# shanjiayao/PTT

Measured on AMD Instinct MI355X. Metric: tracklet frames/sec (hot path: PointNet++ SA stack + Point-Track-Transformer blocks), higher is better.
Workload: dtype f32

## Files before the change

### include/ptt_hip.h

```cpp
#ifndef PTT_HIP_H
#define PTT_HIP_H

#include <stddef.h>
#include <stdint.h>

#ifdef __cplusplus
extern "C" {
#endif

#define PTT_ABI_VERSION 28

enum {
    PTT_OK = 0,
    PTT_EINVAL = -1,
    PTT_EUNSUPPORTED = -2,
    PTT_ELAUNCH = -3,
    PTT_EWORKSPACE = -4
};

typedef void* ptt_stream_t;

int ptt_version(void);
const char* ptt_error_name(int code);
const char* ptt_last_error_string(void);

int ptt_fps_f32(const float* xyz, int B, int N, int npoint, int32_t* idx_out,
                ptt_stream_t stream);
int ptt_fps_ws_f32(const float* xyz, int B, int N, int npoint, int32_t* idx_out, float* workspace,
                   size_t workspace_elems, ptt_stream_t stream);

int ptt_gather_f32(const float* feat, const int32_t* idx, int B, int C, int N, int M,
                   float* out, ptt_stream_t stream);
int ptt_gather_grad_f32(const float* grad_out, const int32_t* idx, int B, int C, int N,
                        int M, float* grad_feat, ptt_stream_t stream);

int ptt_select_centres_f32(const float* xyz, const int32_t* idx, int B, int N, int M, float* new_xyz,
                           int64_t* idx64_out, ptt_stream_t stream);

int ptt_ball_query_f32(const float* new_xyz, const float* xyz, int B, int M, int N,
                       float radius, int nsample, int32_t* idx_out, ptt_stream_t stream);

int ptt_centres_ball_query_f32(const float* xyz, const int32_t* sel, int B, int N, int M, float radius, int nsample,
                               float* new_xyz, int64_t* idx64_out, int32_t* idx_out, ptt_stream_t stream);

int ptt_group_f32(const float* feat, const int32_t* idx, int B, int C, int N, int M,
                  int ns, float* out, ptt_stream_t stream);
int ptt_group_grad_f32(const float* grad_out, const int32_t* idx, int B, int C, int N,
                       int M, int ns, float* grad_feat, ptt_stream_t stream);

size_t ptt_scatter_add_det_workspace(int B, int N, int E);
int ptt_scatter_add_det_f32(const float* src, const int32_t* idx, int B, int C, int N, int E, float* out,
                            void* workspace, size_t workspace_bytes, ptt_stream_t stream);

int ptt_knn_f32(const float* xyz, int B, int N, int k, int32_t* idx_out,
                ptt_stream_t stream);
int ptt_knn_rel_f32(const float* xyz, int B, int N, int k, int32_t* idx_out, float* rel_out,
                    ptt_stream_t stream);

size_t ptt_packed_weight_elems(int Cout, int K);
int ptt_pack_weight_f32(const float* W, int Cout, int K, float* packed,
                        ptt_stream_t stream);
int ptt_pack_weight_rot_f32(const float* W, int Cout, int K, int rot, float* packed,
                            ptt_stream_t stream);

int ptt_linear_f32(const float* X, int rows, int K, int ldx, const float* Wpacked, int Cout,
                   const float* scale, const float* shift, int relu, const float* residual,
                   int ldr, float* out, int ldo, ptt_stream_t stream);

#define PTT_SA_MAX_LAYERS 4

typedef struct ptt_sa_layer {
    const float* Wpacked;
    const float* scale;
    const float* shift;
    int Cin;
    int Cout;
    int relu;
} ptt_sa_layer;

int ptt_rows_mlp_f32(const float* X, int rows, int K, int ldx, const ptt_sa_layer* layers, int n_layers,
                     const float* residual, int ldr, float* out, int ldo, ptt_stream_t stream);

size_t ptt_ball_query_grid_workspace(int B, int N);
int ptt_ball_query_grid_f32(const float* new_xyz, const float* xyz, int B, int M, int N, float radius, int nsample,
                            int32_t* idx_out, void* workspace, size_t workspace_bytes, ptt_stream_t stream);
int ptt_centres_ball_query_grid_f32(const float* xyz, const int32_t* sel, int B, int N, int M, float radius, int nsample,
                                    float* new_xyz, int64_t* idx64_out, int32_t* idx_out, void* workspace, size_t workspace_bytes,
                                    ptt_stream_t stream);
int ptt_fps_ball_knn_f32(const float* xyz, int B, int N, int M, float radius, int nsample, int k, int32_t* inds,
                         int64_t* inds64, float* new_xyz, int32_t* idx, int32_t* knn, float* rel, ptt_stream_t stream);
#define PTT_POINT_JOBS_MAX 4
typedef struct ptt_point_job {
    const float* xyz; const int32_t* centre_sel; const int32_t* point_sel;
    float* new_xyz; int64_t* idx64_out; int32_t* idx_out; float* rel_out;
    int32_t kind, sel_ld, B, Nraw, Npts, M, nsample;
    float radius;
} ptt_point_job;
int ptt_point_jobs_f32(const ptt_point_job* jobs, int n_jobs, ptt_stream_t stream);

#define PTT_ROW_JOBS_MAX 4
typedef struct ptt_row_job {
    const float* X; const float* X2;
    const float* Xmax;
    const float* Wpacked; const float* scale; const float* shift;
    const float* res; const float* res2;
    float* out; float* out2; float* raw;
    const float* rel; const float* w1;
    const float* qkv; const int32_t* knn; const float* pos;
    int32_t rows, K, K1, ldx, ldx2, Cout;
    int32_t act, res_split, ldr, ldr2, out_split, out_col0, ldo, ldo2, ldraw;
    int32_t prologue, epilogue, ldq, q_off, k_off, v_off, ldp, N;
    float sm_scale;
    int32_t col_tiles;
    const int32_t* idx; const float* xyz; const float* centres; const float* wx;
    float radius;
    int32_t ns, M, normalize_xyz, pro_relu;
} ptt_row_job;
int ptt_row_jobs_f32(const ptt_row_job* jobs, int n_jobs, ptt_stream_t stream);

typedef struct ptt_sa_desc {
    const float* xyz;
    const float* new_xyz;
    const int32_t* idx;
    const float* feat;
    int64_t feat_sb, feat_sc, feat_sn;
    float* out;
    int64_t out_sb, out_sc, out_sm;
    int B, N, M, nsample, C;
    float radius;
    int use_xyz;
    int normalize_xyz;
    int n_layers;
    ptt_sa_layer layers[PTT_SA_MAX_LAYERS];
    const float* l0_point_term;
    const float* l0_xyz_weight;
    int l0_channels;
    int l0_relu;
    void* compact_ws;
    size_t compact_ws_bytes;
} ptt_sa_desc;

int ptt_sa_fused_fwd_f32(const ptt_sa_desc* d, ptt_stream_t stream);
size_t ptt_sa_compact_workspace(int B, int M);

typedef struct ptt_xcorr_desc {
    const float* cos_t;
    const float* P;
    const float* w_sim;
    const float* scale0;
    const float* shift0;
    float* out;
    int64_t out_sb, out_sc, out_sn;
    float* sim_out;
    int B, Ns, Nt, C0;
    int n_layers;
    ptt_sa_layer layers[PTT_SA_MAX_LAYERS];
    int32_t split; int64_t out_sh;
    const float* search_feat; const float* templ_feat;
    int64_t s_sb, s_sn, t_sb, t_sn;
    int C; float eps;
} ptt_xcorr_desc;

int ptt_xcorr_fused_fwd_f32(const ptt_xcorr_desc* d, ptt_stream_t stream);

int ptt_cosine_map_f32(const float* search_feat, int64_t s_sb, int64_t s_sn, int64_t s_sc, const float* templ_feat,
                       int64_t t_sb, int64_t t_sn, int64_t t_sc, int B, int Ns, int Nt, int C, float eps,
                       float* cos_t, ptt_stream_t stream);

typedef struct ptt_attn_desc {
    const float* xyz;
    const float* rel;
    const int32_t* knn;
    const float* qkv;
    const float* Wd1p;
    const float* Wd2p;
    const float* bd2;
    const float* Wg1p;
    const float* bg1;
    const float* Wg2p;
    const float* bg2;
    float* res;
    float* attn;
    int B, N, k, D;
    const int32_t* order;
    int heads;
} ptt_attn_desc;

int ptt_pt_attn_pair_f32(const ptt_attn_desc* d, ptt_stream_t stream);
int ptt_spatial_order_f32(const float* xyz, int B, int N, int32_t* order, ptt_stream_t stream);

typedef struct ptt_crop_job {
    const float* points;
    int64_t ld;
    double lo1[3], hi1[3];
    double trans[3];
    double rot[9];
    double lo2[3], hi2[3];
    float* out;
    int32_t* count;
    int32_t n_points;
    int32_t capacity;
    uint8_t* label_out;
    double ltrans[3];
    double lrot[9];
    double llo[3], lhi[3];
    int32_t append;
    int32_t reserved;
} ptt_crop_job;

int ptt_crop_compact_f32(const ptt_crop_job* jobs_device, int n_jobs, ptt_stream_t stream);
#define PTT_CROP_JOBS_BY_VALUE_MAX 8
int ptt_crop_compact_host_f32(const ptt_crop_job* jobs_host, int n_jobs, ptt_stream_t stream);

#define PTT_MAX_SEGMENTS 4
typedef struct ptt_regularize_job {
    const float* seg[PTT_MAX_SEGMENTS];
    const int32_t* seg_count[PTT_MAX_SEGMENTS];
    int32_t seg_capacity[PTT_MAX_SEGMENTS];
    float* out;
    int32_t* info;
    int32_t n_seg;
    int32_t input_size;
} ptt_regularize_job;

int ptt_regularize_f32(const ptt_regularize_job* jobs_device, int n_jobs, const uint32_t* draws, int n_draws,
                       ptt_stream_t stream);
int ptt_crop_regularize_f32(const ptt_crop_job* crop_jobs, const ptt_regularize_job* reg_jobs_device, int n_jobs,
                            const uint32_t* draws, int n_draws, ptt_stream_t stream);

int ptt_mt19937_fill(uint32_t seed, uint32_t* out_host, int n);

typedef struct ptt_track_box {
    double center[3];
    double wlh[3];
    double quat[4];
} ptt_track_box;

int ptt_track_crop_bounds(const ptt_track_box* boxes, int n, double offset, double scale, const double* extra2,
                          ptt_crop_job* jobs_host, int job_stride);
int ptt_track_box_by_offset(ptt_track_box* boxes, int n, float* offsets, int offset_stride, int use_z,
                            const int32_t* active, int64_t* rng_pos);
int ptt_track_select_update(const float* proposals_host, int P, const int32_t* info_host, ptt_track_box* boxes, int n, int use_z,
                            const int32_t* active, int64_t* rng_pos, float* est_out);

int ptt_select_box_f32(const float* pred_box_data, int B, int P, float* out, int32_t* idx_out, ptt_stream_t stream);

#define PTT_REF_CAMERA 0
#define PTT_REF_LIDAR 1
int ptt_box_overlap_f64(const double* gt, const double* pred, int n, int ref_coord, int dims, double* overlap, double* accuracy,
                        ptt_stream_t stream);

#define PTT_TRAIN_MAX_CANDS 1024
typedef struct ptt_train_cand {
    const float* search;
    const uint8_t* label;
    const float* first;
    const float* prev;
    const int32_t* counts;
    float reg[4];
    uint32_t index;
    uint32_t epoch;
    int32_t capacity;
    int32_t reserved;
} ptt_train_cand;

typedef struct ptt_train_batch_desc {
    float* search_points;
    float* template_points;
    float* cls_label;
    float* reg_label;
    int32_t* src_out;
    int32_t* idx_search_out;
    int32_t* idx_template_out;
    int32_t* info;
    int64_t* totals;
    int32_t B, n_cand;
    int32_t search_size, template_size;
    int32_t min_points;
    uint32_t seed_lo, seed_hi;
    int32_t reserved;
} ptt_train_batch_desc;

int ptt_train_batch_f32(const ptt_train_cand* cands_device, const ptt_train_batch_desc* desc_host, ptt_stream_t stream);
int ptt_philox4x32_10(const uint32_t* counter4, const uint32_t* key2, uint32_t* out4);

size_t ptt_bn_stats_workspace(int R, int C);
int ptt_bn_stats_f32(const float* X, int R, int C, int ldx, float eps, float* mean, float* var, float* invstd,
                     void* workspace, size_t workspace_bytes, ptt_stream_t stream);
int ptt_bn_apply_f32(const float* Z, int ldz, const float* mean, const float* invstd, const float* gamma,
                     const float* beta, int R, int C, int relu, float* X, int ldx, ptt_stream_t stream);
int ptt_bn_bwd_f32(const float* G, int ldg, const float* Act, int lda, const float* Z, int ldz, const float* mean,
                   const float* invstd, const float* gamma, int R, int C, int relu, float* dZ, int ldd,
// ... 227 lines not shown
```

### ptt_amd/_lib.py

```python
import ctypes
import os
import re
from ctypes import Structure, c_char_p, c_double, c_float, c_int, c_int32, c_int64, c_longlong, c_size_t, c_uint32, c_void_p

from .build import HEADER as HEADER_PATH, LIB as LIB_PATH


def _strip_comments(text):
    return re.sub(r"/\*.*?\*/|//[^\n]*", " ", text, flags=re.S)


def parse_defines(text):
    return {n: int(v) for n, v in re.findall(r"^[ \t]*#[ \t]*define[ \t]+(PTT_\w+)[ \t]+(-?\d+)[ \t]*$", _strip_comments(text), re.M)}


CTYPES = {"int": c_int, "int32_t": c_int32, "uint32_t": c_uint32, "int64_t": c_int64, "long long": c_longlong, "size_t": c_size_t,
          "float": c_float, "double": c_double, "ptt_stream_t": c_void_p}


def _ctype(decl, name, is_return=False):
    words = decl.replace("*", " * ").split()
    if not is_return and len(words) > 1 and words[-1] != "*":
        words.pop()
    if "*" in words:
        if not is_return:
            return c_void_p
        if words == ["const", "char", "*"]:
            return c_char_p
    base = " ".join(w for w in words if w != "const")
    if base not in CTYPES:
        raise RuntimeError("ptt_amd: %s of %s in include/ptt_hip.h has the type '%s', which ptt_amd/_lib.py does not map to ctypes"
                           % ("the return value" if is_return else "parameter '%s'" % decl.strip(), name, base))
    return CTYPES[base]


def parse_prototypes(text):
    text = re.sub(r"^[ \t]*#.*$", " ", _strip_comments(text), flags=re.M).replace('extern "C" {', " ")
    text = re.sub(r"\{[^{}]*\}", " ", text)
    protos = {}
    for stmt in text.split(";"):
        stmt = " ".join(stmt.split()).lstrip("} ")
        if not stmt or stmt.split()[0] in ("typedef", "enum", "struct"):
            continue
        m = re.fullmatch(r"(.+?)\b(\w+) ?\((.*)\)", stmt)
        if m is None:
            raise RuntimeError("ptt_amd: cannot read '%s' in include/ptt_hip.h as a function prototype" % stmt)
        ret, name, params = m.groups()
        params = [] if params.strip() == "void" else params.split(",")
        protos[name] = (_ctype(ret, name, is_return=True), [_ctype(p, name) for p in params])
    return protos


def _read_header():
    if not os.path.exists(HEADER_PATH):
        raise RuntimeError("ptt_amd: %s is missing — the Python binding takes every prototype and constant of the C ABI from it" % HEADER_PATH)
    with open(HEADER_PATH) as fh:
        return fh.read()


_header = _read_header()
PROTOTYPES = parse_prototypes(_header)
EXPORTS = list(PROTOTYPES)
DEFINES = parse_defines(_header)
ABI_VERSION = DEFINES["PTT_ABI_VERSION"]
PTT_SA_MAX_LAYERS = DEFINES["PTT_SA_MAX_LAYERS"]
PTT_MAX_SEGMENTS = DEFINES["PTT_MAX_SEGMENTS"]
PTT_CROP_JOBS_BY_VALUE_MAX = DEFINES["PTT_CROP_JOBS_BY_VALUE_MAX"]
PTT_TRAIN_MAX_CANDS = DEFINES["PTT_TRAIN_MAX_CANDS"]


class CropJob(Structure):
    _fields_ = [("points", c_void_p), ("ld", c_int64),
                ("lo1", c_double * 3), ("hi1", c_double * 3), ("trans", c_double * 3), ("rot", c_double * 9),
                ("lo2", c_double * 3), ("hi2", c_double * 3),
                ("out", c_void_p), ("count", c_void_p), ("n_points", c_int32), ("capacity", c_int32),
                ("label_out", c_void_p), ("ltrans", c_double * 3), ("lrot", c_double * 9), ("llo", c_double * 3), ("lhi", c_double * 3),
                ("append", c_int32), ("reserved", c_int32)]


class RegularizeJob(Structure):
    _fields_ = [("seg", c_void_p * PTT_MAX_SEGMENTS), ("seg_count", c_void_p * PTT_MAX_SEGMENTS),
                ("seg_capacity", c_int32 * PTT_MAX_SEGMENTS), ("out", c_void_p), ("info", c_void_p),
                ("n_seg", c_int32), ("input_size", c_int32)]


class TrackBox(Structure):
    _fields_ = [("center", c_double * 3), ("wlh", c_double * 3), ("quat", c_double * 4)]


class TrainCand(Structure):
    _fields_ = [("search", c_void_p), ("label", c_void_p), ("first", c_void_p), ("prev", c_void_p), ("counts", c_void_p),
                ("reg", c_float * 4), ("index", c_uint32), ("epoch", c_uint32), ("capacity", c_int32), ("reserved", c_int32)]


class TrainBatchDesc(Structure):
    _fields_ = [("search_points", c_void_p), ("template_points", c_void_p), ("cls_label", c_void_p), ("reg_label", c_void_p),
                ("src_out", c_void_p), ("idx_search_out", c_void_p), ("idx_template_out", c_void_p), ("info", c_void_p), ("totals", c_void_p),
                ("B", c_int32), ("n_cand", c_int32), ("search_size", c_int32), ("template_size", c_int32), ("min_points", c_int32),
                ("seed_lo", c_uint32), ("seed_hi", c_uint32), ("reserved", c_int32)]


class BnTrainTail(Structure):
    _fields_ = [("gamma", c_void_p), ("beta", c_void_p), ("act_a", c_void_p), ("act_b", c_void_p),
                ("running_mean", c_void_p), ("running_var", c_void_p), ("num_batches_tracked", c_void_p), ("momentum", c_float)]


class BnBwdInput(Structure):
    _fields_ = [("g", c_void_p), ("ldg", c_int), ("arg", c_void_p), ("ns", c_int), ("z", c_void_p), ("ldz", c_int),
                ("k1", c_void_p), ("c0", c_void_p), ("c1", c_void_p), ("mean", c_void_p), ("act_a", c_void_p), ("act_b", c_void_p),
                ("dz_out", c_void_p), ("ldd", c_int)]


class PackJob(Structure):
    _fields_ = [("W", c_void_p), ("out_offset", c_int64), ("stride_out", c_int64), ("stride_k", c_int64),
                ("Cout", c_int32), ("K", c_int32)]


class RowJob(Structure):
    _fields_ = [("X", c_void_p), ("X2", c_void_p), ("Xmax", c_void_p), ("Wpacked", c_void_p), ("scale", c_void_p), ("shift", c_void_p),
                ("res", c_void_p), ("res2", c_void_p), ("out", c_void_p), ("out2", c_void_p), ("raw", c_void_p),
                ("rel", c_void_p), ("w1", c_void_p), ("qkv", c_void_p), ("knn", c_void_p), ("pos", c_void_p),
                ("rows", c_int32), ("K", c_int32), ("K1", c_int32), ("ldx", c_int32), ("ldx2", c_int32), ("Cout", c_int32),
                ("act", c_int32), ("res_split", c_int32), ("ldr", c_int32), ("ldr2", c_int32), ("out_split", c_int32),
                ("out_col0", c_int32), ("ldo", c_int32), ("ldo2", c_int32), ("ldraw", c_int32),
                ("prologue", c_int32), ("epilogue", c_int32), ("ldq", c_int32), ("q_off", c_int32), ("k_off", c_int32),
                ("v_off", c_int32), ("ldp", c_int32), ("N", c_int32), ("sm_scale", c_float), ("col_tiles", c_int32),
                ("idx", c_void_p), ("xyz", c_void_p), ("centres", c_void_p), ("wx", c_void_p), ("radius", c_float),
                ("ns", c_int32), ("M", c_int32), ("normalize_xyz", c_int32), ("pro_relu", c_int32)]


class PointJob(Structure):
    _fields_ = [("xyz", c_void_p), ("centre_sel", c_void_p), ("point_sel", c_void_p), ("new_xyz", c_void_p), ("idx64_out", c_void_p),
                ("idx_out", c_void_p), ("rel_out", c_void_p), ("kind", c_int32), ("sel_ld", c_int32), ("B", c_int32),
                ("Nraw", c_int32), ("Npts", c_int32), ("M", c_int32), ("nsample", c_int32), ("radius", c_float)]


class TrackLossDesc(Structure):
    _fields_ = [("seed_cls", c_void_p), ("cls_label", c_void_p), ("search_inds", c_void_p), ("votes", c_void_p), ("reg_label", c_void_p),
                ("box_data", c_void_p), ("centres", c_void_p), ("pos_weight_seed", c_void_p), ("pos_weight_box", c_void_p),
                ("B", c_int32), ("N", c_int32), ("Ns", c_int32), ("M", c_int32), ("ld_reg", c_int32),
                ("w_seed_cls", c_float), ("w_seed_reg", c_float), ("w_box_cls", c_float), ("w_box_reg", c_float)]


class AdamTensor(Structure):
    _fields_ = [("param", c_void_p), ("grad", c_void_p), ("exp_avg", c_void_p), ("exp_avg_sq", c_void_p), ("n", c_int64)]


class GradJob(Structure):
    _fields_ = [("partial", c_void_p), ("nchunks", c_int32), ("reserved", c_int32)]


class GradSegment(Structure):
    _fields_ = [("dst", c_int64), ("n", c_int32), ("cols", c_int32), ("ld", c_int32), ("job0", c_int32), ("njobs", c_int32), ("out", c_int32),
                ("vec", c_int32), ("reserved", c_int32)]


class AdamHyper(Structure):
    _fields_ = [("beta1", c_float), ("beta2", c_float), ("one_minus_beta1", c_float), ("one_minus_beta2", c_float), ("eps", c_float), ("step_size", c_float), ("bias2_sqrt", c_float),
                ("weight_decay", c_float), ("max_norm", c_float), ("write_clipped", c_int32)]


class SaLayer(Structure):
    _fields_ = [("Wpacked", c_void_p), ("scale", c_void_p), ("shift", c_void_p),
                ("Cin", c_int), ("Cout", c_int), ("relu", c_int)]


class SaDesc(Structure):
    _fields_ = [("xyz", c_void_p), ("new_xyz", c_void_p), ("idx", c_void_p), ("feat", c_void_p),
                ("feat_sb", c_int64), ("feat_sc", c_int64), ("feat_sn", c_int64),
                ("out", c_void_p), ("out_sb", c_int64), ("out_sc", c_int64), ("out_sm", c_int64),
                ("B", c_int), ("N", c_int), ("M", c_int), ("nsample", c_int), ("C", c_int),
                ("radius", c_float), ("use_xyz", c_int), ("normalize_xyz", c_int), ("n_layers", c_int),
                ("layers", SaLayer * PTT_SA_MAX_LAYERS),
                ("l0_point_term", c_void_p), ("l0_xyz_weight", c_void_p), ("l0_channels", c_int), ("l0_relu", c_int),
                ("compact_ws", c_void_p), ("compact_ws_bytes", c_size_t)]


class XcorrDesc(Structure):
    _fields_ = [("cos_t", c_void_p), ("P", c_void_p), ("w_sim", c_void_p), ("scale0", c_void_p), ("shift0", c_void_p),
                ("out", c_void_p), ("out_sb", c_int64), ("out_sc", c_int64), ("out_sn", c_int64),
                ("sim_out", c_void_p),
                ("B", c_int), ("Ns", c_int), ("Nt", c_int), ("C0", c_int),
                ("n_layers", c_int), ("layers", SaLayer * PTT_SA_MAX_LAYERS),
                ("split", c_int32), ("out_sh", c_int64), ("search_feat", c_void_p), ("templ_feat", c_void_p),
                ("s_sb", c_int64), ("s_sn", c_int64), ("t_sb", c_int64), ("t_sn", c_int64), ("C", c_int), ("eps", c_float)]


class AttnDesc(Structure):
    _fields_ = [("xyz", c_void_p), ("rel", c_void_p), ("knn", c_void_p), ("qkv", c_void_p),
                ("Wd1p", c_void_p), ("Wd2p", c_void_p), ("bd2", c_void_p),
                ("Wg1p", c_void_p), ("bg1", c_void_p), ("Wg2p", c_void_p), ("bg2", c_void_p),
                ("res", c_void_p), ("attn", c_void_p),
                ("B", c_int), ("N", c_int), ("k", c_int), ("D", c_int), ("order", c_void_p), ("heads", c_int)]


_lib = None


def lib():
    global _lib
    if _lib is None:
        if not os.path.exists(LIB_PATH):
            raise RuntimeError(
                "ptt_amd: %s is missing — build it with `python -m ptt_amd.build` "
                "(hipcc --offload-arch=gfx950); there is no CPU fallback" % LIB_PATH)
        import torch
        try:
            loaded = ctypes.CDLL(LIB_PATH)
        except OSError as e:
            raise RuntimeError("ptt_amd: cannot load %s: %s" % (LIB_PATH, e))
        for name, (restype, argtypes) in PROTOTYPES.items():
            fn = getattr(loaded, name)
            fn.restype, fn.argtypes = restype, argtypes
        if loaded.ptt_version() != ABI_VERSION:
            raise RuntimeError("ptt_amd: %s has ABI version %d, this package expects %d — rebuild it with "
                               "`python -m ptt_amd.build`" % (LIB_PATH, loaded.ptt_version(), ABI_VERSION))
        _lib = loaded
    return _lib


def check(rc, what):
    if rc != 0:
        l = lib()
        raise RuntimeError("%s failed: %s (%s)" % (what, l.ptt_error_name(rc).decode(),
                                                   l.ptt_last_error_string().decode()))
```

### ptt_amd/csrc/common.h

```cpp
#pragma once
#include <hip/hip_runtime.h>
#include <stdint.h>
#include <stdio.h>
#include "../../include/ptt_hip.h"

namespace ptt {

char* last_error_buf();
int fail(int code, const char* fmt, ...);
int check_launch(const char* what);

static inline hipStream_t as_stream(ptt_stream_t s) { return reinterpret_cast<hipStream_t>(s); }

struct DevSwitches {
    int linear_rt = 1, linear_ct = 1;
    int linear_small = 1;
    int sa_gather1 = 0;
    int sa_stagger = 0;
    int sa_wave = 1;
    int sa_rt = 2;
    int sa_lds = 1;
    int sa_stream = 1;
    int sa_chunk = 2;
    int pair_stagger = 0;
    int pair_lds_pad = 0;
    int sa_lds_chunk = 2;
    int fps_plain = 0;
    int ball_cpw = 0;
    int fps_t = 0;
    int group_grad_global = 0;
    long long* stamps = nullptr;
};
const DevSwitches& dev_switches();

int set_lds_limit(const void* fn, int bytes);

bool wgrad_stream_ok(int R, int Cout, int Cin, int ldz, int ldx);
int wgrad_stream_rows(int R);
int launch_wgrad_stream(const float* dZ, int ldz, const float* X, int ldx, int R, int Cout, int Cin, int rows, float* partial,
                        const float* x_scale, const float* x_shift, hipStream_t s);

template <int CTRL, int ROW_MASK>
__device__ __forceinline__ int dpp_i32(int v) {
    return __builtin_amdgcn_update_dpp(v, v, CTRL, ROW_MASK, 0xF, false);
}
template <int CTRL, int ROW_MASK>
__device__ __forceinline__ float dpp_f32(float v) {
    return __builtin_bit_cast(float, dpp_i32<CTRL, ROW_MASK>(__builtin_bit_cast(int, v)));
}

__device__ __forceinline__ float wave_max_f32(float v) {
    v = fmaxf(v, dpp_f32<0xB1, 0xF>(v));
    v = fmaxf(v, dpp_f32<0x4E, 0xF>(v));
    v = fmaxf(v, dpp_f32<0x141, 0xF>(v));
    v = fmaxf(v, dpp_f32<0x140, 0xF>(v));
    v = fmaxf(v, dpp_f32<0x142, 0xA>(v));
    v = fmaxf(v, dpp_f32<0x143, 0xC>(v));
    return __builtin_bit_cast(float, __builtin_amdgcn_readlane(__builtin_bit_cast(int, v), 63));
}
__device__ __forceinline__ float wave_max_f32_fused(float v) {
    asm volatile(
        "s_nop 1\n\tv_max_f32_dpp %0, %0, %0 quad_perm:[1,0,3,2] row_mask:0xf bank_mask:0xf\n\t"
        "s_nop 1\n\tv_max_f32_dpp %0, %0, %0 quad_perm:[2,3,0,1] row_mask:0xf bank_mask:0xf\n\t"
        "s_nop 1\n\tv_max_f32_dpp %0, %0, %0 row_half_mirror row_mask:0xf bank_mask:0xf\n\t"
        "s_nop 1\n\tv_max_f32_dpp %0, %0, %0 row_mirror row_mask:0xf bank_mask:0xf\n\t"
        "s_nop 1\n\tv_max_f32_dpp %0, %0, %0 row_bcast:15 row_mask:0xa bank_mask:0xf\n\t"
        "s_nop 1\n\tv_max_f32_dpp %0, %0, %0 row_bcast:31 row_mask:0xc bank_mask:0xf\n\t"
        "s_nop 1"
        : "+v"(v));
    return __builtin_bit_cast(float, __builtin_amdgcn_readlane(__builtin_bit_cast(int, v), 63));
}

__device__ __forceinline__ float wave_min_f32(float v) {
    v = fminf(v, dpp_f32<0xB1, 0xF>(v));
    v = fminf(v, dpp_f32<0x4E, 0xF>(v));
    v = fminf(v, dpp_f32<0x141, 0xF>(v));
    v = fminf(v, dpp_f32<0x140, 0xF>(v));
    v = fminf(v, dpp_f32<0x142, 0xA>(v));
    v = fminf(v, dpp_f32<0x143, 0xC>(v));
    return __builtin_bit_cast(float, __builtin_amdgcn_readlane(__builtin_bit_cast(int, v), 63));
}
__device__ __forceinline__ int wave_min_i32(int v) {
    v = min(v, dpp_i32<0xB1, 0xF>(v));
    v = min(v, dpp_i32<0x4E, 0xF>(v));
    v = min(v, dpp_i32<0x141, 0xF>(v));
    v = min(v, dpp_i32<0x140, 0xF>(v));
    v = min(v, dpp_i32<0x142, 0xA>(v));
    v = min(v, dpp_i32<0x143, 0xC>(v));
    return __builtin_amdgcn_readlane(v, 63);
}

}
```

### ptt_amd/csrc/mfma_ops.hip

```cpp
#include <math.h>
#include <stdlib.h>
#include <string.h>
#include "common.h"
#include "mfma_common.h"

#ifndef PTT_PAIR_PF
#define PTT_PAIR_PF 1
#endif
#ifndef PTT_GATHER_BATCH
#define PTT_GATHER_BATCH 16
#endif
#ifndef PTT_SA_WAVES
#define PTT_SA_WAVES 2
#endif

namespace ptt {

#ifdef PTT_DEV
#define PTT_STAMP(i) do { if (p.dbg && threadIdx.x == 0 && blockIdx.x < 4096) p.dbg[blockIdx.x * 8 + (i)] = __builtin_readcyclecounter(); } while (0)
#else
#define PTT_STAMP(i) do { } while (0)
#endif

__device__ __forceinline__ void stagger_second_slot(int first_wave_blocks, int quanta) {
// ... 1099 lines not shown
            for (int c = sub * 4; c < q.C; c += 32) {
                const f32x4 av = *reinterpret_cast<const f32x4*>(a + c), sv = *reinterpret_cast<const f32x4*>(sv_ + c);
#pragma unroll
                for (int k = 0; k < 4; ++k) { dot += av[k] * sv[k]; na += av[k] * av[k]; ns += sv[k] * sv[k]; }
            }
#pragma unroll
            for (int m = 1; m < 8; m <<= 1) { dot += __shfl_xor(dot, m, 64); na += __shfl_xor(na, m, 64); ns += __shfl_xor(ns, m, 64); }
            if (sub == 0) simv[i] = dot / (fmaxf(sqrtf(na), q.eps) * fmaxf(sqrtf(ns), q.eps));
        } else {
            if (t < ROWS) {
                const float cs = q.cos_t[(unsigned)((b * p.M + jj) * q.Nt + i0 + t)];
                simv[t] = cs;
                if (q.sim_out) q.sim_out[(unsigned)((b * q.Nt + i0 + t) * p.M + jj)] = cs;
            }
        }
        __syncthreads();

        const int nq = q.C0 >> 2;
        if (!q.scale0 && !q.shift0 && (q.C0 & 3) == 0 && (256 % nq) == 0) {
            typedef float f32x2 __attribute__((ext_vector_type(2)));
            const int c4 = t % nq, step = 256 / nq;
            const f32x4 w4 = *reinterpret_cast<const f32x4*>(q.wsim + c4 * 4);
            const float* prow = q.P + ((size_t)(b * q.Nt + i0) * q.C0 + c4 * 4);
            for (int i = t / nq; i < ROWS; i += step) {
                const f32x4 pv = *reinterpret_cast<const f32x4*>(prow + (unsigned)(i * q.C0));
                const float cs = simv[i];
                const f32x2 c2 = {cs, cs};
                f32x2 lo = __builtin_elementwise_fma(f32x2{w4[0], w4[1]}, c2, f32x2{pv[0], pv[1]});
                f32x2 hi = __builtin_elementwise_fma(f32x2{w4[2], w4[3]}, c2, f32x2{pv[2], pv[3]});
                *reinterpret_cast<f32x4*>(Xs + i * p.ldk + c4 * 4) =
                    f32x4{fmaxf(lo[0], 0.f), fmaxf(lo[1], 0.f), fmaxf(hi[0], 0.f), fmaxf(hi[1], 0.f)};
            }
        } else {
            for (int c = t; c < q.C0; c += 256) {
                const float wsim = q.wsim[c], sc = q.scale0 ? q.scale0[c] : 1.f, sh = q.shift0 ? q.shift0[c] : 0.f;
                const float* pr = q.P + ((long long)b * q.Nt + i0) * q.C0 + c;
#pragma unroll 8
                for (int i = 0; i < ROWS; ++i) {
                    const float v = (pr[(long long)i * q.C0] + wsim * simv[i]) * sc + sh;
                    Xs[i * p.ldk + c] = fmaxf(v, 0.f);
                }
            }
        }
        __syncthreads();

        for (int l = 0; l < nlast; ++l) {
            const SaLayerDev& L = p.L[l];
            const int ctw = (L.NT + 3) >> 2;
            if (ctw <= 1) sa_layer<32 * RT, 1, RT>(p, L, false, Xs, lane, w, j, 1, pre, &p.L[l + 1]);
            else sa_layer<32 * RT, 2, RT>(p, L, false, Xs, lane, w, j, 1, pre, &p.L[l + 1]);
        }
        {
            const bool affine = LL.scale != nullptr;
            f32x16 acc[RT][2];
#pragma unroll
            for (int rt = 0; rt < RT; ++rt)
#pragma unroll
                for (int u = 0; u < 2; ++u)
#pragma unroll
                    for (int r = 0; r < 16; ++r) acc[rt][u][r] = pre.sh[u];
            int nvalid = 0;
#pragma unroll
            for (int u = 0; u < 2; ++u)
                if (w + 4 * u < LL.NT) nvalid = u + 1;
            gemm_tiles<RT, 2, 0>(Xs, p.ldk, LL.nkb, reinterpret_cast<const f32x4*>(LL.Wp), LL.NT, w, nvalid, lane, acc, pre.w);
#pragma unroll
            for (int u = 0; u < 2; ++u) {
                if (u >= nvalid) break;
                const int col = (w + 4 * u) * 32 + (lane & 31);
                float sc = 1.f, sh = 0.f;
                if (affine) { sc = LL.scale[col]; sh = LL.shift ? LL.shift[col] : 0.f; }
#pragma unroll
                for (int rt = 0; rt < RT; ++rt) {
                    float m = affine ? acc[rt][u][0] * sc + sh : acc[rt][u][0];
#pragma unroll
                    for (int r = 1; r < 16; ++r) m = fmaxf(m, affine ? acc[rt][u][r] * sc + sh : acc[rt][u][r]);
                    run[u] = fmaxf(run[u], max_halves(m));
                }
            }
        }
    }
    if (half == 0) {
#pragma unroll
        for (int u = 0; u < 2; ++u) {
            if (w + 4 * u >= LL.NT) break;
            const int col = (w + 4 * u) * 32 + (lane & 31);
            p.out[(SPLIT ? hsel * q.out_sh : 0) + b * p.osb + col * p.osc + jj * p.osm] = LL.relu ? fmaxf(run[u], 0.f) : run[u];
        }
    }
}

template <int NS, int CT, bool AFFINE, int RT>
__device__ __forceinline__ void sa_wave_layer(const SaParams& p, const SaLayerDev& L, bool last, float* Xw, int lane,
                                              int centre0, int ncentres) {
    f32x16 acc[RT][CT];
#pragma unroll
    for (int u = 0; u < CT; ++u) {
        const float s0 = (!AFFINE && L.shift) ? L.shift[u * 32 + (lane & 31)] : 0.f;
#pragma unroll
        for (int rt = 0; rt < RT; ++rt)
#pragma unroll
            for (int r = 0; r < 16; ++r) acc[rt][u][r] = s0;
    }
    gemm_core<RT, CT, CT, 1>(Xw, p.ldk, L.nkb, reinterpret_cast<const f32x4*>(L.Wp), L.NT, 0, lane, acc);
    __builtin_amdgcn_wave_barrier();
    const int half = lane >> 5;
#pragma unroll
    for (int u = 0; u < CT; ++u) {
        const int col = u * 32 + (lane & 31);
        float sc = 1.f, sv = 0.f;
        if constexpr (AFFINE) { sc = L.scale[col]; sv = L.shift ? L.shift[col] : 0.f; }
#pragma unroll
        for (int rt = 0; rt < RT; ++rt) {
            float y[16];
#pragma unroll
            for (int r = 0; r < 16; ++r) y[r] = AFFINE ? acc[rt][u][r] * sc + sv : acc[rt][u][r];
            if (!last) {
#pragma unroll
                for (int r = 0; r < 16; ++r)
                    Xw[(rt * 32 + tile_row(r, half)) * p.ldk + col] = L.relu ? fmaxf(y[r], 0.f) : y[r];
            } else if (NS == 32) {
                float m = y[0];
#pragma unroll
                for (int r = 1; r < 16; ++r) m = fmaxf(m, y[r]);
                m = max_halves(m);
                if (L.relu) m = fmaxf(m, 0.f);
                if (half == 0 && rt < ncentres) {
                    const int c = centre0 + rt; const int b = c / p.M, mm = c - b * p.M;
                    p.out[b * p.osb + col * p.osc + mm * p.osm] = m;
                }
            } else {
                float m0 = y[0], m1 = y[8];
#pragma unroll
                for (int r = 1; r < 8; ++r) { m0 = fmaxf(m0, y[r]); m1 = fmaxf(m1, y[8 + r]); }
                m0 = max_halves(m0);
                m1 = max_halves(m1);
                if (L.relu) { m0 = fmaxf(m0, 0.f); m1 = fmaxf(m1, 0.f); }
                if (half == 0) {
                    if (2 * rt < ncentres) {
                        const int c = centre0 + 2 * rt; const int b = c / p.M, mm = c - b * p.M;
                        p.out[b * p.osb + col * p.osc + mm * p.osm] = m0;
                    }
                    if (2 * rt + 1 < ncentres) {
                        const int c = centre0 + 2 * rt + 1; const int b = c / p.M, mm = c - b * p.M;
                        p.out[b * p.osb + col * p.osc + mm * p.osm] = m1;
                    }
                }
            }
        }
    }
    __builtin_amdgcn_wave_barrier();
}

constexpr int SAC_HDR = 16;
struct SacTable {
    int32_t* ws; int T;
    __host__ __device__ int32_t* ndist() const { return ws + SAC_HDR; }
    __host__ __device__ int32_t* list(int k) const { return ws + SAC_HDR + (size_t)(1 + k) * T; }
    __host__ __device__ int32_t* rows(int k) const { return ws + SAC_HDR + 5 * (size_t)T + (size_t)((4 << k) - 4) * T; }
    static size_t words(size_t T) { return SAC_HDR + 65 * T; }
};
constexpr int SAC_PASSES = 4;

__global__ __launch_bounds__(64) void sa_compact_zero_kernel(int32_t* ws) {
    if (threadIdx.x < 4) ws[threadIdx.x] = 0;
}

template <bool XYZ>
__global__ __launch_bounds__(256) void sa_compact_kernel(const float* __restrict__ xyz, const int32_t* __restrict__ idx, int N, int M,
                                                         SacTable tab) {
    __shared__ int s_cnt[4], s_base[4], s_cls[32], s_pos[32], s_nd[32];
    __shared__ int s_row[32][32];
    const int t = threadIdx.x, lane = t & 63, half = lane >> 5, s = lane & 31, w = t >> 6;
    const int g0 = blockIdx.x * 32, T = tab.T;
    if (t < 4) s_cnt[t] = 0;
    __syncthreads();
    int iv[SAC_PASSES];
    uint32_t x[SAC_PASSES], y[SAC_PASSES], z[SAC_PASSES];
#pragma unroll
    for (int q = 0; q < SAC_PASSES; ++q) iv[q] = idx[(size_t)min(g0 + q * 8 + w * 2 + half, T - 1) * 32 + s];
    if constexpr (XYZ) {
#pragma unroll
        for (int q = 0; q < SAC_PASSES; ++q) {
            const int b = min(g0 + q * 8 + w * 2 + half, T - 1) / M;
            const uint32_t* pt = reinterpret_cast<const uint32_t*>(xyz) + ((size_t)b * N + iv[q]) * 3;
            x[q] = pt[0]; y[q] = pt[1]; z[q] = pt[2];
        }
    }
#pragma unroll
    for (int q = 0; q < SAC_PASSES; ++q) {
        const int lc = q * 8 + w * 2 + half;
        const int i0a = __builtin_amdgcn_readlane(iv[q], 0), i0b = __builtin_amdgcn_readlane(iv[q], 32);
        const int i0 = half ? i0b : i0a;
        const bool real = s == 0 || iv[q] != i0;
        int dup = 0;
        if constexpr (XYZ) {
            const unsigned long long rm = __ballot(real);
            const int J = 31 - __builtin_clz((uint32_t)rm | (uint32_t)(rm >> 32));
            for (int j = 0; j < J; ++j) {
                const uint32_t xa = __builtin_amdgcn_readlane(x[q], j), xb = __builtin_amdgcn_readlane(x[q], 32 + j);
                const uint32_t ya = __builtin_amdgcn_readlane(y[q], j), yb = __builtin_amdgcn_readlane(y[q], 32 + j);
                const uint32_t za = __builtin_amdgcn_readlane(z[q], j), zb = __builtin_amdgcn_readlane(z[q], 32 + j);
                dup |= (int)(j < s) & (int)(x[q] == (half ? xb : xa)) & (int)(y[q] == (half ? yb : ya)) & (int)(z[q] == (half ? zb : za));
            }
        }
        const bool keep = real && !dup;
        const unsigned long long km = __ballot(keep);
        const uint32_t m = half ? (uint32_t)(km >> 32) : (uint32_t)km;
        const int nd = __popc(m);
        if (keep) s_row[lc][__popc(m & ((1u << s) - 1u))] = iv[q];
        if (s == 0) {
            const int k = nd <= 4 ? 0 : nd <= 8 ? 1 : nd <= 16 ? 2 : 3;
            const bool valid = g0 + lc < T;
            s_cls[lc] = valid ? k : -1;
            s_nd[lc] = nd;
            s_pos[lc] = valid ? atomicAdd(&s_cnt[k], 1) : 0;
            if (valid) tab.ndist()[g0 + lc] = nd;
        }
    }
    __syncthreads();
    if (t < 4) s_base[t] = s_cnt[t] ? atomicAdd(&tab.ws[t], s_cnt[t]) : 0;
    __syncthreads();
    for (int e = t; e < 32 * 32; e += 256) {
        const int lc = e >> 5, j = e & 31, k = s_cls[lc];
        if (k < 0 || j >= (4 << k)) continue;
        const int q = s_base[k] + s_pos[lc];
        tab.rows(k)[(size_t)q * (4 << k) + j] = s_row[lc][j < s_nd[lc] ? j : 0];
        if (j == 0) tab.list(k)[q] = g0 + lc;
    }
}

#ifndef PTT_SAL_WGS
#define PTT_SAL_WGS 1
#endif
#ifndef PTT_SAL_WAVES
#define PTT_SAL_WAVES 12
#endif

template <int ROWS>
struct SacTileT {
    static constexpr int LG = ROWS == 32 ? 3 : 4;
    static_assert(ROWS == 32 || ROWS == 64, "32- or 64-row tiles");
    int k, first, n;
    __device__ __forceinline__ static void count(const int32_t* ws, int total, int (&cnt)[4], int (&tiles)[4]) {
#pragma unroll
        for (int k = 0; k < 4; ++k) {
            cnt[k] = min(max(ws[k], 0), total);
            tiles[k] = (k ? tiles[k - 1] : 0) + ((cnt[k] + ((1 << LG) >> k) - 1) >> (LG - k));
        }
    }
    __device__ __forceinline__ void at(int j, const int (&tiles)[4], const int (&cnt)[4]) {
        k = j < tiles[0] ? 0 : j < tiles[1] ? 1 : j < tiles[2] ? 2 : 3;
        const int j0 = k == 0 ? 0 : k == 1 ? tiles[0] : k == 2 ? tiles[1] : tiles[2];
        const int nk = k == 0 ? cnt[0] : k == 1 ? cnt[1] : k == 2 ? cnt[2] : cnt[3];
        first = (j - j0) << (LG - k);
        n = min((1 << LG) >> k, nk - first);
    }
    __device__ __forceinline__ void row(const SacTable& tab, int s, int& n_out, int& ball) const {
        const int cl = s >> (2 + k), inb = cl < n;
        n_out = tab.rows(k)[(size_t)first * (4 << k) + (inb ? s : (s & ((4 << k) - 1)))];
        ball = tab.list(k)[first + (inb ? cl : 0)];
    }
};
using SacTile = SacTileT<32>;

template <int NU>
__device__ __forceinline__ void sac_store(int k, int n, int ball, int M, const f32x16 (&acc)[NU], const float (&sh)[NU],
                                          float* const (&o)[NU], int relu, int half, int osb, int osm) {
    int ob[8];
#pragma unroll
    for (int g = 0; g < 8; ++g) {
        if (g >= (8 >> k)) break;
        const int id = __builtin_amdgcn_readlane(ball, g << (2 + k)), b = id / M;
        ob[g] = b * osb + (id - b * M) * osm;
    }
#pragma unroll
    for (int u = 0; u < NU; ++u) {
        const f32x16& a = acc[u];
        if (k == 3) {
            const float mx = sas_pool(a, sh[u], relu);
            if (half == 0) o[u][ob[0]] = mx;
        } else if (k == 2) {
            float m0 = a[0], m1 = a[8];
#pragma unroll
            for (int r = 1; r < 8; ++r) { m0 = fmaxf(m0, a[r]); m1 = fmaxf(m1, a[8 + r]); }
            m0 = max_halves(m0) + sh[u]; m1 = max_halves(m1) + sh[u];
            if (relu) { m0 = fmaxf(m0, 0.f); m1 = fmaxf(m1, 0.f); }
            if (half < n) o[u][half ? ob[1] : ob[0]] = half ? m1 : m0;
        } else {
            float m[4];
#pragma unroll
            for (int q = 0; q < 4; ++q) m[q] = fmaxf(fmaxf(a[4 * q], a[4 * q + 1]), fmaxf(a[4 * q + 2], a[4 * q + 3]));
            if (k == 1) {
#pragma unroll
                for (int q = 0; q < 4; ++q) m[q] = max_halves(m[q]) + sh[u];
#pragma unroll
                for (int i = 0; i < 2; ++i) {
                    const int g = 2 * half + i;
                    float v = half ? m[2 + i] : m[i];
                    if (relu) v = fmaxf(v, 0.f);
                    if (g < n) o[u][half ? ob[2 + i] : ob[i]] = v;
                }
            } else {
#pragma unroll
                for (int q = 0; q < 4; ++q) {
                    const int g = 2 * q + half;
                    float v = m[q] + sh[u];
                    if (relu) v = fmaxf(v, 0.f);
                    if (g < n) o[u][half ? ob[2 * q + 1] : ob[2 * q]] = v;
                }
            }
        }
    }
}
// ... 473 lines not shown
extern "C" int ptt_pack_weight_strided_f32(const float* W, int Cout, int K, int64_t stride_out, int64_t stride_k, int batch,
                                           int64_t stride_batch, float* packed, ptt_stream_t stream) {
    if (Cout <= 0 || K <= 0 || batch < 0) return fail(PTT_EINVAL, "ptt_pack_weight_strided_f32: Cout=%d K=%d batch=%d", Cout, K, batch);
    if (batch == 0) return PTT_OK;
    if (!W || !packed) return fail(PTT_EINVAL, "ptt_pack_weight_strided_f32: null pointer");
    const size_t total = ptt_packed_weight_elems(Cout, K);
    const int NT = (Cout + 31) / 32;
    size_t g = (total + 255) / 256;
    if (g > 1024) g = 1024;
    hipLaunchKernelGGL(pack_weight_kernel, dim3((unsigned)g, (unsigned)batch), dim3(256), 0, as_stream(stream), W, Cout, K, NT, 0,
                       total, packed, (long long)stride_out, (long long)stride_k, (long long)stride_batch);
    return check_launch("pack_weight_kernel");
}

extern "C" int ptt_pack_weights_f32(const ptt_pack_job* jobs_device, int n_jobs, float* arena, ptt_stream_t stream) {
    if (n_jobs < 0) return fail(PTT_EINVAL, "ptt_pack_weights_f32: n_jobs=%d", n_jobs);
    if (n_jobs == 0) return PTT_OK;
    if (!jobs_device || !arena) return fail(PTT_EINVAL, "ptt_pack_weights_f32: null pointer");
    if (n_jobs > 65535) return fail(PTT_EUNSUPPORTED, "ptt_pack_weights_f32: n_jobs=%d exceeds one launch (65535)", n_jobs);
    hipLaunchKernelGGL(pack_weights_kernel, dim3(32, (unsigned)n_jobs), dim3(256), 0, as_stream(stream), jobs_device, arena);
    return check_launch("pack_weights_kernel");
}

extern "C" int ptt_pack_weight_f32(const float* W, int Cout, int K, float* packed, ptt_stream_t stream) {
    return ptt_pack_weight_rot_f32(W, Cout, K, 0, packed, stream);
}

static int linear_launch(const float* X, int rows, int K, int ldx, const float* Wpacked, int Cout, const float* scale,
                         const float* shift, int relu, const float* residual, int ldr, float* out, int ldo, int batch,
                         long long xb, long long wb, long long ob, long long rb, ptt_stream_t stream,
                         const float* in_a = nullptr, const float* in_b = nullptr);

extern "C" int ptt_linear_act_in_f32(const float* X, int rows, int K, int ldx, const float* in_scale, const float* in_shift,
                                     const float* Wpacked, int Cout, float* out, int ldo, ptt_stream_t stream) {
    if (!in_scale || !in_shift || (K & 3) || (ldx & 3) || ((reinterpret_cast<uintptr_t>(X) | reinterpret_cast<uintptr_t>(in_scale) |
                                                             reinterpret_cast<uintptr_t>(in_shift)) & 15))
        return fail(PTT_EINVAL, "ptt_linear_act_in_f32: needs K %% 4 == 0, ldx %% 4 == 0 and 16-byte aligned X / in_scale / in_shift");
    return linear_launch(X, rows, K, ldx, Wpacked, Cout, nullptr, nullptr, 0, nullptr, 0, out, ldo, 1, 0, 0, 0, 0, stream, in_scale,
                         in_shift);
}

extern "C" int ptt_linear_f32(const float* X, int rows, int K, int ldx, const float* Wpacked, int Cout,
                              const float* scale, const float* shift, int relu, const float* residual, int ldr,
                              float* out, int ldo, ptt_stream_t stream) {
    return linear_launch(X, rows, K, ldx, Wpacked, Cout, scale, shift, relu, residual, ldr, out, ldo, 1, 0, 0, 0, 0, stream);
}

extern "C" int ptt_linear_batched_f32(const float* X, int rows, int K, int ldx, int64_t x_batch_stride, const float* Wpacked,
                                      int64_t w_batch_stride, int Cout, const float* scale, const float* shift, int relu,
                                      const float* residual, int ldr, int64_t r_batch_stride, float* out, int ldo,
                                      int64_t o_batch_stride, int batch, ptt_stream_t stream) {
    if (batch < 0 || batch > 65535) return fail(PTT_EINVAL, "ptt_linear_batched_f32: batch=%d", batch);
    if (batch == 0) return PTT_OK;
    return linear_launch(X, rows, K, ldx, Wpacked, Cout, scale, shift, relu, residual, ldr, out, ldo, batch, x_batch_stride,
                         w_batch_stride, o_batch_stride, r_batch_stride, stream);
}

static int linear_launch(const float* X, int rows, int K, int ldx, const float* Wpacked, int Cout, const float* scale,
                         const float* shift, int relu, const float* residual, int ldr, float* out, int ldo, int batch,
                         long long xb, long long wb, long long ob, long long rb, ptt_stream_t stream, const float* in_a,
                         const float* in_b) {
    if (rows < 0 || K <= 0 || Cout <= 0 || ldx < K || ldo < Cout || (residual && ldr < Cout))
        return fail(PTT_EINVAL, "ptt_linear_f32: rows=%d K=%d Cout=%d ldx=%d ldo=%d ldr=%d", rows, K, Cout, ldx, ldo,
                    ldr);
    if (rows == 0) return PTT_OK;
    if (!X || !Wpacked || !out) return fail(PTT_EINVAL, "ptt_linear_f32: null pointer");
    LinearParams p;
    p.X = X; p.Wp = Wpacked; p.scale = scale; p.shift = shift; p.residual = residual; p.out = out;
    p.rows = rows; p.K = K; p.ldx = ldx; p.Cout = Cout; p.relu = relu; p.ldr = ldr; p.ldo = ldo;
    p.nkb = (K + 7) / 8; p.NT = (Cout + 31) / 32;
    p.vec_ok = ((ldx & 3) == 0 && (xb & 3) == 0 && (reinterpret_cast<uintptr_t>(X) & 15) == 0) ? 1 : 0;
    p.xb = xb; p.wb = wb; p.ob = ob; p.rb = rb;
    p.in_a = in_a; p.in_b = in_b;
    const bool vec = p.vec_ok && (K & 3) == 0;
    hipStream_t s = as_stream(stream);
    if (dev_switches().linear_small && vec && batch == 1 && !in_a && rows <= 8192 && K <= 520 && K >= 32) {
        const int hb = ((p.nkb + 1) / 2 + LS_PD - 1) / LS_PD * LS_PD;
        const int lds = (32 * (2 * hb * 8 + 4) + 4 * 16 * 64) * (int)sizeof(float);
        if (int rc = set_lds_limit(reinterpret_cast<const void*>(linear_small_kernel), lds)) return rc;
        hipLaunchKernelGGL(linear_small_kernel, dim3((rows + 31) / 32, (p.NT + 3) / 4), dim3(512), lds, s, p);
        return check_launch("linear_small_kernel");
    }
    const int rt64 = (rows + 63) / 64, rt32 = (rows + 31) / 32, cg256 = (p.NT + 7) / 8, cg128 = (p.NT + 3) / 4;
    int RT = dev_switches().linear_rt, CT = dev_switches().linear_ct;
    if (rows >= 32768 && Cout >= 256 && RT == 1 && CT == 1) CT = 2;
    const int lds = 2 * (RT * 32) * LIN_LDK * (int)sizeof(float);
    const dim3 grid(RT == 2 ? rt64 : rt32, CT == 2 ? cg256 : cg128, batch);
    int rc = PTT_OK;
#define PTT_LIN_CASE(R, V, C)                                                                                  \
    if (RT == R && vec == V && CT == C) {                                                                      \
        if ((rc = set_lds_limit(reinterpret_cast<const void*>(linear_kernel<R, V, C>), lds))) return rc;       \
        hipLaunchKernelGGL((linear_kernel<R, V, C>), grid, dim3(256), lds, s, p);                              \
    }
    PTT_LIN_CASE(1, true, 1) PTT_LIN_CASE(1, true, 2) PTT_LIN_CASE(1, false, 1) PTT_LIN_CASE(1, false, 2)
#ifdef PTT_DEV
    PTT_LIN_CASE(2, true, 1) PTT_LIN_CASE(2, true, 2) PTT_LIN_CASE(2, false, 1) PTT_LIN_CASE(2, false, 2)
#endif
#undef PTT_LIN_CASE
    return check_launch("linear_kernel");
}

extern "C" int ptt_rows_mlp_f32(const float* X, int rows, int K, int ldx, const ptt_sa_layer* layers, int n_layers,
                                const float* residual, int ldr, float* out, int ldo, ptt_stream_t stream) {
    if (rows < 0 || K <= 0 || ldx < K || n_layers < 1 || n_layers > PTT_SA_MAX_LAYERS || !layers)
        return fail(PTT_EINVAL, "ptt_rows_mlp_f32: rows=%d K=%d ldx=%d layers=%d", rows, K, ldx, n_layers);
    if (rows == 0) return PTT_OK;
    if (!X || !out) return fail(PTT_EINVAL, "ptt_rows_mlp_f32: null pointer");
    if (K > 264) return fail(PTT_EUNSUPPORTED, "ptt_rows_mlp_f32: K=%d (at most 264 input channels)", K);
    RowsMlpParams p;
    p.X = X; p.residual = residual; p.out = out; p.rows = rows; p.K0 = K; p.ldx = ldx; p.ldr = ldr; p.ldo = ldo;
    p.n_layers = n_layers;
    int maxk = 0, cin = K;
    for (int l = 0; l < n_layers; ++l) {
        const ptt_sa_layer& s = layers[l];
        const bool last = l == n_layers - 1;
        if (s.Cin != cin) return fail(PTT_EINVAL, "ptt_rows_mlp_f32: layer %d Cin=%d, expected %d", l, s.Cin, cin);
        if (s.Cout <= 0 || s.Cout > (last ? 384 : 256))
            return fail(PTT_EUNSUPPORTED, "ptt_rows_mlp_f32: layer %d Cout=%d (inner layers <= 256, the last <= 384)", l, s.Cout);
        if (!s.Wpacked) return fail(PTT_EINVAL, "ptt_rows_mlp_f32: layer %d has no weights", l);
        SaLayerDev& L = p.L[l];
        L.Wp = s.Wpacked; L.scale = s.scale; L.shift = s.shift; L.Cin = s.Cin; L.Cout = s.Cout; L.relu = s.relu;
        L.nkb = (s.Cin + 7) / 8; L.NT = (s.Cout + 31) / 32;
        if (L.nkb * 8 > maxk) maxk = L.nkb * 8;
        if (!last && L.NT * 32 > maxk) maxk = L.NT * 32;
        cin = s.Cout;
    }
    if (ldo < cin || (residual && ldr < cin)) return fail(PTT_EINVAL, "ptt_rows_mlp_f32: ldo=%d ldr=%d Cout=%d", ldo, ldr, cin);
    p.ldk = maxk + 4;
    p.vec_in = ((K & 3) == 0 && (ldx & 3) == 0 && (reinterpret_cast<uintptr_t>(X) & 15) == 0) ? 1 : 0;
    const int lds = 32 * p.ldk * (int)sizeof(float);
    int rc = set_lds_limit(reinterpret_cast<const void*>(rows_mlp_kernel), lds);
    if (rc) return rc;
    hipLaunchKernelGGL(rows_mlp_kernel, dim3((rows + 31) / 32), dim3(256), lds, as_stream(stream), p);
    return check_launch("rows_mlp_kernel");
}

extern "C" size_t ptt_sa_compact_workspace(int B, int M) {
    const long long T = (long long)(B > 0 ? B : 0) * (M > 0 ? M : 0);
    return SacTable::words((size_t)T) * sizeof(int32_t);
}

extern "C" int ptt_sa_fused_fwd_f32(const ptt_sa_desc* d, ptt_stream_t stream) {
    if (!d) return fail(PTT_EINVAL, "ptt_sa_fused_fwd_f32: null descriptor");
    if (d->B < 0 || d->N <= 0 || d->M < 0 || d->C < 0 || d->n_layers < 1 || d->n_layers > PTT_SA_MAX_LAYERS)
        return fail(PTT_EINVAL, "ptt_sa_fused_fwd_f32: B=%d N=%d M=%d C=%d layers=%d", d->B, d->N, d->M, d->C,
                    d->n_layers);
    if (d->nsample != 16 && d->nsample != 32 && d->nsample != 64)
        return fail(PTT_EUNSUPPORTED, "ptt_sa_fused_fwd_f32: nsample=%d (16, 32 and 64 are instantiated)", d->nsample);
    if (d->B == 0 || d->M == 0) return PTT_OK;
    const bool hoist = d->l0_point_term != nullptr;
    if (!d->xyz || !d->new_xyz || !d->idx || !d->out || (!hoist && d->C > 0 && !d->feat))
        return fail(PTT_EINVAL, "ptt_sa_fused_fwd_f32: null pointer");
    if (!d->use_xyz && d->C == 0) return fail(PTT_EINVAL, "ptt_sa_fused_fwd_f32: no xyz and no features");
    if (hoist) {
        const int c0 = d->l0_channels;
        if (!d->use_xyz || !d->l0_xyz_weight || c0 <= 0 || (c0 % 32) != 0 || c0 > 256 ||
            (reinterpret_cast<uintptr_t>(d->l0_point_term) & 15) != 0 ||
            (reinterpret_cast<uintptr_t>(d->l0_xyz_weight) & 15) != 0)
            return fail(PTT_EINVAL, "ptt_sa_fused_fwd_f32: hoisted layer 0 needs use_xyz, 16-byte aligned (B,N,C0) and "
                        "(3,C0) arrays and C0 a multiple of 32 <= 256 (C0=%d)", c0);
    }

    SaParams p;
    p.xyz = d->xyz; p.new_xyz = d->new_xyz; p.idx = d->idx; p.feat = d->feat; p.out = d->out;
    p.fsb = d->feat_sb; p.fsc = d->feat_sc; p.fsn = d->feat_sn;
    p.osb = d->out_sb; p.osc = d->out_sc; p.osm = d->out_sm;
    p.B = d->B; p.N = d->N; p.M = d->M; p.C = d->C; p.use_xyz = d->use_xyz ? 1 : 0;
    p.normalize = d->normalize_xyz ? 1 : 0; p.n_layers = d->n_layers; p.radius = d->radius;
    p.K0 = (d->use_xyz ? 3 : 0) + d->C;
    p.hoist = hoist ? 1 : 0; p.l0_relu = d->l0_relu ? 1 : 0; p.wx = d->l0_xyz_weight;
    if (hoist && d->l0_channels == 128 && (unsigned long long)d->B * d->N * 128ull * sizeof(float) < 0x7fffffffull &&
        !dev_switches().sa_gather1)
        p.hoist = 2;
    if (hoist) {
        p.feat = d->l0_point_term; p.C = d->l0_channels; p.K0 = p.C;
        p.fsc = 1; p.fsn = p.C; p.fsb = (long long)d->N * p.C;
    }
    int maxk = 0, cin = p.K0;
    for (int l = 0; l < d->n_layers; ++l) {
        const ptt_sa_layer& s = d->layers[l];
        if (s.Cin != cin) return fail(PTT_EINVAL, "ptt_sa_fused_fwd_f32: layer %d Cin=%d, expected %d", l, s.Cin, cin);
        if (s.Cout <= 0 || (s.Cout % 32) != 0 || s.Cout > 256)
            return fail(PTT_EUNSUPPORTED, "ptt_sa_fused_fwd_f32: layer %d Cout=%d must be a multiple of 32 <= 256", l,
                        s.Cout);
        if (!s.Wpacked) return fail(PTT_EINVAL, "ptt_sa_fused_fwd_f32: layer %d has no weights", l);
        SaLayerDev& L = p.L[l];
        L.Wp = s.Wpacked; L.scale = s.scale; L.shift = s.shift; L.Cin = s.Cin; L.Cout = s.Cout; L.relu = s.relu;
        L.nkb = (s.Cin + 7) / 8; L.NT = s.Cout / 32;
        if (L.nkb * 8 > maxk) maxk = L.nkb * 8;
        if (l + 1 < d->n_layers && s.Cout > maxk) maxk = s.Cout;
        cin = s.Cout;
    }
    {
        const unsigned long long lim = 0x7fffffffull, B = (unsigned long long)d->B;
        if (B * d->N * 12ull >= lim || B * d->M * d->nsample * 4ull >= lim || B * d->M * (unsigned long long)cin * 4ull >= lim ||
            B * d->N * (unsigned long long)(p.C > 0 ? p.C : 1) * 4ull >= lim)
            return fail(PTT_EUNSUPPORTED, "ptt_sa_fused_fwd_f32: B=%d N=%d M=%d: an array of this launch exceeds 2 GiB "
                        "(32-bit offsets) — split the batch", d->B, d->N, d->M);
    }
    p.ldk = maxk + 4;
    p.vec_gather = (p.C > 0 && p.fsc == 1 && (p.C & 3) == 0 && p.C <= 256 && (p.fsn & 3) == 0 &&
                    (p.fsb & 3) == 0 && (reinterpret_cast<uintptr_t>(p.feat) & 15) == 0) ? 1 : 0;
    p.first_wave = 1024; p.stagger = dev_switches().sa_stagger;
    p.dbg = dev_switches().stamps;
    p.cws = nullptr;
    const int total_centres = d->B * d->M;
    hipStream_t s = as_stream(stream);
    int rc;
    if (d->C == 0 && d->use_xyz && !hoist && d->nsample == 32 && d->n_layers == 3 && p.L[0].Cout == 64 && p.L[1].Cout == 64 &&
        p.L[2].Cout == 128 && !p.L[0].scale && !p.L[1].scale && !p.L[2].scale && p.L[0].relu && p.L[1].relu &&
        dev_switches().sa_lds) {
        const int waves = 256 * PTT_SAL_WAVES * PTT_SAL_WGS;
        p.chunk = (total_centres + waves - 1) / waves;
        if (dev_switches().sa_lds_chunk > 0 && p.chunk > dev_switches().sa_lds_chunk) p.chunk = dev_switches().sa_lds_chunk;
        const int nw = total_centres * 3 <= 256 * PTT_SAL_WAVES ? 4 : PTT_SAL_WAVES;
        int wgs = (total_centres + p.chunk * nw - 1) / (p.chunk * nw);
        const int lds = (4096 + 8192 + PTT_SAL_WAVES * 640) * (int)sizeof(float);
        if (d->compact_ws) {
            if (d->compact_ws_bytes < ptt_sa_compact_workspace(d->B, d->M) || (reinterpret_cast<uintptr_t>(d->compact_ws) & 15))
                return fail(PTT_EWORKSPACE, "ptt_sa_fused_fwd_f32: compact_ws needs %zu bytes, 16-byte aligned (got %zu)",
                            ptt_sa_compact_workspace(d->B, d->M), d->compact_ws_bytes);
            p.cws = static_cast<int32_t*>(d->compact_ws);
            hipLaunchKernelGGL(sa_compact_zero_kernel, dim3(1), dim3(64), 0, s, p.cws);
            if ((rc = check_launch("sa_compact_zero_kernel"))) return rc;
            hipLaunchKernelGGL(sa_compact_kernel<true>, dim3((total_centres + 31) / 32), dim3(256), 0, s, d->xyz, d->idx, d->N, d->M,
                               SacTable{p.cws, total_centres});
            if ((rc = check_launch("sa_compact_kernel"))) return rc;
            if (wgs > 256 * PTT_SAL_WGS) wgs = 256 * PTT_SAL_WGS;
            if ((rc = set_lds_limit(reinterpret_cast<const void*>(sa_lds_kernel<true>), lds))) return rc;
            hipLaunchKernelGGL(sa_lds_kernel<true>, dim3(wgs), dim3(64 * nw), lds, s, p);
            return check_launch("sa_lds_kernel");
        }
        if ((rc = set_lds_limit(reinterpret_cast<const void*>(sa_lds_kernel<false>), lds))) return rc;
        hipLaunchKernelGGL(sa_lds_kernel<false>, dim3(wgs), dim3(64 * nw), lds, s, p);
        return check_launch("sa_lds_kernel");
    }
    size_t wbytes = 0;
    bool wave_ok = true;
    for (int l = 0; l < d->n_layers; ++l) {
        wbytes += (size_t)d->layers[l].Cin * d->layers[l].Cout * sizeof(float);
        const int nt = d->layers[l].Cout / 32;
        if (!(nt == 1 || nt == 2 || nt == 4)) wave_ok = false;
    }
    wave_ok = wave_ok && dev_switches().sa_wave;
    if (wave_ok && wbytes <= 64 * 1024 && d->nsample <= 32) {
        const int lds = 4 * 32 * p.ldk * (int)sizeof(float);
        const int cpw = 32 / d->nsample, per_wg = 4 * cpw;
        const dim3 grid((total_centres + per_wg - 1) / per_wg);
        if (d->nsample == 32) {
            if ((rc = set_lds_limit(reinterpret_cast<const void*>(sa_wave_kernel<32, 1>), lds))) return rc;
            hipLaunchKernelGGL((sa_wave_kernel<32, 1>), grid, dim3(256), lds, s, p);
        } else {
            if ((rc = set_lds_limit(reinterpret_cast<const void*>(sa_wave_kernel<16, 1>), lds))) return rc;
            hipLaunchKernelGGL((sa_wave_kernel<16, 1>), grid, dim3(256), lds, s, p);
        }
        return check_launch("sa_wave_kernel");
    }
    if (p.hoist == 2 && d->nsample == 32 && d->n_layers == 2 && p.L[0].Cin == 128 && p.L[0].Cout == 128 &&
        p.L[1].Cout == 256 && !p.L[0].scale && !p.L[1].scale && p.L[0].relu && dev_switches().sa_stream) {
        p.tiles = (total_centres + 1) / 2;
        int wgs = p.tiles < 512 ? p.tiles : 512;
        p.chunk = (p.tiles + wgs - 1) / wgs;
        if (dev_switches().sa_chunk > 0 && p.chunk > dev_switches().sa_chunk) p.chunk = dev_switches().sa_chunk;
        wgs = (p.tiles + p.chunk - 1) / p.chunk;
        if (d->compact_ws) {
            if (d->compact_ws_bytes < ptt_sa_compact_workspace(d->B, d->M) || (reinterpret_cast<uintptr_t>(d->compact_ws) & 15))
                return fail(PTT_EWORKSPACE, "ptt_sa_fused_fwd_f32: compact_ws needs %zu bytes, 16-byte aligned (got %zu)",
                            ptt_sa_compact_workspace(d->B, d->M), d->compact_ws_bytes);
            p.cws = static_cast<int32_t*>(d->compact_ws);
            hipLaunchKernelGGL(sa_compact_zero_kernel, dim3(1), dim3(64), 0, s, p.cws);
            if ((rc = check_launch("sa_compact_zero_kernel"))) return rc;
            hipLaunchKernelGGL(sa_compact_kernel<false>, dim3((total_centres + 31) / 32), dim3(256), 0, s, d->xyz, d->idx, d->N, d->M,
                               SacTable{p.cws, total_centres});
            if ((rc = check_launch("sa_compact_kernel"))) return rc;
            const int lds = (2 * SAS_TILE + 64 * 4 + 64) * (int)sizeof(float);
            if ((rc = set_lds_limit(reinterpret_cast<const void*>(sa_stream_compact_kernel), lds))) return rc;
            hipLaunchKernelGGL(sa_stream_compact_kernel, dim3(p.tiles < 512 ? p.tiles : 512), dim3(256), lds, s, p);
            return check_launch("sa_stream_compact_kernel");
        }
        const int lds = (2 * SAS_TILE + 4 * 16 * 4) * (int)sizeof(float);
        if ((rc = set_lds_limit(reinterpret_cast<const void*>(sa_stream_kernel<32>), lds))) return rc;
        hipLaunchKernelGGL((sa_stream_kernel<32>), dim3(wgs), dim3(256), lds, s, p);
        return check_launch("sa_stream_kernel");
    }
    int RT = dev_switches().sa_rt;
    if (d->nsample == 64) RT = 2;
    const int lds = 32 * RT * p.ldk * (int)sizeof(float);
    if (lds > 160 * 1024) return fail(PTT_EUNSUPPORTED, "ptt_sa_fused_fwd_f32: %d B of LDS per workgroup", lds);
    const int cpw = 32 * RT / d->nsample;
    const dim3 grid((total_centres + cpw - 1) / cpw);
#define PTT_SA_CASE(NSV, RTV)                                                                                   \
    if (d->nsample == NSV && RT == RTV) {                                                                       \
        if ((rc = set_lds_limit(reinterpret_cast<const void*>(sa_fused_kernel<NSV, RTV>), lds))) return rc;     \
        hipLaunchKernelGGL((sa_fused_kernel<NSV, RTV>), grid, dim3(256), lds, s, p);                            \
    }
    PTT_SA_CASE(32, 2) PTT_SA_CASE(32, 1) PTT_SA_CASE(16, 2) PTT_SA_CASE(16, 1) PTT_SA_CASE(64, 2)
#undef PTT_SA_CASE
    return check_launch("sa_fused_kernel");
}

extern "C" int ptt_xcorr_fused_fwd_f32(const ptt_xcorr_desc* d, ptt_stream_t stream) {
    if (!d) return fail(PTT_EINVAL, "ptt_xcorr_fused_fwd_f32: null descriptor");
    if (d->B < 0 || d->Ns <= 0 || d->C0 <= 0 || d->n_layers < 1 || d->n_layers > PTT_SA_MAX_LAYERS)
        return fail(PTT_EINVAL, "ptt_xcorr_fused_fwd_f32: B=%d Ns=%d C0=%d layers=%d", d->B, d->Ns, d->C0, d->n_layers);
    if (d->Nt <= 0 || (d->Nt % 64) != 0)
        return fail(PTT_EUNSUPPORTED, "ptt_xcorr_fused_fwd_f32: Nt=%d (the template seeds are walked in chunks of 64)", d->Nt);
    if (d->n_layers < 2) return fail(PTT_EUNSUPPORTED, "ptt_xcorr_fused_fwd_f32: needs at least two MFMA layers after layer 0");
    if ((d->C0 % 8) != 0 || d->C0 > 256) return fail(PTT_EUNSUPPORTED, "ptt_xcorr_fused_fwd_f32: C0=%d", d->C0);
    if (d->B == 0) return PTT_OK;
    if (!d->P || !d->w_sim || !d->out) return fail(PTT_EINVAL, "ptt_xcorr_fused_fwd_f32: null pointer");
    if ((unsigned long long)d->B * d->Ns * d->Nt >= 0x7fffffffull || (unsigned long long)d->B * d->Nt * d->C0 >= 0x7fffffffull)
        return fail(PTT_EUNSUPPORTED, "ptt_xcorr_fused_fwd_f32: B=%d Ns=%d Nt=%d: 32-bit element offsets — split the batch",
                    d->B, d->Ns, d->Nt);
    XcorrParams q;
    q.P = d->P; q.wsim = d->w_sim; q.scale0 = d->scale0;
    q.shift0 = d->shift0; q.sim_out = d->sim_out; q.cos_t = d->cos_t;
    q.C0 = d->C0; q.Nt = d->Nt;
    q.sfeat = q.tfeat = nullptr; q.s_sb = q.s_sn = q.t_sb = q.t_sn = 0; q.C = 0; q.eps = 0.f; q.out_sh = 0;
    SaParams& p = q.sa;
    memset(&p, 0, sizeof(p));
    p.out = d->out; p.osb = d->out_sb; p.osc = d->out_sc; p.osm = d->out_sn;
    p.B = d->B; p.M = d->Ns; p.n_layers = d->n_layers;
    int maxk = d->C0, cin = d->C0;
    for (int l = 0; l < d->n_layers; ++l) {
        const ptt_sa_layer& s = d->layers[l];
        if (s.Cin != cin) return fail(PTT_EINVAL, "ptt_xcorr_fused_fwd_f32: layer %d Cin=%d, expected %d", l, s.Cin, cin);
        if (s.Cout <= 0 || (s.Cout % 32) != 0 || s.Cout > 256)
            return fail(PTT_EUNSUPPORTED, "ptt_xcorr_fused_fwd_f32: layer %d Cout=%d", l, s.Cout);
        if (!s.Wpacked) return fail(PTT_EINVAL, "ptt_xcorr_fused_fwd_f32: layer %d has no weights", l);
        SaLayerDev& L = p.L[l];
        L.Wp = s.Wpacked; L.scale = s.scale; L.shift = s.shift; L.Cin = s.Cin; L.Cout = s.Cout; L.relu = s.relu;
        L.nkb = (s.Cin + 7) / 8; L.NT = s.Cout / 32;
        if (l + 1 < d->n_layers && s.Cout > maxk) maxk = s.Cout;
        cin = s.Cout;
    }
    p.ldk = ((maxk + 7) / 8) * 8 + 4;
    p.first_wave = 1024; p.stagger = 2;
    if (d->split) {
        if (!d->search_feat || !d->templ_feat || d->sim_out || (d->C & 3) || (d->s_sb & 3) || (d->s_sn & 3) ||
            (d->t_sb & 3) || (d->t_sn & 3) || ((reinterpret_cast<uintptr_t>(d->search_feat) | reinterpret_cast<uintptr_t>(d->templ_feat)) & 15) ||
            ((d->B * d->Ns) & 7) || d->C <= 0)
            return fail(PTT_EINVAL, "ptt_xcorr_fused_fwd_f32: the split form needs the features (unit channel stride, C %% 4 == 0, 16-byte "
                                    "aligned rows), B * Ns %% 8 == 0 and no sim_out");
        q.sfeat = d->search_feat; q.tfeat = d->templ_feat; q.s_sb = d->s_sb; q.s_sn = d->s_sn; q.t_sb = d->t_sb; q.t_sn = d->t_sn;
        q.C = d->C; q.eps = d->eps; q.out_sh = d->out_sh;
        const int lds = (32 * p.ldk + 32) * (int)sizeof(float);
        int rc = set_lds_limit(reinterpret_cast<const void*>(xcorr_fused_kernel<1, true>), lds);
        if (rc) return rc;
        hipLaunchKernelGGL((xcorr_fused_kernel<1, true>), dim3(2 * d->B * d->Ns), dim3(256), lds, as_stream(stream), q);
        return check_launch("xcorr_fused_kernel");
    }
    if (!d->cos_t) return fail(PTT_EINVAL, "ptt_xcorr_fused_fwd_f32: null pointer (cos_t comes from ptt_cosine_map_f32)");
    const int lds = (64 * p.ldk + 64) * (int)sizeof(float);
    int rc = set_lds_limit(reinterpret_cast<const void*>(xcorr_fused_kernel<2, false>), lds);
    if (rc) return rc;
    hipLaunchKernelGGL((xcorr_fused_kernel<2, false>), dim3(d->B * d->Ns), dim3(256), lds, as_stream(stream), q);
    return check_launch("xcorr_fused_kernel");
}

extern "C" int ptt_cosine_map_f32(const float* search_feat, int64_t s_sb, int64_t s_sn, int64_t s_sc, const float* templ_feat,
                                  int64_t t_sb, int64_t t_sn, int64_t t_sc, int B, int Ns, int Nt, int C, float eps,
                                  float* cos_t, ptt_stream_t stream) {
    if (B < 0 || Ns <= 0 || Nt <= 0 || C <= 0) return fail(PTT_EINVAL, "ptt_cosine_map_f32: B=%d Ns=%d Nt=%d C=%d", B, Ns, Nt, C);
    if (B == 0) return PTT_OK;
    if (!search_feat || !templ_feat || !cos_t) return fail(PTT_EINVAL, "ptt_cosine_map_f32: null pointer");
    CosParams q;
    q.sfeat = search_feat; q.tfeat = templ_feat; q.cos_t = cos_t;
    q.s_sb = s_sb; q.s_sn = s_sn; q.s_sc = s_sc; q.t_sb = t_sb; q.t_sn = t_sn; q.t_sc = t_sc;
    q.B = B; q.Ns = Ns; q.Nt = Nt; q.C = C; q.eps = eps;
    hipLaunchKernelGGL(cos_map_kernel, dim3((B * Ns + 3) / 4), dim3(256), 0, as_stream(stream), q);
    return check_launch("cos_map_kernel");
}

extern "C" int ptt_pt_attn_pair_f32(const ptt_attn_desc* d, ptt_stream_t stream) {
    if (!d) return fail(PTT_EINVAL, "ptt_pt_attn_pair_f32: null descriptor");
    if (d->B < 0 || d->N <= 0) return fail(PTT_EINVAL, "ptt_pt_attn_pair_f32: B=%d N=%d", d->B, d->N);
    if (d->D != 512 || d->k != 16)
        return fail(PTT_EUNSUPPORTED, "ptt_pt_attn_pair_f32: D=%d k=%d (D=512, k=16 is instantiated)", d->D, d->k);
    if (d->B == 0) return PTT_OK;
    if (!d->xyz || !d->knn || !d->qkv || !d->Wd1p || !d->Wd2p || !d->bd2 || !d->Wg1p || !d->bg1 ||
        !d->Wg2p || !d->res)
        return fail(PTT_EINVAL, "ptt_pt_attn_pair_f32: null pointer");
    AttnParams p;
    p.xyz = d->xyz; p.rel = d->rel; p.knn = d->knn; p.qkv = d->qkv; p.Wd1p = d->Wd1p; p.Wd2p = d->Wd2p; p.bd2 = d->bd2;
    p.Wg1p = d->Wg1p; p.bg1 = d->bg1; p.Wg2p = d->Wg2p; p.bg2 = d->bg2; p.res = d->res; p.attn = d->attn;
    p.order = d->order;
    p.BN = d->B * d->N; p.N = d->N;
    p.first_wave = 512; p.stagger = dev_switches().pair_stagger;
    p.dbg = dev_switches().stamps;
    if ((d->N & 1) != 0)
        return fail(PTT_EUNSUPPORTED, "ptt_pt_attn_pair_f32: N=%d must be even (a tile holds two points of one cloud)",
                    d->N);
    const int heads = d->heads ? d->heads : 1;
    int lds = (32 * (512 + 4) + 32 + 32 * 12) * (int)sizeof(float);
    lds += dev_switches().pair_lds_pad;
    const void* kern;
    switch (heads) {
        case 1: kern = reinterpret_cast<const void*>(pt_attn_pair_kernel<512>); break;
        case 2: kern = reinterpret_cast<const void*>(pt_attn_pair_heads_kernel<2>); break;
        case 4: kern = reinterpret_cast<const void*>(pt_attn_pair_heads_kernel<4>); break;
        case 8: kern = reinterpret_cast<const void*>(pt_attn_pair_heads_kernel<8>); break;
        default: return fail(PTT_EUNSUPPORTED, "ptt_pt_attn_pair_f32: heads=%d (1, 2, 4, 8 are instantiated)", d->heads);
    }
    int rc = set_lds_limit(kern, lds);
    if (rc) return rc;
    const dim3 grid((p.BN + 1) / 2);
    switch (heads) {
        case 1: hipLaunchKernelGGL((pt_attn_pair_kernel<512>), grid, dim3(256), lds, as_stream(stream), p); break;
        case 2: hipLaunchKernelGGL((pt_attn_pair_heads_kernel<2>), grid, dim3(256), lds, as_stream(stream), p); break;
        case 4: hipLaunchKernelGGL((pt_attn_pair_heads_kernel<4>), grid, dim3(256), lds, as_stream(stream), p); break;
        default: hipLaunchKernelGGL((pt_attn_pair_heads_kernel<8>), grid, dim3(256), lds, as_stream(stream), p); break;
    }
    return check_launch(heads == 1 ? "pt_attn_pair_kernel" : "pt_attn_pair_heads_kernel");
}
```

### ptt_amd/csrc/point_ops.hip

```cpp
#pragma clang fp contract(off)

#include <limits.h>
#include <stdlib.h>
#include "common.h"

namespace ptt {

__device__ __forceinline__ float sqdist3(float ax, float ay, float az, float bx, float by, float bz) {
    const float dx = ax - bx, dy = ay - by, dz = az - bz;
    return (dx * dx + dy * dy) + dz * dz;
}

__device__ __forceinline__ float knn_dist(float ax, float ay, float az, float bx, float by, float bz) {
    const float d = sqdist3(ax, ay, az, bx, by, bz);
    return d < __builtin_inff() ? d : 3.402823466e+38f;
}

__device__ __forceinline__ float lane_bcast(float v, int src_lane) {
    return __builtin_bit_cast(float, __builtin_amdgcn_readlane(__builtin_bit_cast(int, v), src_lane));
}

typedef float fps_f2 __attribute__((ext_vector_type(2)));


template <int T, int P, bool LX, int ABL = 0>
__global__ __launch_bounds__(T) void fps_kernel(const float* __restrict__ xyz, int N, int npoint,
                                               int32_t* __restrict__ idx_out) {
    constexpr int W = T / 64;
    const int b = blockIdx.x;
    const float* __restrict__ pts = xyz + (size_t)b * N * 3;
    int32_t* __restrict__ out = idx_out + (size_t)b * npoint;
    const int t = threadIdx.x;
    const int lane = t & 63;
    const int wv = t >> 6;

    extern __shared__ int sel_lds[];
    float* xyz_lds = reinterpret_cast<float*>(sel_lds + ((npoint + 3) & ~3));

    float px[P], py[P], pz[P], md[P];
#pragma unroll
    for (int i = 0; i < P; ++i) {
        const int k = t * P + i;
        float x = 0.f, y = 0.f, z = 0.f, m = -1.0f;
        if (k < N) {
            x = pts[3 * k + 0];
            y = pts[3 * k + 1];
            z = pts[3 * k + 2];
            const float mag = (x * x + y * y) + z * z;
            m = (mag > 1e-3f) ? 1e10f : -1.0f;
            if (LX) { xyz_lds[3 * k + 0] = x; xyz_lds[3 * k + 1] = y; xyz_lds[3 * k + 2] = z; }
        }
        px[i] = x; py[i] = y; pz[i] = z; md[i] = m;
    }

    __shared__ __attribute__((aligned(16))) float slots[2][W > 1 ? W : 1][8];

    float lx = pts[0], ly = pts[1], lz = pts[2];
    if (t == 0 && npoint > 0) sel_lds[0] = 0;
    if (LX) __syncthreads();

    for (int j = 1; j < npoint; ++j) {
        float best = -1.0f, bx = 0.f, by = 0.f, bz = 0.f;
        int besti = 0;
        if constexpr ((P % 2) == 0) {
            const fps_f2 lxv = {lx, lx}, lyv = {ly, ly}, lzv = {lz, lz};
#pragma unroll
            for (int i = 0; i < ((ABL & 32) ? 2 : P); i += 2) {
                const fps_f2 dx = fps_f2{px[i], px[i + 1]} - lxv, dy = fps_f2{py[i], py[i + 1]} - lyv,
                             dz = fps_f2{pz[i], pz[i + 1]} - lzv;
                const fps_f2 d = (dx * dx + dy * dy) + dz * dz;
#pragma unroll
                for (int h = 0; h < 2; ++h) {
                    const float m = fminf(md[i + h], d[h]);
                    md[i + h] = m;
                    const bool take = m > best;
                    best = take ? m : best;
                    besti = take ? t * P + i + h : besti;
                    if (!LX) {
                        bx = take ? px[i + h] : bx;
                        by = take ? py[i + h] : by;
                        bz = take ? pz[i + h] : bz;
                    }
                }
            }
        } else {
#pragma unroll
            for (int i = 0; i < P; ++i) {
                const float d = sqdist3(px[i], py[i], pz[i], lx, ly, lz);
                const float m = fminf(md[i], d);
                md[i] = m;
                const bool take = m > best;
                best = take ? m : best;
                besti = take ? t * P + i : besti;
                if (!LX) {
                    bx = take ? px[i] : bx;
                    by = take ? py[i] : by;
                    bz = take ? pz[i] : bz;
                }
            }
        }
        float wmax;
        if constexpr (ABL & 1) wmax = __builtin_amdgcn_readfirstlane(best); else wmax = wave_max_f32_fused(best);
        int src;
        if constexpr (ABL & 2) {
            src = (int)(__builtin_bit_cast(unsigned, wmax) & 63u);
        } else {
            const unsigned long long winners = __ballot(best == wmax);
            src = __ffsll((long long)winners) - 1;
            if constexpr (ABL & 1) src &= 63;
        }
        if constexpr (W == 1) {
            int widx = __builtin_amdgcn_readlane(besti, src);
            if (wmax < 0.f) widx = 0;
            if constexpr ((ABL & 8) != 0) {
                lx = (float)widx * 1e-3f; ly = lx; lz = lx;
            } else if constexpr (LX) {
                lx = xyz_lds[3 * widx + 0]; ly = xyz_lds[3 * widx + 1]; lz = xyz_lds[3 * widx + 2];
            } else if (wmax < 0.f) {
                lx = pts[0]; ly = pts[1]; lz = pts[2];
            } else {
                lx = lane_bcast(bx, src); ly = lane_bcast(by, src); lz = lane_bcast(bz, src);
            }
            if (lane == 0) sel_lds[j] = widx;
        } else if constexpr ((ABL & 4) != 0) {
            int gi = __builtin_amdgcn_readlane(besti, src);
            if (wmax < 0.f) gi = 0;
            if constexpr ((ABL & 8) != 0) { lx = (float)gi * 1e-3f; ly = lx; lz = lx; }
            else { lx = xyz_lds[3 * gi + 0]; ly = xyz_lds[3 * gi + 1]; lz = xyz_lds[3 * gi + 2]; }
            if (lane == 0 && wv == 0) sel_lds[j] = gi;
        } else {
            const int par = j & 1;
            if (lane == src) {
                if constexpr (LX) {
                    *reinterpret_cast<float2*>(slots[par][wv]) = make_float2(best, __builtin_bit_cast(float, besti));
                } else {
                    float4* s4 = reinterpret_cast<float4*>(slots[par][wv]);
                    s4[0] = make_float4(best, __builtin_bit_cast(float, besti), bx, by);
                    slots[par][wv][4] = bz;
                }
            }
            if constexpr ((ABL & 16) == 0) __syncthreads();
            float gd, gx = 0.f, gy = 0.f, gz = 0.f;
            int gi;
            if constexpr (W <= 4) {
                gd = -1.0f; gi = 0;
#pragma unroll
                for (int w = 0; w < W; ++w) {
                    if constexpr (LX) {
                        const float2 s2 = *reinterpret_cast<const float2*>(slots[par][w]);
                        const bool take = s2.x > gd;
                        gd = take ? s2.x : gd;
                        gi = take ? __builtin_bit_cast(int, s2.y) : gi;
                    } else {
                        const float4 s4 = *reinterpret_cast<const float4*>(slots[par][w]);
                        const float sz = slots[par][w][4];
                        const bool take = s4.x > gd;
                        gd = take ? s4.x : gd;
                        gi = take ? __builtin_bit_cast(int, s4.y) : gi;
                        gx = take ? s4.z : gx;
                        gy = take ? s4.w : gy;
                        gz = take ? sz : gz;
                    }
                }
            } else {
                if constexpr (LX) {
                    float2 s2 = make_float2(-1.0f, 0.f);
                    if (lane < W) s2 = *reinterpret_cast<const float2*>(slots[par][lane]);
                    gd = wave_max_f32_fused(s2.x);
                    const int sl = __ffsll((long long)__ballot(s2.x == gd)) - 1;
                    gi = __builtin_amdgcn_readlane(__builtin_bit_cast(int, s2.y), sl);
                } else {
                    float4 s4 = make_float4(-1.0f, 0.f, 0.f, 0.f);
                    float sz = 0.f;
                    if (lane < W) { s4 = *reinterpret_cast<const float4*>(slots[par][lane]); sz = slots[par][lane][4]; }
                    gd = wave_max_f32_fused(s4.x);
                    const int sl = __ffsll((long long)__ballot(s4.x == gd)) - 1;
                    gi = __builtin_amdgcn_readlane(__builtin_bit_cast(int, s4.y), sl);
                    gx = lane_bcast(s4.z, sl); gy = lane_bcast(s4.w, sl); gz = lane_bcast(sz, sl);
                }
            }
            if (gd < 0.f) gi = 0;
            if constexpr ((ABL & 16) != 0) gi &= 1023;
            if constexpr ((ABL & 8) != 0) {
                lx = (float)gi * 1e-3f; ly = lx; lz = lx;
            } else if constexpr (LX) {
                lx = xyz_lds[3 * gi + 0]; ly = xyz_lds[3 * gi + 1]; lz = xyz_lds[3 * gi + 2];
            } else {
                if (gd < 0.f) { gx = pts[0]; gy = pts[1]; gz = pts[2]; }
                lx = gx; ly = gy; lz = gz;
            }
            if (t == 0) sel_lds[j] = gi;
        }
    }
    __syncthreads();
    for (int j = t; j < npoint; j += T) out[j] = sel_lds[j];
}

template <int T, int P>
static int launch_fps(const float* xyz, int B, int N, int npoint, int32_t* idx, hipStream_t s) {
    const size_t sel_bytes = (size_t)((npoint + 3) & ~3) * sizeof(int);
    if (sel_bytes + (size_t)N * 12 + 1024 <= 65536 && !dev_switches().fps_plain) {
#ifdef PTT_DEV
        if (const char* e = getenv("PTT_FPS_ABL")) {
            const int abl = atoi(e);
#define PTT_FPS_ABL_CASE(A) if (abl == A) { hipLaunchKernelGGL((fps_kernel<T, P, true, A>), dim3(B), dim3(T), sel_bytes + (size_t)N * 12, s, xyz, N, npoint, idx); return check_launch("fps_kernel(abl)"); }
            PTT_FPS_ABL_CASE(1) PTT_FPS_ABL_CASE(2) PTT_FPS_ABL_CASE(3) PTT_FPS_ABL_CASE(4) PTT_FPS_ABL_CASE(8) PTT_FPS_ABL_CASE(12) PTT_FPS_ABL_CASE(15)
            PTT_FPS_ABL_CASE(16) PTT_FPS_ABL_CASE(32) PTT_FPS_ABL_CASE(47) PTT_FPS_ABL_CASE(7) PTT_FPS_ABL_CASE(24) PTT_FPS_ABL_CASE(40)
#undef PTT_FPS_ABL_CASE
        }
#endif
        hipLaunchKernelGGL((fps_kernel<T, P, true>), dim3(B), dim3(T), sel_bytes + (size_t)N * 12, s, xyz, N, npoint, idx);
        return check_launch("fps_kernel");
    }
    hipLaunchKernelGGL((fps_kernel<T, P, false>), dim3(B), dim3(T), sel_bytes, s, xyz, N, npoint, idx);
    return check_launch("fps_kernel");
}

template <int CPW>
__device__ __forceinline__ void ball_sweep(const float* __restrict__ pts, int N, float r2, int ns, const float (&cx)[CPW],
                                           const float (&cy)[CPW], const float (&cz)[CPW], int ncentres,
                                           int32_t* __restrict__ out0, int lane) {
    int cnt[CPW], first[CPW];
#pragma unroll
    for (int c = 0; c < CPW; ++c) { cnt[c] = (c < ncentres) ? 0 : ns; first[c] = 0; }
    for (int base = 0; base < N; base += 64) {
        const int k = base + lane;
        const bool in = k < N;
        float px = 0.f, py = 0.f, pz = 0.f;
        if (in) { px = pts[3 * k + 0]; py = pts[3 * k + 1]; pz = pts[3 * k + 2]; }
        bool active = false;
#pragma unroll
        for (int c = 0; c < CPW; ++c) {
            if (cnt[c] >= ns) continue;
            const float d = sqdist3(cx[c], cy[c], cz[c], px, py, pz);
            const bool hit = in && d < r2;
            const unsigned long long mask = __ballot(hit);
            if (mask != 0ull) {
                if (cnt[c] == 0) first[c] = base + (__ffsll((long long)mask) - 1);
                const int pos = cnt[c] + __popcll(mask & ((1ull << lane) - 1ull));
                if (hit && pos < ns) out0[(size_t)c * ns + pos] = k;
                cnt[c] += __popcll(mask);
            }
            active = active || cnt[c] < ns;
        }
        if (!active) break;
    }
#pragma unroll
    for (int c = 0; c < CPW; ++c) {
        if (c >= ncentres) break;
        const int fill = (cnt[c] > 0) ? first[c] : 0;
        for (int s = cnt[c] + lane; s < ns; s += 64) out0[(size_t)c * ns + s] = fill;
    }
}

template <int CPW>
__global__ __launch_bounds__(256) void ball_query_kernel(const float* __restrict__ new_xyz,
                                                         const float* __restrict__ xyz, int BM, int M, int N,
                                                         float r2, int ns, int32_t* __restrict__ idx_out) {
    const int centre = (blockIdx.x * 4 + (threadIdx.x >> 6)) * CPW;
    if (centre >= BM) return;
    const int lane = threadIdx.x & 63;
    const int b = centre / M;
    float cx[CPW], cy[CPW], cz[CPW];
    const int nc = min(CPW, BM - centre);
#pragma unroll
    for (int c = 0; c < CPW; ++c) {
        const int cc = centre + (c < nc ? c : 0);
        cx[c] = new_xyz[(size_t)cc * 3 + 0]; cy[c] = new_xyz[(size_t)cc * 3 + 1]; cz[c] = new_xyz[(size_t)cc * 3 + 2];
    }
    ball_sweep<CPW>(xyz + (size_t)b * N * 3, N, r2, ns, cx, cy, cz, nc, idx_out + (size_t)centre * ns, lane);
}

template <int CPW>
__global__ __launch_bounds__(256) void centres_ball_query_kernel(const float* __restrict__ xyz, const int32_t* __restrict__ sel,
                                                                 int BM, int M, int N, float r2, int ns,
                                                                 float* __restrict__ new_xyz, long long* __restrict__ idx64,
                                                                 int32_t* __restrict__ idx_out) {
    const int centre = (blockIdx.x * 4 + (threadIdx.x >> 6)) * CPW;
    if (centre >= BM) return;
    const int lane = threadIdx.x & 63;
    const int b = centre / M;
    const float* __restrict__ pts = xyz + (size_t)b * N * 3;
    float cx[CPW], cy[CPW], cz[CPW];
    const int nc = min(CPW, BM - centre);
#pragma unroll
    for (int c = 0; c < CPW; ++c) {
        const int cc = centre + (c < nc ? c : 0);
        const int n = sel ? sel[cc] : cc - b * M;
        cx[c] = pts[3 * n + 0]; cy[c] = pts[3 * n + 1]; cz[c] = pts[3 * n + 2];
        if (lane == 0 && c < nc) {
            new_xyz[(size_t)cc * 3 + 0] = cx[c]; new_xyz[(size_t)cc * 3 + 1] = cy[c]; new_xyz[(size_t)cc * 3 + 2] = cz[c];
            if (idx64) idx64[cc] = n;
        }
    }
    ball_sweep<CPW>(pts, N, r2, ns, cx, cy, cz, nc, idx_out + (size_t)centre * ns, lane);
}

__global__ void gather_kernel(const float* __restrict__ feat, const int32_t* __restrict__ idx, int C, int N, int M,
                              float* __restrict__ out, size_t total) {
    for (size_t e = (size_t)blockIdx.x * blockDim.x + threadIdx.x; e < total; e += (size_t)gridDim.x * blockDim.x) {
        const int j = (int)(e % M);
        const size_t bc = e / M;
        const int b = (int)(bc / C);
        out[e] = feat[bc * N + idx[(size_t)b * M + j]];
    }
}
__global__ void gather_grad_kernel(const float* __restrict__ go, const int32_t* __restrict__ idx, int C, int N, int M,
                                   float* __restrict__ gf, size_t total) {
    for (size_t e = (size_t)blockIdx.x * blockDim.x + threadIdx.x; e < total; e += (size_t)gridDim.x * blockDim.x) {
        const int j = (int)(e % M);
        const size_t bc = e / M;
        const int b = (int)(bc / C);
        atomicAdd(&gf[bc * N + idx[(size_t)b * M + j]], go[e]);
    }
}
__global__ void group_kernel(const float* __restrict__ feat, const int32_t* __restrict__ idx, int C, int N, int M,
                             int ns, float* __restrict__ out, size_t total) {
    const size_t mk = (size_t)M * ns;
    for (size_t e = (size_t)blockIdx.x * blockDim.x + threadIdx.x; e < total; e += (size_t)gridDim.x * blockDim.x) {
        const size_t jk = e % mk;
        const size_t bc = e / mk;
        const int b = (int)(bc / C);
        out[e] = feat[bc * N + idx[(size_t)b * mk + jk]];
    }
}
__global__ void group_grad_kernel(const float* __restrict__ go, const int32_t* __restrict__ idx, int C, int N, int M,
                                  int ns, float* __restrict__ gf, size_t total) {
    const size_t mk = (size_t)M * ns;
    for (size_t e = (size_t)blockIdx.x * blockDim.x + threadIdx.x; e < total; e += (size_t)gridDim.x * blockDim.x) {
        const size_t jk = e % mk;
        const size_t bc = e / mk;
        const int b = (int)(bc / C);
        atomicAdd(&gf[bc * N + idx[(size_t)b * mk + jk]], go[e]);
    }
}

__global__ __launch_bounds__(512) void group_grad_lds_kernel(const float* __restrict__ go, const int32_t* __restrict__ idx,
                                                             int C, int N, int M, int ns, int CC, int nchunks,
                                                             float* __restrict__ gf) {
    extern __shared__ float acc[];
    const int b = blockIdx.x / nchunks, c0 = (blockIdx.x % nchunks) * CC;
    const int cc = min(CC, C - c0), mk = M * ns;
    for (int i = threadIdx.x; i < cc * N; i += blockDim.x) acc[i] = 0.f;
    __syncthreads();
    const int32_t* ib = idx + (size_t)b * mk;
    for (int ci = 0; ci < cc; ++ci) {
        const float* g = go + ((size_t)b * C + c0 + ci) * mk;
        float* a = acc + ci * N;
        for (int jk = threadIdx.x; jk < mk; jk += blockDim.x) atomicAdd(&a[ib[jk]], g[jk]);
    }
    __syncthreads();
    float* o = gf + ((size_t)b * C + c0) * N;
    for (int i = threadIdx.x; i < cc * N; i += blockDim.x) o[i] = acc[i];
}

__global__ __launch_bounds__(1024) void scatter_csr_kernel(const int32_t* __restrict__ idx, int N, int E, int Epad,
                                                           int32_t* __restrict__ order, int32_t* __restrict__ start) {
    extern __shared__ unsigned keys[];
    const int b = blockIdx.x;
    const int32_t* ib = idx + (size_t)b * E;
    for (int e = threadIdx.x; e < Epad; e += blockDim.x)
        keys[e] = (e < E) ? (unsigned)ib[e] * (unsigned)Epad + (unsigned)e : 0xffffffffu;
    __syncthreads();
    for (int k = 2; k <= Epad; k <<= 1)
        for (int j = k >> 1; j > 0; j >>= 1) {
            for (int i = threadIdx.x; i < Epad; i += blockDim.x) {
                const int x = i ^ j;
                if (x > i) {
                    const unsigned a = keys[i], c = keys[x];
                    const bool up = (i & k) == 0;
                    if (up ? (a > c) : (a < c)) { keys[i] = c; keys[x] = a; }
                }
            }
            __syncthreads();
        }
    for (int e = threadIdx.x; e < E; e += blockDim.x) order[(size_t)b * E + e] = (int32_t)(keys[e] & (unsigned)(Epad - 1));
    for (int n = threadIdx.x; n <= N; n += blockDim.x) {
        const unsigned want = (unsigned)n * (unsigned)Epad;
        int lo = 0, hi = E;
        while (lo < hi) {
            const int mid = (lo + hi) >> 1;
            if (keys[mid] < want) lo = mid + 1; else hi = mid;
        }
        start[(size_t)b * (N + 1) + n] = (n == N) ? E : lo;
    }
}

__global__ __launch_bounds__(1024) void scatter_csr_count_kernel(const int32_t* __restrict__ idx, int N, int E, int32_t* __restrict__ order,
                                                                 int32_t* __restrict__ start) {
    extern __shared__ unsigned csr_smem[];
    unsigned* off = csr_smem;
    unsigned* binstart = csr_smem + 16 * N;
    unsigned* wave_tot = binstart + N + 1;
    const int b = blockIdx.x, t = threadIdx.x, lane = t & 63, w = t >> 6;
    const int32_t* ib = idx + (size_t)b * E;
    for (int i = t; i < 16 * N; i += 1024) off[i] = 0u;
    __syncthreads();
    const int per = ((E + 15) / 16 + 63) / 64 * 64;
    const int e0 = w * per, e1 = min(E, e0 + per);
    for (int e = e0 + lane; e < e1; e += 64) {
        const unsigned n = (unsigned)ib[e];
        if (n < (unsigned)N) atomicAdd(&off[w * N + n], 1u);
    }
    __syncthreads();
    unsigned tot[2];
#pragma unroll
    for (int u = 0; u < 2; ++u) {
        const int n = 2 * t + u;
        unsigned run = 0;
        if (n < N)
            for (int k = 0; k < 16; ++k) { const unsigned c = off[k * N + n]; off[k * N + n] = run; run += c; }
        tot[u] = run;
    }
    unsigned incl = tot[0] + tot[1];
    for (int d = 1; d < 64; d <<= 1) { const unsigned v = __shfl_up(incl, d, 64); if (lane >= d) incl += v; }
    if (lane == 63) wave_tot[w] = incl;
    __syncthreads();
    unsigned base = 0;
    for (int k = 0; k < w; ++k) base += wave_tot[k];
    const unsigned excl = base + incl - (tot[0] + tot[1]);
    if (2 * t < N) binstart[2 * t] = excl;
    if (2 * t + 1 < N) binstart[2 * t + 1] = excl + tot[0];
    if (t == 1023) binstart[N] = base + incl;
    __syncthreads();
    for (int n = t; n <= N; n += 1024) start[(size_t)b * (N + 1) + n] = (int32_t)binstart[n];
    for (int r0 = e0; r0 < e1; r0 += 64) {
        const int e = r0 + lane;
        const unsigned n = e < e1 ? (unsigned)ib[e] : 0xffffffffu;
        const bool valid = n < (unsigned)N;
        unsigned long long todo = __ballot(valid);
        unsigned rank = 0, cnt = 0;
        while (todo) {
            const int leader = __ffsll((long long)todo) - 1;
            const unsigned lb = (unsigned)__builtin_amdgcn_readlane((int)n, leader);
            const unsigned long long same = __ballot(valid && n == lb);
            if (valid && n == lb) {
                rank = (unsigned)__popcll(same & ((1ull << lane) - 1ull));
                cnt = (unsigned)__popcll(same);
            }
            todo &= ~same;
        }
        if (valid) {
            const unsigned o = off[w * N + n];
            order[(size_t)b * E + binstart[n] + o + rank] = e;
            __builtin_amdgcn_wave_barrier();
            if (rank + 1 == cnt) off[w * N + n] = o + cnt;
        }
    }
// ... 497 lines not shown
    const int32_t* __restrict__ slice = ws + (size_t)b * grid_slice_ints(N);
    const GridHead g = *reinterpret_cast<const GridHead*>(slice);
    const int32_t* __restrict__ cstart = slice + 8;
    const int32_t* __restrict__ cpts = slice + 8 + GRID_MAX_CELLS + 1;
    float cx, cy, cz;
    if (sel_mode) {
        const int n = sel ? sel[centre] : centre - b * M;
        cx = pts[3 * n]; cy = pts[3 * n + 1]; cz = pts[3 * n + 2];
        if (lane == 0) {
            new_xyz_out[(size_t)centre * 3] = cx; new_xyz_out[(size_t)centre * 3 + 1] = cy; new_xyz_out[(size_t)centre * 3 + 2] = cz;
            if (idx64) idx64[centre] = n;
        }
    } else {
        cx = centres[(size_t)centre * 3]; cy = centres[(size_t)centre * 3 + 1]; cz = centres[(size_t)centre * 3 + 2];
    }
    for (int w = lane; w < words; w += 64) bits[w] = 0u;
    __builtin_amdgcn_wave_barrier();
    const int ix = grid_cell_coord(cx, g.ox, g.inv, g.nx), iy = grid_cell_coord(cy, g.oy, g.inv, g.ny), iz = grid_cell_coord(cz, g.oz, g.inv, g.nz);
    for (int dz = -1; dz <= 1; ++dz) {
        const int z = iz + dz;
        if (z < 0 || z >= g.nz) continue;
        for (int dy = -1; dy <= 1; ++dy) {
            const int y = iy + dy;
            if (y < 0 || y >= g.ny) continue;
            const int x0 = ix > 0 ? ix - 1 : 0, x1 = ix + 1 < g.nx ? ix + 1 : g.nx - 1;
            const int c0 = (z * g.ny + y) * g.nx + x0;
            const int s0 = cstart[c0], s1 = cstart[c0 + (x1 - x0) + 1];
            for (int e = s0 + lane; e < s1; e += 64) {
                const int k = cpts[e];
                const float d = sqdist3(cx, cy, cz, pts[3 * k], pts[3 * k + 1], pts[3 * k + 2]);
                if (d < r2) atomicOr(&bits[k >> 5], 1u << (k & 31));
            }
        }
    }
    __builtin_amdgcn_wave_barrier();
    asm volatile("s_waitcnt lgkmcnt(0)" ::: "memory");
    int32_t* __restrict__ out = idx_out + (size_t)centre * ns;
    int cnt = 0, first = 0;
    for (int w0 = 0; w0 < words && cnt < ns; w0 += 64) {
        const int w = w0 + lane;
        unsigned v = w < words ? bits[w] : 0u;
        const int mine = __popc(v);
        int incl = mine;
#pragma unroll
        for (int off = 1; off < 64; off <<= 1) { const int u = __shfl_up(incl, off, 64); if (lane >= off) incl += u; }
        const int total = __shfl(incl, 63, 64);
        if (total == 0) continue;
        if (cnt == 0) {
            const unsigned long long any = __ballot(mine > 0);
            const int fl = __ffsll((long long)any) - 1;
            const unsigned fv = __shfl(v, fl, 64);
            first = ((w0 + fl) << 5) + (__ffs(fv) - 1);
        }
        int pos = cnt + incl - mine;
        while (v != 0u && pos < ns) {
            const int bit = __ffs(v) - 1;
            out[pos++] = (w << 5) + bit;
            v &= v - 1u;
        }
        cnt += total;
    }
    const int have = cnt < ns ? cnt : ns;
    const int fill = cnt > 0 ? first : 0;
    for (int s2 = have + lane; s2 < ns; s2 += 64) out[s2] = fill;
}

}

using namespace ptt;

extern "C" int ptt_fps_f32(const float* xyz, int B, int N, int npoint, int32_t* idx_out, ptt_stream_t stream) {
    if (B < 0 || N <= 0 || npoint < 0) return fail(PTT_EINVAL, "ptt_fps_f32: B=%d N=%d npoint=%d", B, N, npoint);
    if (B == 0 || npoint == 0) return PTT_OK;
    if (!xyz || !idx_out) return fail(PTT_EINVAL, "ptt_fps_f32: null pointer");
    if (npoint > 15360) return fail(PTT_EUNSUPPORTED, "ptt_fps_f32: npoint=%d exceeds the LDS index buffer (15360)", npoint);
    hipStream_t s = as_stream(stream);
    if (N <= 64) return launch_fps<64, 1>(xyz, B, N, npoint, idx_out, s);
    if (N <= 128) return launch_fps<64, 2>(xyz, B, N, npoint, idx_out, s);
    if (N <= 256) return launch_fps<64, 4>(xyz, B, N, npoint, idx_out, s);
    if (N <= 512) {
        if (const int T = dev_switches().fps_t) {
            if (T == 256) return launch_fps<256, 2>(xyz, B, N, npoint, idx_out, s);
            if (T == 128) return launch_fps<128, 4>(xyz, B, N, npoint, idx_out, s);
            if (T == 512) return launch_fps<512, 1>(xyz, B, N, npoint, idx_out, s);
        }
        return launch_fps<64, 8>(xyz, B, N, npoint, idx_out, s);
    }
    if (N <= 1024) {
        if (const int T = dev_switches().fps_t) {
            if (T == 64) return launch_fps<64, 16>(xyz, B, N, npoint, idx_out, s);
            if (T == 128) return launch_fps<128, 8>(xyz, B, N, npoint, idx_out, s);
            if (T == 512) return launch_fps<512, 2>(xyz, B, N, npoint, idx_out, s);
        }
        return launch_fps<256, 4>(xyz, B, N, npoint, idx_out, s);
    }
    if (N <= 2048) {
        if (const int T = dev_switches().fps_t) {
            if (T == 512) return launch_fps<512, 4>(xyz, B, N, npoint, idx_out, s);
            if (T == 1024) return launch_fps<1024, 2>(xyz, B, N, npoint, idx_out, s);
            if (T == 128) return launch_fps<128, 16>(xyz, B, N, npoint, idx_out, s);
        }
        return launch_fps<256, 8>(xyz, B, N, npoint, idx_out, s);
    }
    if (N <= 4096) return launch_fps<512, 8>(xyz, B, N, npoint, idx_out, s);
    if (N <= 8192) return launch_fps<1024, 8>(xyz, B, N, npoint, idx_out, s);
    if (N <= 16384) return launch_fps<1024, 16>(xyz, B, N, npoint, idx_out, s);
    return fail(PTT_EUNSUPPORTED, "ptt_fps_f32: N=%d exceeds the register-resident limit 16384 (use ptt_fps_ws_f32)", N);
}

extern "C" int ptt_spatial_order_f32(const float* xyz, int B, int N, int32_t* order, ptt_stream_t stream) {
    if (B < 0 || N <= 0) return fail(PTT_EINVAL, "ptt_spatial_order_f32: B=%d N=%d", B, N);
    if (B == 0) return PTT_OK;
    if (!xyz || !order) return fail(PTT_EINVAL, "ptt_spatial_order_f32: null pointer");
    if (N > 8192 || (long long)B * N > INT_MAX) return fail(PTT_EUNSUPPORTED, "ptt_spatial_order_f32: N=%d (at most 8192 points per cloud are sorted in LDS)", N);
    int P = 2;
    while (P < N) P <<= 1;
    const int lds = P * (int)sizeof(unsigned long long);
    if (int rc = set_lds_limit(reinterpret_cast<const void*>(spatial_order_kernel), lds)) return rc;
    hipLaunchKernelGGL(spatial_order_kernel, dim3(B), dim3(1024), lds, as_stream(stream), xyz, N, P, order);
    return check_launch("spatial_order_kernel");
}

extern "C" int ptt_fps_ws_f32(const float* xyz, int B, int N, int npoint, int32_t* idx_out, float* workspace, size_t workspace_elems,
                              ptt_stream_t stream) {
    if (B < 0 || N <= 0 || npoint < 0) return fail(PTT_EINVAL, "ptt_fps_ws_f32: B=%d N=%d npoint=%d", B, N, npoint);
    if (B == 0 || npoint == 0) return PTT_OK;
    if (!xyz || !idx_out) return fail(PTT_EINVAL, "ptt_fps_ws_f32: null pointer");
    if ((long long)N * 3 > INT_MAX) return fail(PTT_EUNSUPPORTED, "ptt_fps_ws_f32: N=%d", N);
    if (!workspace || workspace_elems < (size_t)B * N)
        return fail(PTT_EWORKSPACE, "ptt_fps_ws_f32: %zu floats of workspace needed", (size_t)B * N);
    hipLaunchKernelGGL(fps_ws_kernel, dim3(B), dim3(1024), 0, as_stream(stream), xyz, N, npoint, workspace, idx_out);
    return check_launch("fps_ws_kernel");
}

static int ball_cpw(int BM, int M) {
    const int force = dev_switches().ball_cpw;
    if (force == 1 || (M & 3) != 0) return 1;
    if (force == 8 && (M & 7) == 0) return 8;
    if (force == 4) return 4;
    return BM >= 4 * 256 * 8 ? 4 : 1;
}

extern "C" int ptt_ball_query_f32(const float* new_xyz, const float* xyz, int B, int M, int N, float radius,
                                  int nsample, int32_t* idx_out, ptt_stream_t stream) {
    if (B < 0 || M < 0 || N <= 0 || nsample <= 0)
        return fail(PTT_EINVAL, "ptt_ball_query_f32: B=%d M=%d N=%d nsample=%d", B, M, N, nsample);
    if (B == 0 || M == 0) return PTT_OK;
    if (!new_xyz || !xyz || !idx_out) return fail(PTT_EINVAL, "ptt_ball_query_f32: null pointer");
    const float r2 = radius * radius;
    const int BM = B * M;
    const int cpw = ball_cpw(BM, M);
    if (cpw == 8)
        hipLaunchKernelGGL((ball_query_kernel<8>), dim3((BM / 8 + 3) / 4), dim3(256), 0, as_stream(stream), new_xyz, xyz, BM, M,
                           N, r2, nsample, idx_out);
    else if (cpw == 4)
        hipLaunchKernelGGL((ball_query_kernel<4>), dim3((BM / 4 + 3) / 4), dim3(256), 0, as_stream(stream), new_xyz, xyz, BM, M,
                           N, r2, nsample, idx_out);
    else
        hipLaunchKernelGGL((ball_query_kernel<1>), dim3((BM + 3) / 4), dim3(256), 0, as_stream(stream), new_xyz, xyz, BM, M,
                           N, r2, nsample, idx_out);
    return check_launch("ball_query_kernel");
}

extern "C" int ptt_gather_f32(const float* feat, const int32_t* idx, int B, int C, int N, int M, float* out,
                              ptt_stream_t stream) {
    if (B < 0 || C < 0 || N <= 0 || M < 0) return fail(PTT_EINVAL, "ptt_gather_f32: bad sizes");
    const size_t total = (size_t)B * C * M;
    if (total == 0) return PTT_OK;
    if (!feat || !idx || !out) return fail(PTT_EINVAL, "ptt_gather_f32: null pointer");
    hipLaunchKernelGGL(gather_kernel, dim3(grid_for(total, 256)), dim3(256), 0, as_stream(stream), feat, idx, C, N, M,
                       out, total);
    return check_launch("gather_kernel");
}

extern "C" int ptt_select_centres_f32(const float* xyz, const int32_t* idx, int B, int N, int M, float* new_xyz,
                                      int64_t* idx64_out, ptt_stream_t stream) {
    if (B < 0 || N <= 0 || M < 0 || (!idx && M > N)) return fail(PTT_EINVAL, "ptt_select_centres_f32: B=%d N=%d M=%d", B, N, M);
    const size_t total = (size_t)B * M;
    if (total == 0) return PTT_OK;
    if (!xyz || !new_xyz) return fail(PTT_EINVAL, "ptt_select_centres_f32: null pointer");
    hipLaunchKernelGGL(select_centres_kernel, dim3(grid_for(total, 256)), dim3(256), 0, as_stream(stream), xyz, idx, N, M,
                       new_xyz, reinterpret_cast<long long*>(idx64_out), total);
    return check_launch("select_centres_kernel");
}

extern "C" int ptt_gather_grad_f32(const float* grad_out, const int32_t* idx, int B, int C, int N, int M,
                                   float* grad_feat, ptt_stream_t stream) {
    if (B < 0 || C < 0 || N <= 0 || M < 0) return fail(PTT_EINVAL, "ptt_gather_grad_f32: bad sizes");
    const size_t nout = (size_t)B * C * N;
    if (nout == 0) return PTT_OK;
    if (!grad_feat) return fail(PTT_EINVAL, "ptt_gather_grad_f32: null pointer");
    if (hipMemsetAsync(grad_feat, 0, nout * sizeof(float), as_stream(stream)) != hipSuccess)
        return check_launch("gather_grad memset");
    const size_t total = (size_t)B * C * M;
    if (total == 0) return PTT_OK;
    if (!grad_out || !idx) return fail(PTT_EINVAL, "ptt_gather_grad_f32: null pointer");
    hipLaunchKernelGGL(gather_grad_kernel, dim3(grid_for(total, 256)), dim3(256), 0, as_stream(stream), grad_out, idx,
                       C, N, M, grad_feat, total);
    return check_launch("gather_grad_kernel");
}

extern "C" int ptt_group_f32(const float* feat, const int32_t* idx, int B, int C, int N, int M, int ns, float* out,
                             ptt_stream_t stream) {
    if (B < 0 || C < 0 || N <= 0 || M < 0 || ns < 0) return fail(PTT_EINVAL, "ptt_group_f32: bad sizes");
    const size_t total = (size_t)B * C * M * ns;
    if (total == 0) return PTT_OK;
    if (!feat || !idx || !out) return fail(PTT_EINVAL, "ptt_group_f32: null pointer");
    hipLaunchKernelGGL(group_kernel, dim3(grid_for(total, 256)), dim3(256), 0, as_stream(stream), feat, idx, C, N, M,
                       ns, out, total);
    return check_launch("group_kernel");
}

extern "C" int ptt_centres_ball_query_f32(const float* xyz, const int32_t* sel, int B, int N, int M, float radius, int nsample,
                                          float* new_xyz, int64_t* idx64_out, int32_t* idx_out, ptt_stream_t stream) {
    if (B < 0 || M < 0 || N <= 0 || nsample <= 0 || (!sel && M > N))
        return fail(PTT_EINVAL, "ptt_centres_ball_query_f32: B=%d M=%d N=%d nsample=%d", B, M, N, nsample);
    if (B == 0 || M == 0) return PTT_OK;
    if (!xyz || !new_xyz || !idx_out) return fail(PTT_EINVAL, "ptt_centres_ball_query_f32: null pointer");
    const int BM = B * M;
    const int cpw = ball_cpw(BM, M);
    if (cpw == 8)
        hipLaunchKernelGGL((centres_ball_query_kernel<8>), dim3((BM / 8 + 3) / 4), dim3(256), 0, as_stream(stream), xyz, sel, BM,
                           M, N, radius * radius, nsample, new_xyz, reinterpret_cast<long long*>(idx64_out), idx_out);
    else if (cpw == 4)
        hipLaunchKernelGGL((centres_ball_query_kernel<4>), dim3((BM / 4 + 3) / 4), dim3(256), 0, as_stream(stream), xyz, sel, BM,
                           M, N, radius * radius, nsample, new_xyz, reinterpret_cast<long long*>(idx64_out), idx_out);
    else
        hipLaunchKernelGGL((centres_ball_query_kernel<1>), dim3((BM + 3) / 4), dim3(256), 0, as_stream(stream), xyz, sel, BM, M,
                           N, radius * radius, nsample, new_xyz, reinterpret_cast<long long*>(idx64_out), idx_out);
    return check_launch("centres_ball_query_kernel");
}


extern "C" size_t ptt_ball_query_grid_workspace(int B, int N) {
    if (B <= 0 || N <= 0) return 0;
    return (size_t)B * grid_slice_ints(N) * sizeof(int32_t);
}

static int ball_query_grid_launch(const char* who, const float* xyz, const float* centres, const int32_t* sel, int sel_mode, int B, int N, int M,
                                  float radius, int nsample, float* new_xyz, int64_t* idx64, int32_t* idx_out, void* ws, size_t ws_bytes,
                                  ptt_stream_t stream) {
    if (B < 0 || M < 0 || N <= 0 || nsample <= 0) return fail(PTT_EINVAL, "%s: B=%d M=%d N=%d nsample=%d", who, B, M, N, nsample);
    if (B == 0 || M == 0) return PTT_OK;
    if (N > 131072) return fail(PTT_EUNSUPPORTED, "%s: N=%d (the hit bitmap of a wave lives in LDS: at most 131072 points)", who, N);
    if (!ws || ws_bytes < ptt_ball_query_grid_workspace(B, N) || (reinterpret_cast<uintptr_t>(ws) & 15))
        return fail(PTT_EWORKSPACE, "%s: %zu bytes of 16-byte aligned workspace needed", who, ptt_ball_query_grid_workspace(B, N));
    hipStream_t s = as_stream(stream);
    hipLaunchKernelGGL(grid_build_kernel, dim3(B), dim3(1024), 0, s, xyz, N, radius, static_cast<int32_t*>(ws));
    const int BM = B * M, lds = 4 * ((N + 31) / 32) * (int)sizeof(unsigned);
    if (int rc = set_lds_limit(reinterpret_cast<const void*>(ball_query_grid_kernel), lds)) return rc;
    hipLaunchKernelGGL(ball_query_grid_kernel, dim3((BM + 3) / 4), dim3(256), lds, s, xyz, centres, sel, sel_mode, BM, M, N, radius * radius,
                       nsample, static_cast<const int32_t*>(ws), new_xyz, reinterpret_cast<long long*>(idx64), idx_out);
    return check_launch(who);
}

extern "C" int ptt_ball_query_grid_f32(const float* new_xyz, const float* xyz, int B, int M, int N, float radius, int nsample,
                                       int32_t* idx_out, void* workspace, size_t workspace_bytes, ptt_stream_t stream) {
    if ((B > 0 && M > 0) && (!new_xyz || !xyz || !idx_out)) return fail(PTT_EINVAL, "ptt_ball_query_grid_f32: null pointer");
    return ball_query_grid_launch("ptt_ball_query_grid_f32", xyz, new_xyz, nullptr, 0, B, N, M, radius, nsample, nullptr, nullptr, idx_out,
                                  workspace, workspace_bytes, stream);
}

extern "C" int ptt_centres_ball_query_grid_f32(const float* xyz, const int32_t* sel, int B, int N, int M, float radius, int nsample,
                                               float* new_xyz, int64_t* idx64_out, int32_t* idx_out, void* workspace,
                                               size_t workspace_bytes, ptt_stream_t stream) {
    if (!sel && M > N) return fail(PTT_EINVAL, "ptt_centres_ball_query_grid_f32: M=%d > N=%d without a selection", M, N);
    if ((B > 0 && M > 0) && (!xyz || !new_xyz || !idx_out)) return fail(PTT_EINVAL, "ptt_centres_ball_query_grid_f32: null pointer");
    return ball_query_grid_launch("ptt_centres_ball_query_grid_f32", xyz, nullptr, sel, 1, B, N, M, radius, nsample, new_xyz, idx64_out,
                                  idx_out, workspace, workspace_bytes, stream);
}

extern "C" int ptt_fps_ball_knn_f32(const float* xyz, int B, int N, int M, float radius, int nsample, int k, int32_t* inds,
                                    int64_t* inds64, float* new_xyz, int32_t* idx, int32_t* knn, float* rel, ptt_stream_t stream) {
    if (B < 0 || N <= 0 || M <= 0 || nsample <= 0 || k < 0) return fail(PTT_EINVAL, "ptt_fps_ball_knn_f32: B=%d N=%d M=%d nsample=%d k=%d", B, N, M, nsample, k);
    if (N > 256 || M > 128 || M > N || k > M)
        return fail(PTT_EUNSUPPORTED, "ptt_fps_ball_knn_f32: at most 256 points, 128 centres, k <= centres (N=%d M=%d k=%d)", N, M, k);
    if (B == 0) return PTT_OK;
    if (!xyz || !inds || !new_xyz || !idx || (k > 0 && !knn)) return fail(PTT_EINVAL, "ptt_fps_ball_knn_f32: null pointer");
    FbkParams p;
    p.xyz = xyz; p.B = B; p.N = N; p.M = M; p.ns = nsample; p.k = k; p.r2 = radius * radius;
    p.inds = inds; p.inds64 = reinterpret_cast<long long*>(inds64); p.new_xyz = new_xyz; p.idx = idx; p.knn = k > 0 ? knn : nullptr; p.rel = rel;
    hipLaunchKernelGGL(fps_ball_knn_kernel, dim3(B * ((M + 3) / 4)), dim3(256), 0, as_stream(stream), p);
    return check_launch("fps_ball_knn_kernel");
}

extern "C" int ptt_point_jobs_f32(const ptt_point_job* jobs, int n_jobs, ptt_stream_t stream) {
    if (!jobs || n_jobs < 1 || n_jobs > PTT_POINT_JOBS_MAX) return fail(PTT_EINVAL, "ptt_point_jobs_f32: n_jobs=%d (1..%d)", n_jobs, PTT_POINT_JOBS_MAX);
    PointJobs P;
    P.n = 0;
    int waves = 0;
    for (int i = 0; i < n_jobs; ++i) {
        const ptt_point_job& j = jobs[i];
        if (j.B < 0 || j.Nraw <= 0 || j.Npts <= 0 || j.M < 0 || j.nsample <= 0 || (j.kind != 0 && j.kind != 1))
            return fail(PTT_EINVAL, "ptt_point_jobs_f32: job %d: kind=%d B=%d Nraw=%d Npts=%d M=%d nsample=%d", i, j.kind, j.B, j.Nraw, j.Npts, j.M, j.nsample);
        if (j.B == 0 || j.M == 0) continue;
        if (!j.xyz || !j.idx_out || (j.kind == 0 && !j.new_xyz)) return fail(PTT_EINVAL, "ptt_point_jobs_f32: job %d: null pointer", i);
        if ((j.centre_sel || j.point_sel) && (j.sel_ld < j.M || (j.point_sel && j.sel_ld < j.Npts)))
            return fail(PTT_EINVAL, "ptt_point_jobs_f32: job %d: sel_ld=%d", i, j.sel_ld);
        if ((!j.centre_sel && j.M > j.Nraw) || (!j.point_sel && j.Npts > j.Nraw))
            return fail(PTT_EINVAL, "ptt_point_jobs_f32: job %d: identity selection past the cloud", i);
        if (j.kind == 1 && (j.Npts > 128 || j.M != j.Npts || j.nsample > j.Npts))
            return fail(PTT_EUNSUPPORTED, "ptt_point_jobs_f32: job %d: the kNN job takes at most 128 points, every point a query (Npts=%d M=%d k=%d)", i, j.Npts, j.M, j.nsample);
        PointJobDev& D = P.j[P.n++];
        D.xyz = j.xyz; D.csel = j.centre_sel; D.psel = j.point_sel; D.new_xyz = j.new_xyz;
        D.idx64 = reinterpret_cast<long long*>(j.idx64_out); D.idx_out = j.idx_out; D.rel_out = j.rel_out;
        D.kind = j.kind; D.sel_ld = j.sel_ld; D.B = j.B; D.Nraw = j.Nraw; D.Npts = j.Npts; D.M = j.M; D.ns = j.nsample;
        D.r2 = j.radius * j.radius;
        D.wave0 = waves;
        waves += (j.B * j.M + 3) / 4 * 4;
    }
    if (P.n == 0) return PTT_OK;
    hipLaunchKernelGGL(point_jobs_kernel, dim3(waves / 4), dim3(256), 0, as_stream(stream), P);
    return check_launch("point_jobs_kernel");
}

extern "C" int ptt_group_grad_f32(const float* grad_out, const int32_t* idx, int B, int C, int N, int M, int ns,
                                  float* grad_feat, ptt_stream_t stream) {
    if (B < 0 || C < 0 || N <= 0 || M < 0 || ns < 0) return fail(PTT_EINVAL, "ptt_group_grad_f32: bad sizes");
    const size_t nout = (size_t)B * C * N;
    if (nout == 0) return PTT_OK;
    if (!grad_feat) return fail(PTT_EINVAL, "ptt_group_grad_f32: null pointer");
    const size_t total = (size_t)B * C * M * ns;
    if (total > 0 && (!grad_out || !idx)) return fail(PTT_EINVAL, "ptt_group_grad_f32: null pointer");
    if (total > 0 && N <= 16384 && !dev_switches().group_grad_global) {
        int CC = 65536 / (4 * N);
        if (CC > 16) CC = 16;
        if (CC > C) CC = C;
        const int nchunks = (C + CC - 1) / CC;
        hipLaunchKernelGGL(group_grad_lds_kernel, dim3(B * nchunks), dim3(512), (size_t)CC * N * sizeof(float),
                           as_stream(stream), grad_out, idx, C, N, M, ns, CC, nchunks, grad_feat);
        return check_launch("group_grad_lds_kernel");
    }
    if (hipMemsetAsync(grad_feat, 0, nout * sizeof(float), as_stream(stream)) != hipSuccess)
        return check_launch("group_grad memset");
    if (total == 0) return PTT_OK;
    hipLaunchKernelGGL(group_grad_kernel, dim3(grid_for(total, 256)), dim3(256), 0, as_stream(stream), grad_out, idx,
                       C, N, M, ns, grad_feat, total);
    return check_launch("group_grad_kernel");
}

extern "C" size_t ptt_scatter_add_det_workspace(int B, int N, int E) {
    if (B <= 0 || N <= 0 || E <= 0) return 0;
    return ((size_t)B * E + (size_t)B * (N + 1)) * sizeof(int32_t);
}

extern "C" int ptt_scatter_add_det_f32(const float* src, const int32_t* idx, int B, int C, int N, int E, float* out,
                                       void* workspace, size_t workspace_bytes, ptt_stream_t stream) {
    if (B < 0 || C < 0 || N <= 0 || E < 0) return fail(PTT_EINVAL, "ptt_scatter_add_det_f32: bad sizes");
    const size_t nout = (size_t)B * C * N;
    if (nout == 0) return PTT_OK;
    if (!out) return fail(PTT_EINVAL, "ptt_scatter_add_det_f32: null pointer");
    hipStream_t s = as_stream(stream);
    if (E == 0) {
        if (hipMemsetAsync(out, 0, nout * sizeof(float), s) != hipSuccess) return check_launch("scatter_add_det memset");
        return PTT_OK;
    }
    if (!src || !idx) return fail(PTT_EINVAL, "ptt_scatter_add_det_f32: null pointer");
    if (E > 16384 || (unsigned long long)N * 16384ull > 0xffffffffull)
        return fail(PTT_EUNSUPPORTED, "ptt_scatter_add_det_f32: E=%d N=%d (at most 16384 entries per cloud)", E, N);
    const size_t need = ptt_scatter_add_det_workspace(B, N, E);
    if (!workspace || workspace_bytes < need)
        return fail(PTT_EWORKSPACE, "ptt_scatter_add_det_f32: workspace of %zu bytes, %zu needed", workspace_bytes, need);
    int32_t* order = static_cast<int32_t*>(workspace);
    int32_t* start = order + (size_t)B * E;
    int rc = launch_scatter_csr(idx, B, N, E, order, start, s);
    if (rc) return rc;
    const int CC = 8, nchunks = (C + CC - 1) / CC;
    const size_t lds = (size_t)E * (sizeof(float) + sizeof(int));
    if ((rc = set_lds_limit(reinterpret_cast<const void*>(scatter_add_det_kernel), (int)lds))) return rc;
    hipLaunchKernelGGL(scatter_add_det_kernel, dim3(B * nchunks), dim3(512), lds, s, src, order, start, C, N, E, CC, nchunks,
                       out);
    return check_launch("scatter_add_det_kernel");
}

extern "C" int ptt_scatter_csr_i32(const int32_t* idx, int B, int N, int E, int32_t* order, int32_t* start, ptt_stream_t stream) {
    if (B < 0 || N <= 0 || E <= 0) return fail(PTT_EINVAL, "ptt_scatter_csr_i32: B=%d N=%d E=%d", B, N, E);
    if (B == 0) return PTT_OK;
    if (!idx || !order || !start) return fail(PTT_EINVAL, "ptt_scatter_csr_i32: null pointer");
    if (N > 2048 && (E > 16384 || (unsigned long long)N * 16384ull > 0xffffffffull))
        return fail(PTT_EUNSUPPORTED, "ptt_scatter_csr_i32: E=%d N=%d (more than 2048 bins: at most 16384 entries per cloud)", E, N);
    return launch_scatter_csr(idx, B, N, E, order, start, as_stream(stream));
}

// ... 25 lines not shown
```

### ptt_amd/models/backbones_3d/pointnet2/pointnet2_modules.py

```python
import os
from typing import List

import torch
import torch.nn as nn
import torch.nn.functional as F

from .... import ops, train_ops
from ....param_cache import (DropsCachesOnModeChange, FoldedLayer, ParamCache, conv_bn_tensors, fold_conv_bn,
                             index_table)
from . import pointnet2_utils
from . import pytorch_utils as pt_utils

STREAM_COMPACT_MIN_BALLS = 2048
STREAM_COMPACT_MAX_POINTS = 1024


class PointnetSAModuleVotes(DropsCachesOnModeChange, nn.Module):
    def __init__(self, *, mlp: List[int], radius: float = None, nsample: int = None, bn: bool = True,
                 use_xyz: bool = True, normalize_xyz: bool = False, sample_uniformly: bool = False,
                 sample_method='fps'):
        super().__init__()
        self.radius = radius
        self.nsample = nsample
        self.mlp_module = None
        self.use_xyz = use_xyz
        self.normalize_xyz = normalize_xyz
        self.sample_uniformly = sample_uniformly
        self.grouper = pointnet2_utils.QueryAndGroup(radius, nsample, use_xyz=use_xyz, ret_grouped_xyz=True,
                                                     normalize_xyz=normalize_xyz, sample_uniformly=sample_uniformly,
                                                     ret_unique_cnt=False)
        mlp_spec = mlp
        if use_xyz and len(mlp_spec) > 0:
            mlp_spec[0] += 3
        self.mlp_module = pt_utils.SharedMLP(mlp_spec, bn=bn)
        self.sample_method = sample_method
        self._fused_cache = ParamCache()
        self.centres_knn_k = 0
        self.centres_knn = None

    def _sample(self, xyz, features, npoint):
        if self.sample_method == 'fps':
            return pointnet2_utils.furthest_point_sample(xyz, npoint)
        if self.sample_method in ('rs', 'sequence'):
            return index_table(xyz.size(0), npoint, xyz.device, torch.int32)
        if self.sample_method == 'ffps':
            raise NotImplementedError("sample_method 'ffps' needs furthest_point_sampling_with_dist, which the "
                                      "reference's extension never provided (tools/cfgs/kitti_models/ptt.yaml:42)")
        raise NotImplementedError(self.sample_method)

    def _fusable(self, xyz, features):
        if self.training or not xyz.is_cuda:
            return False
        name = 'PointnetSAModuleVotes(nsample=%s, mlp=%s)' % (self.nsample, [u.conv.weight.shape[0] for u in self.mlp_module
                                                                              if hasattr(u, 'conv')])
        if ops.autograd_recording(self, xyz, features):
            return ops.note_unfused(name, 'autograd is recording (wrap inference in torch.no_grad())')
        if self.sample_uniformly or self.nsample not in (16, 32, 64):
            return ops.note_unfused(name, 'nsample must be 16, 32 or 64 and sample_uniformly off')
        if xyz.dtype != torch.float32 or (features is not None and features.dtype != torch.float32):
            return ops.note_unfused(name, 'inputs must be float32')
        if len(self.mlp_module) > 4:
            return ops.note_unfused(name, 'more than 4 SharedMLP layers')
        for unit in self.mlp_module:
            conv = getattr(unit, 'conv', None)
            if conv is None or conv.kernel_size != (1, 1) or conv.weight.shape[0] % 32 != 0 or conv.weight.shape[0] > 256:
                return ops.note_unfused(name, 'layer widths must be multiples of 32, at most 256, 1x1 convolutions')
            if list(unit._modules.keys())[0] != 'conv':
                return ops.note_unfused(name, 'pre-activation units')
        return True

    def _fused_params(self, device):
        return self._fused_cache.get(conv_bn_tensors(self.mlp_module), device, self._fold)

    def _fold(self):
        layers, scale0 = [], None
        for li, unit in enumerate(self.mlp_module):
            w = unit.conv.weight
            cout, cin = w.shape[0], w.shape[1]
            rot = 3 if (li == 0 and self.use_xyz and cin > 3) else 0
            scale, shift = fold_conv_bn(unit)
            scale0 = scale if li == 0 else scale0
            wq = w if scale is None else w * scale.view(-1, 1, 1, 1)
            layers.append(FoldedLayer(ops.pack_weight(wq, rot), None, shift, cin, cout, hasattr(unit, 'activation')))
        hoist = None
        w0 = self.mlp_module[0].conv.weight
        if (self.use_xyz and len(layers) >= 2 and w0.shape[1] > 3 and layers[0].cout <= 256
                and os.environ.get('PTT_SA_HOIST', '1') != '0'):
            w2 = w0.reshape(w0.shape[0], w0.shape[1]).float()
            wx = w2[:, 0:3] if scale0 is None else w2[:, 0:3] * scale0[:, None]
            wf = w2[:, 3:] if scale0 is None else w2[:, 3:] * scale0[:, None]
            hoist = (ops.pack_weight(wf.contiguous()), wx.t().contiguous(), layers[0].cout, layers[0].relu)
        return layers, hoist

    def forward(self, xyz: torch.Tensor, features: torch.Tensor, npoint: int, inds: torch.Tensor = None, pre=None,
                compact: bool = False):
        self.centres_knn = None
        if self._fusable(xyz, features):
            return self._forward_fused(xyz, features, npoint, inds, pre, compact)
        return self._forward_train(xyz, features, npoint, inds)

    def _forward_fused(self, xyz, features, npoint, inds, pre, compact):
        if (pre is None and inds is None and self.sample_method == 'fps' and xyz.shape[1] <= 256 and npoint <= 128
                and xyz.shape[0] * npoint * self.nsample <= ops.ONE_FRAME_MAX_SA_ROWS and self.centres_knn_k <= npoint):
            xyz = xyz.contiguous()
            inds, inds64, new_xyz, idx, self.centres_knn = ops.fps_ball_knn(xyz, npoint, self.radius, self.nsample, self.centres_knn_k)
            pre = (new_xyz, idx, inds64)
        prefix = inds is None and self.sample_method in ('rs', 'sequence')
        if pre is not None:
            pass
        elif prefix:
            inds64 = index_table(xyz.size(0), npoint, xyz.device, torch.int64)
        elif inds is None:
            inds = self._sample(xyz, features, npoint)
        else:
            assert inds.shape[1] == npoint
            inds = inds.to(torch.int32)

        xyz = xyz.contiguous()
        if pre is not None:
            new_xyz, idx, inds64 = pre
        elif prefix:
            new_xyz, _, idx = ops.centres_ball_query(xyz, None, npoint, self.radius, self.nsample)
        else:
            new_xyz, inds64, idx = ops.centres_ball_query(xyz, inds.contiguous(), npoint, self.radius, self.nsample)
        layers, hoist = self._fused_params(xyz.device)
        if hoist is not None and features is not None:
            wf_packed, wx, c0, relu0 = hoist
            rows = features.transpose(1, 2)
            uniform = rows.stride(2) == 1 and rows.stride(0) == rows.shape[1] * rows.stride(1)
            term = ops.linear(rows if uniform else rows.contiguous(), wf_packed, c0, None, layers[0].shift, relu=False)
            B, M, ns = xyz.shape[0], npoint, self.nsample
            if (B * M * ns <= ops.ONE_FRAME_MAX_SA_ROWS and ns in (16, 32) and len(layers) == 3 and c0 % 4 == 0 and c0 >= 192):
                L1, L2 = layers[1], layers[2]
                h = torch.empty((B * M * ns, L1.cout), dtype=torch.float32, device=xyz.device)
                ops.row_jobs([pt_utils.layer_job(L1, prologue=3, x=term, idx=idx, xyz=xyz, centres=new_xyz, wx=wx,
                                                 radius=self.radius, ns=ns, M=M, N=xyz.shape[1], normalize_xyz=self.normalize_xyz,
                                                 pro_relu=relu0, out=h)])
                pooled = torch.empty((B, M, L2.cout), dtype=torch.float32, device=xyz.device)
                ops.row_jobs([pt_utils.layer_job(L2, x=h, epilogue=2, ns=ns, M=M, out=pooled)])
                return new_xyz, pooled.transpose(1, 2), inds64
            new_features = ops.sa_fused_forward(xyz, new_xyz, idx, None, layers[1:], self.radius, True,
                                                self.normalize_xyz, point_major_out=True, l0=(term, wx, relu0),
                                                compact=(bool(compact) and B * M >= STREAM_COMPACT_MIN_BALLS
                                                         and xyz.shape[1] <= STREAM_COMPACT_MAX_POINTS))
        else:
            new_features = ops.sa_fused_forward(xyz, new_xyz, idx, features, layers, self.radius,
                                                self.use_xyz, self.normalize_xyz, point_major_out=True,
                                                compact=features is None)
        return new_xyz, new_features, inds64

    def _forward_train(self, xyz, features, npoint, inds):
        if inds is None:
            inds = self._sample(xyz, features, npoint)
        else:
            assert inds.shape[1] == npoint
            inds = inds.to(torch.int32)
        hoist = (self.use_xyz and not self.sample_uniformly and self.nsample * npoint <= 16384
                 and train_ops.usable(self.mlp_module, xyz if features is None else features)
                 and self.mlp_module[0].conv.weight.shape[0] % 4 == 0)
        if hoist and not xyz.requires_grad and inds.dtype == torch.int32:
            new_xyz, inds64, idx = ops.centres_ball_query(xyz.contiguous(), inds.contiguous(), npoint, self.radius, self.nsample)
            y = train_ops.sa_level_hoisted(xyz, new_xyz, features, idx, self.mlp_module, self.radius, self.normalize_xyz)
            return new_xyz, y, inds64
        xyz_flipped = xyz.transpose(1, 2).contiguous()
        new_xyz = pointnet2_utils.gather_operation(xyz_flipped, inds).transpose(1, 2).contiguous()
        if hoist and features is not None:
            idx = pointnet2_utils.ball_query(self.radius, self.nsample, xyz, new_xyz)
            y = train_ops.sa_level_hoisted(xyz, new_xyz, features, idx, self.mlp_module, self.radius, self.normalize_xyz)
            return new_xyz, y, inds.to(torch.int64)
        grouped_features, grouped_xyz = self.grouper(xyz, new_xyz, features)
        if train_ops.usable(self.mlp_module, grouped_features):
            return new_xyz, train_ops.shared_mlp_pool(grouped_features, self.mlp_module, pool_dim=3), inds.to(torch.int64)
        y = self.mlp_module(grouped_features)
        y = y.max(dim=3)[0]
        return new_xyz, y, inds.to(torch.int64)
```

### ptt_amd/models/backbones_3d/pointnet2_backbone.py

```python
from typing import List

import torch
import torch.nn as nn

from ... import graph_policy, ops, train_ops
from ...param_cache import ParamCache, index_table
from .pointnet2 import pointnet2_modules


class PointNet2BackboneLight(nn.Module):
    def __init__(self, model_cfg, input_channels, **kwargs):
        super().__init__()
        self.model_cfg = model_cfg
        input_channels -= 3
        self.num_points_each_layer = []
        self.SA_modules = nn.ModuleList()
        sa = self.model_cfg.SA_CONFIG
        for k in range(len(sa.RADIUS)):
            mlps = list(sa.MLPS[k])
            if k == 0:
                mlps[0] = input_channels
            self.SA_modules.append(pointnet2_modules.PointnetSAModuleVotes(
                radius=sa.RADIUS[k], nsample=sa.NSAMPLE[k], mlp=mlps,
                use_xyz=sa.get('USE_XYZ', True), normalize_xyz=sa.get('NORMALIZE_XYZ', True),
                sample_method=sa.SAMPLE_METHOD[k]))
        self.cov_final = nn.Conv1d(256, 256, kernel_size=1)
        self.num_point_features = sa.MLPS[-1][-1]
        self._cov_cache = ParamCache()
        self.seed_knn = 16
        self.overlap_branches = True
        self._side_stream = None

    @staticmethod
    def _break_up_pc(pc):
        xyz = pc[..., 0:3].contiguous()
        features = pc[..., 3:].contiguous() if pc.size(-1) > 3 else None
        return xyz, features

    def _cov_final(self, features):
        if not features.is_cuda:
            return self.cov_final(features)
        if self.training:
            if features.dtype != torch.float32:
                return self.cov_final(features)
            return train_ops.rows_linear(self.cov_final, features.transpose(1, 2)).transpose(1, 2)
        if ops.autograd_recording(self.cov_final, features) or features.dtype != torch.float32:
            ops.note_unfused('PointNet2BackboneLight.cov_final', 'autograd is recording or input is not float32')
            return self.cov_final(features)
        w, b = self.cov_final.weight, self.cov_final.bias
        wpacked, bias = self._cov_cache.get([w, b], w.device, lambda: (ops.pack_weight(w), b.detach().float().contiguous()))
        rows = features.transpose(1, 2)
        out = ops.linear(rows, wpacked, w.shape[0], None, bias)
        return out.transpose(1, 2)

    def branch_forward(self, pts, npoints: List, inds0=None, want_knn=0, compact_levels=()):
        xyz, features = self._break_up_pc(pts)
        sa = self.model_cfg.SA_CONFIG
        one_frame = (not self.training and xyz.is_cuda and features is None and len(self.SA_modules) == 3
                     and xyz.shape[0] * npoints[0] <= 4 * ops.ONE_FRAME_MAX_POINTS
                     and self.SA_modules[0].sample_method == 'fps'
                     and all(m.sample_method in ('rs', 'sequence') for m in self.SA_modules[1:])
                     and npoints[0] >= npoints[1] >= npoints[2] and (not want_knn or npoints[2] <= 128)
                     and all(m._fusable(xyz, None) for m in self.SA_modules[:1]))
        knn = None
        if one_frame:
            from .pointnet2 import pointnet2_utils
            xyz = xyz.contiguous()
            if inds0 is None:
                inds0 = pointnet2_utils.furthest_point_sample(xyz, npoints[0])
            inds0 = inds0.to(torch.int32).contiguous()
            levels, inds64, knn = ops.sa_levels_point_jobs(xyz, inds0, list(npoints), list(sa.RADIUS), list(sa.NSAMPLE),
                                                           knn_k=want_knn)
            seq = [None] + [index_table(xyz.size(0), n, xyz.device, torch.int64) for n in npoints[1:3]]
            xyz, features, inds0 = self.SA_modules[0](xyz=xyz, features=features, npoint=npoints[0], inds=inds0,
                                                      pre=(levels[0][0], levels[0][1], inds64))
            xyz, features, inds1 = self.SA_modules[1](xyz=xyz, features=features, npoint=npoints[1],
                                                      pre=(levels[1][0], levels[1][1], seq[1]))
            xyz, features, inds2 = self.SA_modules[2](xyz=xyz, features=features, npoint=npoints[2],
                                                      pre=(levels[2][0], levels[2][1], seq[2]))
        else:
            xyz, features, inds0 = self.SA_modules[0](xyz=xyz, features=features, npoint=npoints[0], inds=inds0)
            xyz, features, inds1 = self.SA_modules[1](xyz=xyz, features=features, npoint=npoints[1], compact=1 in compact_levels)
            xyz, features, inds2 = self.SA_modules[2](xyz=xyz, features=features, npoint=npoints[2], compact=2 in compact_levels)
        point_features = self._cov_final(features)
        assert inds1.dtype == inds2.dtype == torch.int64, 'index type must be int64, not {}'.format(inds2.dtype)
        if all(m.sample_method in ('rs', 'sequence') for m in self.SA_modules[1:]) and inds0.shape[1] >= npoints[2]:
            inds = inds0[:, :npoints[2]]
        else:
            inds = inds0.gather(1, inds1).gather(1, inds2)
        if want_knn:
            return xyz, point_features, inds, knn
        return xyz, point_features, inds

    def sample(self, search_points, template_points):
        from .pointnet2 import pointnet2_utils
        sa = self.model_cfg.SA_CONFIG
        assert sa.SAMPLE_METHOD[0] == 'fps'
        return (pointnet2_utils.furthest_point_sample(search_points[..., 0:3].contiguous(), sa.NPOINTS_SEARCH[0]),
                pointnet2_utils.furthest_point_sample(template_points[..., 0:3].contiguous(), sa.NPOINTS_TEMPLATE[0]))

    def forward_branches(self, search_points, template_points, inds=None):
        sa = self.model_cfg.SA_CONFIG
        i_s, i_t = inds if inds is not None else (None, None)
        last = (len(self.SA_modules) - 1,) if (search_points.is_cuda and not self.training) else ()
        if not (self.overlap_branches and search_points.is_cuda and not self.training):
            r = self.branch_forward(search_points, sa.NPOINTS_SEARCH, i_s, want_knn=self.seed_knn, compact_levels=last)
            t_seeds, t_feats, t_inds = self.branch_forward(template_points, sa.NPOINTS_TEMPLATE, i_t)
        else:
            if self._side_stream is None or self._side_stream.device != search_points.device:
                self._side_stream = torch.cuda.Stream(device=search_points.device)
            main = torch.cuda.current_stream(search_points.device)
            side = graph_policy.branch(main, self._side_stream)
            with torch.cuda.stream(side):
                t_seeds, t_feats, t_inds = self.branch_forward(template_points, sa.NPOINTS_TEMPLATE, i_t)
            r = self.branch_forward(search_points, sa.NPOINTS_SEARCH, i_s, want_knn=self.seed_knn, compact_levels=last)
            graph_policy.join(main, side)
            if side is not main:
                for t in (t_seeds, t_feats, t_inds, template_points):
                    t.record_stream(main)
        s_seeds, s_feats, s_inds = r[:3]
        s_knn = r[3] if len(r) > 3 else None
        out = {'search_seeds': s_seeds, 'search_feats': s_feats, 'search_inds': s_inds,
               'template_seeds': t_seeds, 'template_feats': t_feats, 'template_inds': t_inds}
        if s_knn is not None:
            out['search_seeds_knn'] = s_knn
        return out

    def forward(self, batch_dict):
        batch_dict.update(self.forward_branches(batch_dict['search_points'], batch_dict['template_points'],
                                                batch_dict.pop('fps_inds', None)))
        batch_dict.pop('search_points')
        batch_dict.pop('template_points')
        return batch_dict
```

### ptt_amd/models/trackers/tracker3d_template.py

```python
import os

import torch
import torch.nn as nn

from .. import backbones_3d, similarity_modules, voting_heads


class Tracker3DTemplate(nn.Module):
    def __init__(self, model_cfg, num_class, dataset):
        super().__init__()
        self.model_cfg = model_cfg
        self.num_class = num_class
        self.dataset = dataset
        self.training = dataset.training
        self.class_names = dataset.class_names
        self.register_buffer('global_step', torch.LongTensor(1).zero_())
        self.module_topology = ['backbone_3d', 'similarity_module', 'centroid_voting_head', 'box_voting_head']

    @property
    def mode(self):
        return 'TRAIN' if self.training else 'TEST'

    def forward(self, **kwargs):
        raise NotImplementedError

    def update_global_step(self):
        self.global_step += 1

    def build_networks(self):
        info = {
            'module_list': [],
            'num_rawpoint_features': self.dataset.point_feature_encoder.num_point_features,
            'num_point_features': self.dataset.point_feature_encoder.num_point_features,
            'grid_size': self.dataset.grid_size,
            'point_cloud_range': self.dataset.point_cloud_range,
            'voxel_size': self.dataset.voxel_size,
        }
        for name in self.module_topology:
            module, info = getattr(self, 'build_%s' % name)(model_info_dict=info)
            self.add_module(name, module)
        return info['module_list']

    def build_backbone_3d(self, model_info_dict):
        cfg = self.model_cfg.get('BACKBONE_3D', None)
        if cfg is None:
            return None, model_info_dict
        module = backbones_3d.__all__[cfg.NAME](
            model_cfg=cfg, input_channels=model_info_dict['num_point_features'],
            grid_size=model_info_dict['grid_size'], voxel_size=model_info_dict['voxel_size'],
            point_cloud_range=model_info_dict['point_cloud_range'])
        model_info_dict['module_list'].append(module)
        model_info_dict['num_point_features'] = module.num_point_features
        return module, model_info_dict

    def build_similarity_module(self, model_info_dict):
        cfg = self.model_cfg.get('SIMILARITY_MODULE', None)
        if cfg is None:
            return None, model_info_dict
        module = similarity_modules.__all__[cfg.NAME](model_cfg=cfg)
        model_info_dict['module_list'].append(module)
        return module, model_info_dict

    def _build_head(self, key, model_info_dict):
        cfg = self.model_cfg.get(key, None)
        if cfg is None:
            return None, model_info_dict
        module = voting_heads.__all__[cfg.NAME](
            model_cfg=cfg, input_channels=model_info_dict['num_point_features'], num_class=1)
        model_info_dict['module_list'].append(module)
        return module, model_info_dict

    def build_centroid_voting_head(self, model_info_dict):
        return self._build_head('CENTROID_HEAD', model_info_dict)

    def build_box_voting_head(self, model_info_dict):
        return self._build_head('BOX_HEAD', model_info_dict)

    def post_processing(self, batch_dict):
        pass

    def load_params_from_file(self, filename, logger, to_cpu=False):
        if not os.path.isfile(filename):
            raise FileNotFoundError(filename)
        logger.info('==> Loading parameters from checkpoint %s to %s' % (filename, 'CPU' if to_cpu else 'GPU'))
        checkpoint = torch.load(filename, map_location=torch.device('cpu') if to_cpu else None)
        disk = checkpoint['model_state']
        if 'version' in checkpoint:
            logger.info('==> Checkpoint trained from version: %s' % checkpoint['version'])
        own = self.state_dict()
        taken = {k: v for k, v in disk.items() if k in own and own[k].shape == v.shape}
        own.update(taken)
        self.load_state_dict(own)
        for k in own:
            if k not in taken:
                logger.info('Not updated weight %s: %s' % (k, str(own[k].shape)))
        logger.info('==> Done (loaded %d/%d)' % (len(taken), len(own)))

    def load_params_with_optimizer(self, filename, to_cpu=False, optimizer=None, logger=None):
        if not os.path.isfile(filename):
            raise FileNotFoundError(filename)
        logger.info('==> Loading parameters from checkpoint %s to %s' % (filename, 'CPU' if to_cpu else 'GPU'))
        loc = torch.device('cpu') if to_cpu else None
        checkpoint = torch.load(filename, map_location=loc)
        self.load_state_dict(checkpoint['model_state'])
        if optimizer is not None:
            if checkpoint.get('optimizer_state') is not None:
                optimizer.load_state_dict(checkpoint['optimizer_state'])
            else:
                stem, ext = os.path.splitext(filename)
                side = '%s_optim%s' % (stem, ext)
                if os.path.exists(side):
                    optimizer.load_state_dict(torch.load(side, map_location=loc)['optimizer_state'])
        if 'version' in checkpoint:
            print('==> Checkpoint trained from version: %s' % checkpoint['version'])
        logger.info('==> Done')
        return checkpoint.get('it', 0.0), checkpoint.get('epoch', -1)
```

### ptt_amd/ops.py

```python
import contextlib
import ctypes
import os

import torch

from . import _lib
from ._lib import AttnDesc, SaDesc, SaLayer, XcorrDesc


def _stream():
    return ctypes.c_void_p(torch.cuda.current_stream().cuda_stream)


_timing = None


def start_kernel_timing(names):
    global _timing
    _timing = {n: [] for n in names}


def stop_kernel_timing():
    global _timing
    t, _timing = _timing, None
# ... 44 lines not shown


def publish_params(device, replaced=True):
    global param_generation
    if replaced:
        param_generation += 1
    if device.type == 'cuda' and not torch.cuda.is_current_stream_capturing():
        torch.cuda.current_stream(device).synchronize()


def drop_params():
    global param_generation
    param_generation += 1


class StateWatch(object):

    def __init__(self, module):
        self.tensors = list(module.parameters()) + list(module.buffers())
        self.mark()

    def _key(self):
        return list(map(torch.Tensor.data_ptr, self.tensors)), [t._version for t in self.tensors]

    def mark(self):
        self.generation, self.key = param_generation, self._key()

    def changed(self):
        return param_generation != self.generation or self._key() != self.key


def require_finite(*tensors):
    bad = [k for k, t in enumerate(tensors) if t is not None and t.is_floating_point() and not bool(torch.isfinite(t).all())]
    if bad:
        raise ValueError("non-finite values in tensor(s) %s" % ", ".join("#%d %s" % (k, tuple(tensors[k].shape)) for k in bad))


def _chk(t, name, dtype, ndim=None):
    if not isinstance(t, torch.Tensor):
        raise TypeError("%s must be a torch.Tensor" % name)
    if not t.is_cuda:
        raise RuntimeError("%s must be a device (HIP) tensor — CPU tensors are not supported" % name)
    if t.dtype != dtype:
        raise RuntimeError("%s must be %s, got %s" % (name, dtype, t.dtype))
    if not t.is_contiguous():
        raise RuntimeError("%s must be contiguous" % name)
    if ndim is not None and t.dim() != ndim:
        raise RuntimeError("%s must have %d dimensions, got %s" % (name, ndim, tuple(t.shape)))
    return t


def _ptr(t):
    return ctypes.c_void_p(t.data_ptr()) if t is not None else ctypes.c_void_p(0)


_UNTIMED = contextlib.nullcontext()


def _launch(name, device, *args, timed=None):
    with torch.cuda.device(device), (_timed(timed) if timed else _UNTIMED):
        rc = getattr(_lib.lib(), name)(*args, _stream())
    if rc:
        _lib.check(rc, name)


def _host(name, *args):
    return getattr(_lib.lib(), name)(*args)


def _host_checked(name, *args):
    _lib.check(_host(name, *args), name)


def _workspace(query, device, *dims):
    ws = _ws(_host(query, *dims), device)
    return ws, (_ptr(ws), ws.numel() * 8)


FPS_RESIDENT_MAX_N, FPS_RESIDENT_MAX_NPOINT = 16384, 15360


def furthest_point_sampling(xyz, npoint):
    _chk(xyz, "xyz", torch.float32, 3)
    B, N, _ = xyz.shape
    out = torch.empty((B, int(npoint)), dtype=torch.int32, device=xyz.device)
    if N <= FPS_RESIDENT_MAX_N and int(npoint) <= FPS_RESIDENT_MAX_NPOINT:
        _launch("ptt_fps_f32", xyz.device, _ptr(xyz), B, N, int(npoint), _ptr(out), timed='ptt_fps_f32')
    else:
        ws = torch.empty((B * N,), dtype=torch.float32, device=xyz.device)
        _launch("ptt_fps_ws_f32", xyz.device, _ptr(xyz), B, N, int(npoint), _ptr(out), _ptr(ws), ws.numel(), timed='ptt_fps_f32')
    return out


def gather_points(features, idx):
    _chk(features, "features", torch.float32, 3)
    _chk(idx, "idx", torch.int32, 2)
    B, C, N = features.shape
    M = idx.shape[1]
    out = torch.empty((B, C, M), dtype=torch.float32, device=features.device)
    _launch("ptt_gather_f32", features.device, _ptr(features), _ptr(idx), B, C, N, M, _ptr(out))
    return out


def scatter_add_det(src, idx, N):
    B, C, E = src.shape
    out = torch.empty((B, C, int(N)), dtype=torch.float32, device=src.device)
    nbytes = _host("ptt_scatter_add_det_workspace", B, int(N), E)
    ws = torch.empty((max(1, (nbytes + 3) // 4),), dtype=torch.int32, device=src.device)
    _launch("ptt_scatter_add_det_f32", src.device, _ptr(src), _ptr(idx), B, C, int(N), E, _ptr(out), _ptr(ws), ws.numel() * 4)
    return out


_ATOMIC_GRADS = os.environ.get("PTT_ATOMIC_GRADS", "0")


def set_atomic_grads(on):
    global _ATOMIC_GRADS
    prev = _ATOMIC_GRADS == "1"
    _ATOMIC_GRADS = "1" if on else "0"
    return prev


def _det_grads(entries, N):
    if int(N) * 16384 > 0xffffffff:
        return False
    return entries <= 16384 and _ATOMIC_GRADS != "1"


def gather_points_grad(grad_out, idx, N):
    _chk(grad_out, "grad_out", torch.float32, 3)
    _chk(idx, "idx", torch.int32, 2)
    B, C, M = grad_out.shape
    if M > 0 and _det_grads(M, N):
        return scatter_add_det(grad_out, idx, N)
    out = torch.empty((B, C, int(N)), dtype=torch.float32, device=grad_out.device)
    _launch("ptt_gather_grad_f32", grad_out.device, _ptr(grad_out), _ptr(idx), B, C, int(N), M, _ptr(out))
    return out


def select_centres(xyz, idx, npoint, want_idx64=True):
    _chk(xyz, "xyz", torch.float32, 3)
    B, N, _ = xyz.shape
    if idx is not None:
        _chk(idx, "idx", torch.int32, 2)
    new_xyz = torch.empty((B, int(npoint), 3), dtype=torch.float32, device=xyz.device)
    idx64 = torch.empty((B, int(npoint)), dtype=torch.int64, device=xyz.device) if (want_idx64 and idx is not None) else None
    _launch("ptt_select_centres_f32", xyz.device, _ptr(xyz), _ptr(idx), B, N, int(npoint), _ptr(new_xyz), _ptr(idx64))
    return new_xyz, idx64


GRID_BALL_QUERY_MIN_POINTS = 4096


def ball_query(new_xyz, xyz, radius, nsample):
    _chk(new_xyz, "new_xyz", torch.float32, 3)
    _chk(xyz, "xyz", torch.float32, 3)
    B, M, _ = new_xyz.shape
    N = xyz.shape[1]
    out = torch.empty((B, M, int(nsample)), dtype=torch.int32, device=xyz.device)
    if GRID_BALL_QUERY_MIN_POINTS <= N <= 131072:
        ws, ws_arg = _workspace("ptt_ball_query_grid_workspace", xyz.device, B, N)
        _launch("ptt_ball_query_grid_f32", xyz.device, _ptr(new_xyz), _ptr(xyz), B, M, N, float(radius), int(nsample), _ptr(out), *ws_arg,
                timed='ptt_ball_query_f32')
    else:
        _launch("ptt_ball_query_f32", xyz.device, _ptr(new_xyz), _ptr(xyz), B, M, N, float(radius), int(nsample), _ptr(out),
                timed='ptt_ball_query_f32')
    return out


def centres_ball_query(xyz, sel, npoint, radius, nsample, want_idx64=True):
    _chk(xyz, "xyz", torch.float32, 3)
    B, N, _ = xyz.shape
    if sel is not None:
        _chk(sel, "sel", torch.int32, 2)
    M = int(npoint)
    new_xyz = torch.empty((B, M, 3), dtype=torch.float32, device=xyz.device)
    idx64 = torch.empty((B, M), dtype=torch.int64, device=xyz.device) if (want_idx64 and sel is not None) else None
    idx = torch.empty((B, M, int(nsample)), dtype=torch.int32, device=xyz.device)
    if GRID_BALL_QUERY_MIN_POINTS <= N <= 131072:
        ws, ws_arg = _workspace("ptt_ball_query_grid_workspace", xyz.device, B, N)
        _launch("ptt_centres_ball_query_grid_f32", xyz.device, _ptr(xyz), _ptr(sel), B, N, M, float(radius), int(nsample), _ptr(new_xyz), _ptr(idx64),
                _ptr(idx), *ws_arg, timed='ptt_ball_query_f32')
    else:
        _launch("ptt_centres_ball_query_f32", xyz.device, _ptr(xyz), _ptr(sel), B, N, M, float(radius), int(nsample), _ptr(new_xyz), _ptr(idx64),
                _ptr(idx), timed='ptt_ball_query_f32')
    return new_xyz, idx64, idx


def group_points(features, idx):
    _chk(features, "features", torch.float32, 3)
    _chk(idx, "idx", torch.int32, 3)
    B, C, N = features.shape
    _, M, ns = idx.shape
    out = torch.empty((B, C, M, ns), dtype=torch.float32, device=features.device)
    _launch("ptt_group_f32", features.device, _ptr(features), _ptr(idx), B, C, N, M, ns, _ptr(out))
    return out


def group_points_grad(grad_out, idx, N):
    _chk(grad_out, "grad_out", torch.float32, 4)
    _chk(idx, "idx", torch.int32, 3)
    B, C, M, ns = grad_out.shape
    if M * ns > 0 and _det_grads(M * ns, N):
        return scatter_add_det(grad_out.view(B, C, M * ns), idx.view(B, M * ns), N)
    out = torch.empty((B, C, int(N)), dtype=torch.float32, device=grad_out.device)
    _launch("ptt_group_grad_f32", grad_out.device, _ptr(grad_out), _ptr(idx), B, C, int(N), M, ns, _ptr(out))
    return out


def _unreached(name):
    def fn(*a, **k):
        raise NotImplementedError("%s is never reached by PTT (SURVEY.md §2.1) and is not provided" % name)
    fn.__name__ = name
    return fn


three_nn = _unreached("three_nn")
three_interpolate = _unreached("three_interpolate")
three_interpolate_grad = _unreached("three_interpolate_grad")
furthest_point_sampling_with_dist = _unreached("furthest_point_sampling_with_dist")


def knn(xyz, k, want_rel=False):
    _chk(xyz, "xyz", torch.float32, 3)
    B, N, _ = xyz.shape
    out = torch.empty((B, N, int(k)), dtype=torch.int32, device=xyz.device)
    rel = torch.empty((B, N, int(k), 3), dtype=torch.float32, device=xyz.device) if want_rel else None
    _launch("ptt_knn_rel_f32", xyz.device, _ptr(xyz), B, N, int(k), _ptr(out), _ptr(rel), timed='ptt_knn_f32')
    return (out, rel) if want_rel else out


def pack_weight(weight, rot=0):
    w = weight.detach()
    w = w.reshape(w.shape[0], -1).contiguous().float()
    _chk(w, "weight", torch.float32, 2)
    Cout, K = w.shape
    n = _host("ptt_packed_weight_elems", Cout, K)
    out = torch.empty((n,), dtype=torch.float32, device=w.device)
    _launch("ptt_pack_weight_rot_f32", w.device, _ptr(w), Cout, K, int(rot), _ptr(out))
    return out


ONE_FRAME_MAX_SA_ROWS = 4096
ROW_JOB_MAX_ROWS = 1024
ONE_FRAME_MAX_POINTS = int(os.environ.get("PTT_PT_PER_LAYER_MAX", "512"))


def linear(x, wpacked, cout, scale=None, shift=None, relu=False, residual=None, out=None):
    if not x.is_cuda or x.dtype != torch.float32:
        raise RuntimeError("x must be a float32 device tensor")
    K = x.shape[-1]
    x2 = x.reshape(-1, K)
    if x2.stride(1) != 1:
        x2 = x2.contiguous()
    rows = x2.shape[0]
    if out is None:
        out = torch.empty(tuple(x.shape[:-1]) + (int(cout),), dtype=torch.float32, device=x.device)
    o2 = out.view(-1, int(cout))
    r2 = None
    if residual is not None:
        r2 = residual.reshape(-1, int(cout))
        if r2.stride(1) != 1:
            r2 = r2.contiguous()
    if (scale is None and (rows > 8192 or (rows >= 6144 and int(cout) == 256)) and x2.data_ptr() % 16 == 0 and o2.is_contiguous()
            and _host("ptt_rows_gemm_supported", rows, K, int(cout), x2.stride(0), int(cout))):
        _launch("ptt_rows_gemm_f32", x.device, _ptr(x2), rows, K, x2.stride(0), None, None, _ptr(wpacked), int(cout), _ptr(shift), 1 if relu else 0,
                _ptr(r2), r2.stride(0) if r2 is not None else int(cout), _ptr(o2), int(cout), None, 0, timed='ptt_linear_f32')
        return out
    if rows <= ROW_JOB_MAX_ROWS and 192 <= K <= 1024 and o2.stride(1) == 1:
        row_jobs([row_job(wpacked, cout, x=x2, scale=scale, shift=shift, act=1 if relu else 0, res=r2, out=o2)])
        return out
    _launch("ptt_linear_f32", x.device, _ptr(x2), rows, K, x2.stride(0) if rows > 1 else K, _ptr(wpacked), int(cout), _ptr(scale), _ptr(shift),
            1 if relu else 0, _ptr(r2), (r2.stride(0) if (r2 is not None and rows > 1) else int(cout)), _ptr(o2),
            o2.stride(0) if rows > 1 else int(cout), timed='ptt_linear_f32')
    return out


def sa_fused_forward(xyz, new_xyz, idx, features, layers, radius, use_xyz=True, normalize_xyz=False,
                     point_major_out=True, l0=None, compact=False):
    _chk(xyz, "xyz", torch.float32, 3)
    _chk(new_xyz, "new_xyz", torch.float32, 3)
    _chk(idx, "idx", torch.int32, 3)
    B, N, _ = xyz.shape
    _, M, ns = idx.shape
    d = SaDesc()
    d.xyz, d.new_xyz, d.idx = xyz.data_ptr(), new_xyz.data_ptr(), idx.data_ptr()
    if features is not None:
        if not features.is_cuda or features.dtype != torch.float32 or features.dim() != 3:
            raise RuntimeError("features must be a (B,C,N) float32 device tensor")
        d.feat = features.data_ptr()
        d.feat_sb, d.feat_sc, d.feat_sn = features.stride()
        d.C = features.shape[1]
    else:
        d.feat, d.C = None, 0
    cout = layers[-1][4]
    if point_major_out:
        store = torch.empty((B, M, cout), dtype=torch.float32, device=xyz.device)
        out = store.transpose(1, 2)
    else:
        out = torch.empty((B, cout, M), dtype=torch.float32, device=xyz.device)
    d.out = out.data_ptr()
    d.out_sb, d.out_sc, d.out_sm = out.stride()
    d.B, d.N, d.M, d.nsample = B, N, M, ns
    d.radius, d.use_xyz, d.normalize_xyz = float(radius), int(bool(use_xyz)), int(bool(normalize_xyz))
    d.n_layers = len(layers)
    for i, (wp, sc, sh, cin, co, relu) in enumerate(layers):
        L = d.layers[i]
        L.Wpacked = wp.data_ptr()
        L.scale = sc.data_ptr() if sc is not None else None
        L.shift = sh.data_ptr() if sh is not None else None
        L.Cin, L.Cout, L.relu = int(cin), int(co), int(bool(relu))
    if l0 is not None:
        term, wx, l0_relu = l0
        if features is not None:
            raise RuntimeError("with a hoisted layer 0 the point features are already inside l0[0]")
        _chk(term, "l0 point term", torch.float32, 3)
        _chk(wx, "l0 xyz weight", torch.float32, 2)
        if term.shape[0] != B or term.shape[1] != N or wx.shape[0] != 3 or wx.shape[1] != term.shape[2]:
            raise RuntimeError("l0 point term must be (B,N,C0) and the xyz weight (3,C0)")
        d.l0_point_term, d.l0_xyz_weight = term.data_ptr(), wx.data_ptr()
        d.l0_channels, d.l0_relu = term.shape[2], int(bool(l0_relu))
    if isinstance(compact, torch.Tensor):
        if not compact.is_cuda or compact.device != xyz.device or not compact.is_contiguous():
            raise RuntimeError("compact workspace must be a contiguous tensor on %s" % xyz.device)
        d.compact_ws, d.compact_ws_bytes = compact.data_ptr(), compact.numel() * compact.element_size()
    elif compact:
        ws, (_, d.compact_ws_bytes) = _workspace("ptt_sa_compact_workspace", xyz.device, B, M)
        d.compact_ws = ws.data_ptr()
    _launch("ptt_sa_fused_fwd_f32", xyz.device, ctypes.byref(d), timed='ptt_sa_fused_fwd_f32')
    return out


def cosine_map(search_feats, templ_feats, eps=1e-8):
    for t_, n_ in ((search_feats, "search_feats"), (templ_feats, "templ_feats")):
        if not isinstance(t_, torch.Tensor) or not t_.is_cuda or t_.dtype != torch.float32 or t_.dim() != 3:
            raise RuntimeError("%s must be a (B,C,N) float32 device tensor" % n_)
    if search_feats.shape[:2] != templ_feats.shape[:2] or search_feats.device != templ_feats.device:
        raise RuntimeError("search_feats and templ_feats must share batch size, channel count and device")
    B, C, Ns = search_feats.shape
    Nt = templ_feats.shape[2]
    out = torch.empty((B, Ns, Nt), dtype=torch.float32, device=search_feats.device)
    ssb, ssc, ssn = search_feats.stride()
    tsb, tsc, tsn = templ_feats.stride()
    _launch("ptt_cosine_map_f32", out.device, search_feats.data_ptr(), ssb, ssn, ssc, templ_feats.data_ptr(), tsb, tsn, tsc, B, Ns, Nt, C, float(eps),
            out.data_ptr(), timed='ptt_cosine_map_f32')
    return out


def rows_mlp(x, layers, residual=None):
    if not x.is_cuda or x.dtype != torch.float32 or x.stride(-1) != 1:
        raise RuntimeError("rows_mlp: x must be a float32 device tensor with contiguous rows")
    K = x.shape[-1]
    x2 = x.reshape(-1, K)
    rows = x2.shape[0]
    cout = int(layers[-1][4])
    out = torch.empty((rows, cout), dtype=torch.float32, device=x.device)
    res2 = None
    if residual is not None:
        res2 = residual.reshape(-1, cout)
        _chk(res2 if res2.is_contiguous() else res2.contiguous(), "residual", torch.float32, 2)
        res2 = res2 if res2.stride(1) == 1 else res2.contiguous()
    arr = (SaLayer * len(layers))()
    for i, (wp, sc, sh, cin, co, relu) in enumerate(layers):
        arr[i].Wpacked = wp.data_ptr()
        arr[i].scale = sc.data_ptr() if sc is not None else None
        arr[i].shift = sh.data_ptr() if sh is not None else None
        arr[i].Cin, arr[i].Cout, arr[i].relu = int(cin), int(co), int(bool(relu))
    _launch("ptt_rows_mlp_f32", x.device, _ptr(x2), rows, K, x2.stride(0), arr, len(layers), _ptr(res2), res2.stride(0) if res2 is not None else 0,
            _ptr(out), cout, timed='ptt_rows_mlp_f32')
    return out.view(*x.shape[:-1], cout)


def xcorr_fused(search_feats, templ_feats, P, w_sim, scale0, shift0, layers, eps=1e-8, want_sim=False, cos_t=None, split=False):
    for t_, n_ in ((search_feats, "search_feats"), (templ_feats, "templ_feats")):
        if not t_.is_cuda or t_.dtype != torch.float32 or t_.dim() != 3:
            raise RuntimeError("%s must be a (B,C,N) float32 device tensor" % n_)
    _chk(P, "P", torch.float32, 3)
    _chk(w_sim, "w_sim", torch.float32, 1)
    B, C, Ns = search_feats.shape
    Nt = templ_feats.shape[2]
    C0 = P.shape[2]
    if Nt <= 0 or Nt % 64:
        raise RuntimeError("xcorr_fused: Nt=%d (ptt_xcorr_fused_fwd_f32 walks the template seeds in chunks of 64)" % Nt)
    if P.shape[0] != B or P.shape[1] != Nt or w_sim.shape[0] != C0 or templ_feats.shape[:2] != search_feats.shape[:2]:
        raise RuntimeError("xcorr_fused: inconsistent shapes")
    cout = layers[-1][4]
    split = (split and not want_sim and search_feats.stride(1) == 1 and templ_feats.stride(1) == 1 and C % 4 == 0 and (B * Ns) % 8 == 0
             and all(st % 4 == 0 for st in (search_feats.stride(0), search_feats.stride(2), templ_feats.stride(0), templ_feats.stride(2)))
             and search_feats.data_ptr() % 16 == 0 and templ_feats.data_ptr() % 16 == 0 and bool(layers[-1][5]))
    if not split:
        if cos_t is None:
            cos_t = cosine_map(search_feats, templ_feats, eps=eps)
        _chk(cos_t, "cos_t", torch.float32, 3)
        if tuple(cos_t.shape) != (B, Ns, Nt):
            raise RuntimeError("xcorr_fused: cos_t must be (B,Ns,Nt)")
    store = torch.empty(((2, B, Ns, cout) if split else (B, Ns, cout)), dtype=torch.float32, device=P.device)
    out = store.transpose(-1, -2)
    sim = torch.empty((B, Nt, Ns), dtype=torch.float32, device=P.device) if want_sim else None
    d = XcorrDesc()
    if split:
        d.split, d.out_sh = 1, store.stride(0)
        d.search_feat, d.templ_feat = search_feats.data_ptr(), templ_feats.data_ptr()
        d.s_sb, d.s_sn, d.t_sb, d.t_sn = search_feats.stride(0), search_feats.stride(2), templ_feats.stride(0), templ_feats.stride(2)
        d.C, d.eps = int(C), float(eps)
    else:
        d.cos_t = cos_t.data_ptr()
    d.P, d.w_sim = P.data_ptr(), w_sim.data_ptr()
    d.scale0 = scale0.data_ptr() if scale0 is not None else None
    d.shift0 = shift0.data_ptr() if shift0 is not None else None
    d.out = out.data_ptr()
    d.out_sb, d.out_sc, d.out_sn = out.stride()[-3:]
    d.sim_out = sim.data_ptr() if sim is not None else None
    d.B, d.Ns, d.Nt, d.C0 = B, Ns, Nt, C0
    d.n_layers = len(layers)
    for i, (wp, sc, sh, cin, co, relu) in enumerate(layers):
        L = d.layers[i]
        L.Wpacked = wp.data_ptr()
        L.scale = sc.data_ptr() if sc is not None else None
        L.shift = sh.data_ptr() if sh is not None else None
        L.Cin, L.Cout, L.relu = int(cin), int(co), int(bool(relu))
    _launch("ptt_xcorr_fused_fwd_f32", P.device, ctypes.byref(d), timed='ptt_xcorr_fused_fwd_f32')
    return out, sim


def pack_delta0(weight, bias):
    return pack_weight(torch.cat([weight.detach().float().reshape(weight.shape[0], 3),
                                  bias.detach().float().reshape(-1, 1)], dim=1).contiguous())


def spatial_order(xyz):
    _chk(xyz, "xyz", torch.float32, 3)
    B, N, _ = xyz.shape
    order = torch.empty((B, N), dtype=torch.int32, device=xyz.device)
    _launch("ptt_spatial_order_f32", xyz.device, _ptr(xyz), B, N, _ptr(order))
    return order


def pt_attn_pair(xyz, knn_idx, qkv, wd1p, wd2p, bd2, wg1p, bg1, wg2p, bg2, d_model, want_attn=True, rel=None, order=None,
                 heads=1):
    _chk(xyz, "xyz", torch.float32, 3)
    _chk(knn_idx, "knn_idx", torch.int32, 3)
    _chk(qkv, "qkv", torch.float32, 3)
    B, N, _ = xyz.shape
    k = knn_idx.shape[2]
    D = int(d_model)
    res = torch.empty((B, N, D), dtype=torch.float32, device=xyz.device)
    ashape = (B, N, k, D) if heads == 1 else (B * heads, N, k, D // heads)
    attn = torch.empty(ashape, dtype=torch.float32, device=xyz.device) if want_attn else None
    d = AttnDesc()
    d.xyz, d.knn, d.qkv = xyz.data_ptr(), knn_idx.data_ptr(), qkv.data_ptr()
    d.rel = rel.data_ptr() if rel is not None else None
    d.Wd1p, d.Wd2p, d.bd2 = wd1p.data_ptr(), wd2p.data_ptr(), bd2.data_ptr()
    d.Wg1p, d.bg1, d.Wg2p, d.bg2 = wg1p.data_ptr(), bg1.data_ptr(), wg2p.data_ptr(), bg2.data_ptr()
    d.res = res.data_ptr()
    d.attn = attn.data_ptr() if attn is not None else None
    d.B, d.N, d.k, d.D, d.heads = B, N, k, D, int(heads)
    if order is not None:
        _chk(order, "order", torch.int32, 2)
        if tuple(order.shape) != (B, N):
            raise ValueError("order: (B,N) int32 expected")
        d.order = order.data_ptr()
    _launch("ptt_pt_attn_pair_f32", xyz.device, ctypes.byref(d), timed='ptt_pt_attn_pair_f32')
    return res, attn


def layernorm(x, weight, bias, eps, residual=None, out=None):
    if not x.is_cuda or x.dtype != torch.float32:
        raise RuntimeError("x must be a float32 device tensor")
    C = x.shape[-1]
    x2 = x.reshape(-1, C)
    if x2.stride(1) != 1:
        x2 = x2.contiguous()
    if out is None:
        out = torch.empty(x.shape, dtype=torch.float32, device=x.device)
    o2 = out.view(-1, C)
# ... 1196 lines not shown
```

Measured before the change: 17450.

## File SA compaction tables from ball query and enable compaction on more levels

The ball query kernels can now fill the SA compaction table (neighbour-count classes, row lists) while sweeping, so the fused SA forward can skip its separate zero and compact kernels when the table is already filed. A batched reset kernel zeroes up to four tables in one launch. The tracker also turns on compaction for SA levels 1 and 2 on both the search and template branches, where before only the last search level used it. In exchange the ball query kernel does extra LDS and atomic work plus a __syncthreads, and blocks no longer exit early.

```diff
diff --git a/include/ptt_hip.h b/include/ptt_hip.h
--- a/include/ptt_hip.h
+++ b/include/ptt_hip.h
@@ -8,7 +8,7 @@
 extern "C" {
 #endif
 
-#define PTT_ABI_VERSION 28
+#define PTT_ABI_VERSION 29
 
 enum {
     PTT_OK = 0,
@@ -42,6 +42,13 @@
 
 int ptt_centres_ball_query_f32(const float* xyz, const int32_t* sel, int B, int N, int M, float radius, int nsample,
                                float* new_xyz, int64_t* idx64_out, int32_t* idx_out, ptt_stream_t stream);
+
+int ptt_ball_query_table_f32(const float* new_xyz, const float* xyz, int B, int M, int N, float radius, int nsample,
+                             int32_t* idx_out, void* compact_ws, size_t compact_ws_bytes, ptt_stream_t stream);
+int ptt_centres_ball_query_table_f32(const float* xyz, const int32_t* sel, int B, int N, int M, float radius, int nsample,
+                                     float* new_xyz, int64_t* idx64_out, int32_t* idx_out, void* compact_ws,
+                                     size_t compact_ws_bytes, ptt_stream_t stream);
+int ptt_sa_compact_reset(void* ws0, void* ws1, void* ws2, void* ws3, ptt_stream_t stream);
 
 int ptt_group_f32(const float* feat, const int32_t* idx, int B, int C, int N, int M,
                   int ns, float* out, ptt_stream_t stream);
@@ -117,6 +124,10 @@
     int32_t ns, M, normalize_xyz, pro_relu;
 } ptt_row_job;
 int ptt_row_jobs_f32(const ptt_row_job* jobs, int n_jobs, ptt_stream_t stream);
+
+#define PTT_SA_COMPACT_BUILD 0
+#define PTT_SA_COMPACT_RESET 1
+#define PTT_SA_COMPACT_FILED 2
 
 typedef struct ptt_sa_desc {
     const float* xyz;
@@ -138,6 +149,7 @@
     int l0_relu;
     void* compact_ws;
     size_t compact_ws_bytes;
+    int compact_state;
 } ptt_sa_desc;
 
 int ptt_sa_fused_fwd_f32(const ptt_sa_desc* d, ptt_stream_t stream);
diff --git a/ptt_amd/_lib.py b/ptt_amd/_lib.py
--- a/ptt_amd/_lib.py
+++ b/ptt_amd/_lib.py
@@ -67,6 +67,7 @@
 PTT_MAX_SEGMENTS = DEFINES["PTT_MAX_SEGMENTS"]
 PTT_CROP_JOBS_BY_VALUE_MAX = DEFINES["PTT_CROP_JOBS_BY_VALUE_MAX"]
 PTT_TRAIN_MAX_CANDS = DEFINES["PTT_TRAIN_MAX_CANDS"]
+SA_COMPACT_BUILD, SA_COMPACT_RESET, SA_COMPACT_FILED = (DEFINES["PTT_SA_COMPACT_" + n] for n in ("BUILD", "RESET", "FILED"))
 
 
 class CropJob(Structure):
@@ -173,7 +174,7 @@
                 ("radius", c_float), ("use_xyz", c_int), ("normalize_xyz", c_int), ("n_layers", c_int),
                 ("layers", SaLayer * PTT_SA_MAX_LAYERS),
                 ("l0_point_term", c_void_p), ("l0_xyz_weight", c_void_p), ("l0_channels", c_int), ("l0_relu", c_int),
-                ("compact_ws", c_void_p), ("compact_ws_bytes", c_size_t)]
+                ("compact_ws", c_void_p), ("compact_ws_bytes", c_size_t), ("compact_state", c_int)]
 
 
 class XcorrDesc(Structure):
diff --git a/ptt_amd/csrc/common.h b/ptt_amd/csrc/common.h
--- a/ptt_amd/csrc/common.h
+++ b/ptt_amd/csrc/common.h
@@ -39,6 +39,15 @@
 int wgrad_stream_rows(int R);
 int launch_wgrad_stream(const float* dZ, int ldz, const float* X, int ldx, int R, int Cout, int Cin, int rows, float* partial,
                         const float* x_scale, const float* x_shift, hipStream_t s);
+
+constexpr int SAC_HDR = 16;
+struct SacTable {
+    int32_t* ws; int T;
+    __host__ __device__ int32_t* ndist() const { return ws + SAC_HDR; }
+    __host__ __device__ int32_t* list(int k) const { return ws + SAC_HDR + (size_t)(1 + k) * T; }
+    __host__ __device__ int32_t* rows(int k) const { return ws + SAC_HDR + 5 * (size_t)T + (size_t)((4 << k) - 4) * T; }
+    static size_t words(size_t T) { return SAC_HDR + 65 * T; }
+};
 
 template <int CTRL, int ROW_MASK>
 __device__ __forceinline__ int dpp_i32(int v) {
diff --git a/ptt_amd/csrc/mfma_ops.hip b/ptt_amd/csrc/mfma_ops.hip
--- a/ptt_amd/csrc/mfma_ops.hip
+++ b/ptt_amd/csrc/mfma_ops.hip
@@ -1275,14 +1275,6 @@
     __builtin_amdgcn_wave_barrier();
 }
 
-constexpr int SAC_HDR = 16;
-struct SacTable {
-    int32_t* ws; int T;
-    __host__ __device__ int32_t* ndist() const { return ws + SAC_HDR; }
-    __host__ __device__ int32_t* list(int k) const { return ws + SAC_HDR + (size_t)(1 + k) * T; }
-    __host__ __device__ int32_t* rows(int k) const { return ws + SAC_HDR + 5 * (size_t)T + (size_t)((4 << k) - 4) * T; }
-    static size_t words(size_t T) { return SAC_HDR + 65 * T; }
-};
 constexpr int SAC_PASSES = 4;
 
 __global__ __launch_bounds__(64) void sa_compact_zero_kernel(int32_t* ws) {
@@ -2062,6 +2054,8 @@
     if (!d->xyz || !d->new_xyz || !d->idx || !d->out || (!hoist && d->C > 0 && !d->feat))
         return fail(PTT_EINVAL, "ptt_sa_fused_fwd_f32: null pointer");
     if (!d->use_xyz && d->C == 0) return fail(PTT_EINVAL, "ptt_sa_fused_fwd_f32: no xyz and no features");
+    if (d->compact_ws && (d->compact_state < PTT_SA_COMPACT_BUILD || d->compact_state > PTT_SA_COMPACT_FILED))
+        return fail(PTT_EINVAL, "ptt_sa_fused_fwd_f32: compact_state=%d", d->compact_state);
     if (hoist) {
         const int c0 = d->l0_channels;
         if (!d->use_xyz || !d->l0_xyz_weight || c0 <= 0 || (c0 % 32) != 0 || c0 > 256 ||
@@ -2130,9 +2124,13 @@
             if (d->compact_ws_bytes < ptt_sa_compact_workspace(d->B, d->M) || (reinterpret_cast<uintptr_t>(d->compact_ws) & 15))
                 return fail(PTT_EWORKSPACE, "ptt_sa_fused_fwd_f32: compact_ws needs %zu bytes, 16-byte aligned (got %zu)",
                             ptt_sa_compact_workspace(d->B, d->M), d->compact_ws_bytes);
+            if (d->compact_state == PTT_SA_COMPACT_FILED)
+                return fail(PTT_EINVAL, "ptt_sa_fused_fwd_f32: no ball query files the table of the level without point features");
             p.cws = static_cast<int32_t*>(d->compact_ws);
-            hipLaunchKernelGGL(sa_compact_zero_kernel, dim3(1), dim3(64), 0, s, p.cws);
-            if ((rc = check_launch("sa_compact_zero_kernel"))) return rc;
+            if (d->compact_state != PTT_SA_COMPACT_RESET) {
+                hipLaunchKernelGGL(sa_compact_zero_kernel, dim3(1), dim3(64), 0, s, p.cws);
+                if ((rc = check_launch("sa_compact_zero_kernel"))) return rc;
+            }
             hipLaunchKernelGGL(sa_compact_kernel<true>, dim3((total_centres + 31) / 32), dim3(256), 0, s, d->xyz, d->idx, d->N, d->M,
                                SacTable{p.cws, total_centres});
             if ((rc = check_launch("sa_compact_kernel"))) return rc;
@@ -2178,11 +2176,15 @@
                 return fail(PTT_EWORKSPACE, "ptt_sa_fused_fwd_f32: compact_ws needs %zu bytes, 16-byte aligned (got %zu)",
                             ptt_sa_compact_workspace(d->B, d->M), d->compact_ws_bytes);
             p.cws = static_cast<int32_t*>(d->compact_ws);
-            hipLaunchKernelGGL(sa_compact_zero_kernel, dim3(1), dim3(64), 0, s, p.cws);
-            if ((rc = check_launch("sa_compact_zero_kernel"))) return rc;
-            hipLaunchKernelGGL(sa_compact_kernel<false>, dim3((total_centres + 31) / 32), dim3(256), 0, s, d->xyz, d->idx, d->N, d->M,
-                               SacTable{p.cws, total_centres});
-            if ((rc = check_launch("sa_compact_kernel"))) return rc;
+            if (d->compact_state == PTT_SA_COMPACT_BUILD) {
+                hipLaunchKernelGGL(sa_compact_zero_kernel, dim3(1), dim3(64), 0, s, p.cws);
+                if ((rc = check_launch("sa_compact_zero_kernel"))) return rc;
+            }
+            if (d->compact_state != PTT_SA_COMPACT_FILED) {
+                hipLaunchKernelGGL(sa_compact_kernel<false>, dim3((total_centres + 31) / 32), dim3(256), 0, s, d->xyz, d->idx, d->N,
+                                   d->M, SacTable{p.cws, total_centres});
+                if ((rc = check_launch("sa_compact_kernel"))) return rc;
+            }
             const int lds = (2 * SAS_TILE + 64 * 4 + 64) * (int)sizeof(float);
             if ((rc = set_lds_limit(reinterpret_cast<const void*>(sa_stream_compact_kernel), lds))) return rc;
             hipLaunchKernelGGL(sa_stream_compact_kernel, dim3(p.tiles < 512 ? p.tiles : 512), dim3(256), lds, s, p);
diff --git a/ptt_amd/csrc/point_ops.hip b/ptt_amd/csrc/point_ops.hip
--- a/ptt_amd/csrc/point_ops.hip
+++ b/ptt_amd/csrc/point_ops.hip
@@ -2,6 +2,7 @@
 
 #include <limits.h>
 #include <stdlib.h>
+#include <type_traits>
 #include "common.h"
 
 namespace ptt {
@@ -216,10 +217,10 @@
     return check_launch("fps_kernel");
 }
 
-template <int CPW>
+template <int CPW, bool TABLE = false>
 __device__ __forceinline__ void ball_sweep(const float* __restrict__ pts, int N, float r2, int ns, const float (&cx)[CPW],
                                            const float (&cy)[CPW], const float (&cz)[CPW], int ncentres,
-                                           int32_t* __restrict__ out0, int lane) {
+                                           int32_t* __restrict__ out0, int lane, int* srow = nullptr, int* nd = nullptr) {
     int cnt[CPW], first[CPW];
 #pragma unroll
     for (int c = 0; c < CPW; ++c) { cnt[c] = (c < ncentres) ? 0 : ns; first[c] = 0; }
@@ -238,7 +239,10 @@
             if (mask != 0ull) {
                 if (cnt[c] == 0) first[c] = base + (__ffsll((long long)mask) - 1);
                 const int pos = cnt[c] + __popcll(mask & ((1ull << lane) - 1ull));
-                if (hit && pos < ns) out0[(size_t)c * ns + pos] = k;
+                if (hit && pos < ns) {
+                    out0[(size_t)c * ns + pos] = k;
+                    if constexpr (TABLE) srow[c * 32 + pos] = k;
+                }
                 cnt[c] += __popcll(mask);
             }
             active = active || cnt[c] < ns;
@@ -250,50 +254,128 @@
         if (c >= ncentres) break;
         const int fill = (cnt[c] > 0) ? first[c] : 0;
         for (int s = cnt[c] + lane; s < ns; s += 64) out0[(size_t)c * ns + s] = fill;
+        if constexpr (TABLE) {
+            nd[c] = max(1, min(cnt[c], ns));
+            if (cnt[c] == 0 && lane == 0) srow[c * 32] = 0;
+        }
     }
 }
 
 template <int CPW>
+struct BallTableLds {
+    int cnt[4], base[4], cls[4 * CPW], pos[4 * CPW], nd[4 * CPW];
+    int row[4 * CPW][32];
+};
+template <int CPW, bool TABLE>
+__device__ __forceinline__ BallTableLds<CPW>* ball_table_lds() {
+    if constexpr (TABLE) {
+        __shared__ BallTableLds<CPW> L;
+        if (threadIdx.x < 4) L.cnt[threadIdx.x] = 0;
+        __syncthreads();
+        return &L;
+    } else {
+        return nullptr;
+    }
+}
+template <int CPW>
+__device__ __forceinline__ void ball_table_file(BallTableLds<CPW>& L, const SacTable& tab, int centre, int nc, const int (&nd)[CPW]) {
+    const int t = threadIdx.x, lane = t & 63, w = t >> 6;
+    if (lane == 0) {
+#pragma unroll
+        for (int c = 0; c < CPW; ++c) {
+            const bool valid = c < nc;
+            const int lc = w * CPW + c, n = valid ? nd[c] : 1;
+            const int k = n <= 4 ? 0 : n <= 8 ? 1 : n <= 16 ? 2 : 3;
+            L.cls[lc] = valid ? k : -1;
+            L.nd[lc] = n;
+            L.pos[lc] = valid ? atomicAdd(&L.cnt[k], 1) : 0;
+            if (valid) tab.ndist()[centre + c] = n;
+        }
+    }
+    __syncthreads();
+    if (t < 4) L.base[t] = L.cnt[t] ? atomicAdd(&tab.ws[t], L.cnt[t]) : 0;
+    __syncthreads();
+    const int g0 = blockIdx.x * 4 * CPW;
+    for (int e = t; e < 4 * CPW * 32; e += 256) {
+        const int lc = e >> 5, j = e & 31, k = L.cls[lc];
+        if (k < 0 || j >= (4 << k)) continue;
+        const int q = L.base[k] + L.pos[lc];
+        tab.rows(k)[(size_t)q * (4 << k) + j] = L.row[lc][j < L.nd[lc] ? j : 0];
+        if (j == 0) tab.list(k)[q] = g0 + lc;
+    }
+}
+
+struct NoBallTable {};
+template <bool TABLE>
+using BallTableArg = typename std::conditional<TABLE, SacTable, NoBallTable>::type;
+
+template <int CPW, bool TABLE = false>
 __global__ __launch_bounds__(256) void ball_query_kernel(const float* __restrict__ new_xyz,
                                                          const float* __restrict__ xyz, int BM, int M, int N,
-                                                         float r2, int ns, int32_t* __restrict__ idx_out) {
+                                                         float r2, int ns, int32_t* __restrict__ idx_out, BallTableArg<TABLE> tab) {
     const int centre = (blockIdx.x * 4 + (threadIdx.x >> 6)) * CPW;
-    if (centre >= BM) return;
+    if constexpr (!TABLE) {
+        if (centre >= BM) return;
+    }
+    BallTableLds<CPW>* const L = ball_table_lds<CPW, TABLE>();
     const int lane = threadIdx.x & 63;
-    const int b = centre / M;
-    float cx[CPW], cy[CPW], cz[CPW];
-    const int nc = min(CPW, BM - centre);
-#pragma unroll
-    for (int c = 0; c < CPW; ++c) {
-        const int cc = centre + (c < nc ? c : 0);
-        cx[c] = new_xyz[(size_t)cc * 3 + 0]; cy[c] = new_xyz[(size_t)cc * 3 + 1]; cz[c] = new_xyz[(size_t)cc * 3 + 2];
-    }
-    ball_sweep<CPW>(xyz + (size_t)b * N * 3, N, r2, ns, cx, cy, cz, nc, idx_out + (size_t)centre * ns, lane);
-}
-
-template <int CPW>
+    const bool live = !TABLE || centre < BM;
+    int nc = min(CPW, BM - centre);
+    if constexpr (TABLE) nc = live ? nc : 0;
+    int nd[CPW];
+    if (live) {
+        const int b = centre / M;
+        float cx[CPW], cy[CPW], cz[CPW];
+#pragma unroll
+        for (int c = 0; c < CPW; ++c) {
+            const int cc = centre + (c < nc ? c : 0);
+            cx[c] = new_xyz[(size_t)cc * 3 + 0]; cy[c] = new_xyz[(size_t)cc * 3 + 1]; cz[c] = new_xyz[(size_t)cc * 3 + 2];
+        }
+        ball_sweep<CPW, TABLE>(xyz + (size_t)b * N * 3, N, r2, ns, cx, cy, cz, nc, idx_out + (size_t)centre * ns, lane,
+                               TABLE ? &L->row[(threadIdx.x >> 6) * CPW][0] : nullptr, nd);
+    }
+    if constexpr (TABLE) ball_table_file<CPW>(*L, tab, centre, nc, nd);
+}
+
+template <int CPW, bool TABLE = false>
 __global__ __launch_bounds__(256) void centres_ball_query_kernel(const float* __restrict__ xyz, const int32_t* __restrict__ sel,
                                                                  int BM, int M, int N, float r2, int ns,
                                                                  float* __restrict__ new_xyz, long long* __restrict__ idx64,
-                                                                 int32_t* __restrict__ idx_out) {
+                                                                 int32_t* __restrict__ idx_out, BallTableArg<TABLE> tab) {
     const int centre = (blockIdx.x * 4 + (threadIdx.x >> 6)) * CPW;
-    if (centre >= BM) return;
+    if constexpr (!TABLE) {
+        if (centre >= BM) return;
+    }
+    BallTableLds<CPW>* const L = ball_table_lds<CPW, TABLE>();
     const int lane = threadIdx.x & 63;
-    const int b = centre / M;
-    const float* __restrict__ pts = xyz + (size_t)b * N * 3;
-    float cx[CPW], cy[CPW], cz[CPW];
-    const int nc = min(CPW, BM - centre);
-#pragma unroll
-    for (int c = 0; c < CPW; ++c) {
-        const int cc = centre + (c < nc ? c : 0);
-        const int n = sel ? sel[cc] : cc - b * M;
-        cx[c] = pts[3 * n + 0]; cy[c] = pts[3 * n + 1]; cz[c] = pts[3 * n + 2];
-        if (lane == 0 && c < nc) {
-            new_xyz[(size_t)cc * 3 + 0] = cx[c]; new_xyz[(size_t)cc * 3 + 1] = cy[c]; new_xyz[(size_t)cc * 3 + 2] = cz[c];
-            if (idx64) idx64[cc] = n;
-        }
-    }
-    ball_sweep<CPW>(pts, N, r2, ns, cx, cy, cz, nc, idx_out + (size_t)centre * ns, lane);
+    const bool live = !TABLE || centre < BM;
+    int nc = min(CPW, BM - centre);
+    if constexpr (TABLE) nc = live ? nc : 0;
+    int nd[CPW];
+    if (live) {
+        const int b = centre / M;
+        const float* __restrict__ pts = xyz + (size_t)b * N * 3;
+        float cx[CPW], cy[CPW], cz[CPW];
+#pragma unroll
+        for (int c = 0; c < CPW; ++c) {
+            const int cc = centre + (c < nc ? c : 0);
+            const int n = sel ? sel[cc] : cc - b * M;
+            cx[c] = pts[3 * n + 0]; cy[c] = pts[3 * n + 1]; cz[c] = pts[3 * n + 2];
+            if (lane == 0 && c < nc) {
+                new_xyz[(size_t)cc * 3 + 0] = cx[c]; new_xyz[(size_t)cc * 3 + 1] = cy[c]; new_xyz[(size_t)cc * 3 + 2] = cz[c];
+                if (idx64) idx64[cc] = n;
+            }
+        }
+        ball_sweep<CPW, TABLE>(pts, N, r2, ns, cx, cy, cz, nc, idx_out + (size_t)centre * ns, lane,
+                               TABLE ? &L->row[(threadIdx.x >> 6) * CPW][0] : nullptr, nd);
+    }
+    if constexpr (TABLE) ball_table_file<CPW>(*L, tab, centre, nc, nd);
+}
+
+__global__ __launch_bounds__(64) void sa_compact_reset_kernel(int32_t* a, int32_t* b, int32_t* c, int32_t* d) {
+    const int t = threadIdx.x;
+    int32_t* const ws = (t >> 2) == 0 ? a : (t >> 2) == 1 ? b : (t >> 2) == 2 ? c : d;
+    if (t < 16 && ws) ws[t & 3] = 0;
 }
 
 __global__ void gather_kernel(const float* __restrict__ feat, const int32_t* __restrict__ idx, int C, int N, int M,
@@ -1097,14 +1179,64 @@
     const int cpw = ball_cpw(BM, M);
     if (cpw == 8)
         hipLaunchKernelGGL((ball_query_kernel<8>), dim3((BM / 8 + 3) / 4), dim3(256), 0, as_stream(stream), new_xyz, xyz, BM, M,
-                           N, r2, nsample, idx_out);
+                           N, r2, nsample, idx_out, NoBallTable{});
     else if (cpw == 4)
         hipLaunchKernelGGL((ball_query_kernel<4>), dim3((BM / 4 + 3) / 4), dim3(256), 0, as_stream(stream), new_xyz, xyz, BM, M,
-                           N, r2, nsample, idx_out);
+                           N, r2, nsample, idx_out, NoBallTable{});
     else
         hipLaunchKernelGGL((ball_query_kernel<1>), dim3((BM + 3) / 4), dim3(256), 0, as_stream(stream), new_xyz, xyz, BM, M,
-                           N, r2, nsample, idx_out);
+                           N, r2, nsample, idx_out, NoBallTable{});
     return check_launch("ball_query_kernel");
+}
+
+static int ball_cpw_table(int BM, int M) {
+    const int force = dev_switches().ball_cpw;
+    if (force || (M & 3) != 0) return ball_cpw(BM, M);
+    return BM >= 2048 ? 4 : 1;
+}
+
+static int ball_table_check(const char* who, int B, int M, int nsample, void* ws, size_t ws_bytes) {
+    if (nsample != 32) return fail(PTT_EUNSUPPORTED, "%s: the ball table has 32 slots per ball (nsample=%d)", who, nsample);
+    if (!ws || ws_bytes < ptt_sa_compact_workspace(B, M) || (reinterpret_cast<uintptr_t>(ws) & 15))
+        return fail(PTT_EWORKSPACE, "%s: compact_ws needs %zu bytes, 16-byte aligned (got %zu)", who, ptt_sa_compact_workspace(B, M),
+                    ws_bytes);
+    return PTT_OK;
+}
+
+extern "C" int ptt_ball_query_table_f32(const float* new_xyz, const float* xyz, int B, int M, int N, float radius, int nsample,
+                                        int32_t* idx_out, void* compact_ws, size_t compact_ws_bytes, ptt_stream_t stream) {
+    if (B < 0 || M < 0 || N <= 0 || nsample <= 0)
+        return fail(PTT_EINVAL, "ptt_ball_query_table_f32: B=%d M=%d N=%d nsample=%d", B, M, N, nsample);
+    if (B == 0 || M == 0) return PTT_OK;
+    if (!new_xyz || !xyz || !idx_out) return fail(PTT_EINVAL, "ptt_ball_query_table_f32: null pointer");
+    if (int rc = ball_table_check("ptt_ball_query_table_f32", B, M, nsample, compact_ws, compact_ws_bytes)) return rc;
+    const float r2 = radius * radius;
+    const int BM = B * M;
+    const int cpw = ball_cpw_table(BM, M);
+    const SacTable tab{static_cast<int32_t*>(compact_ws), BM};
+    if (cpw == 8)
+        hipLaunchKernelGGL((ball_query_kernel<8, true>), dim3((BM / 8 + 3) / 4), dim3(256), 0, as_stream(stream), new_xyz, xyz, BM, M,
+                           N, r2, nsample, idx_out, tab);
+    else if (cpw == 4)
+        hipLaunchKernelGGL((ball_query_kernel<4, true>), dim3((BM / 4 + 3) / 4), dim3(256), 0, as_stream(stream), new_xyz, xyz, BM, M,
+                           N, r2, nsample, idx_out, tab);
+    else
+        hipLaunchKernelGGL((ball_query_kernel<1, true>), dim3((BM + 3) / 4), dim3(256), 0, as_stream(stream), new_xyz, xyz, BM, M,
+                           N, r2, nsample, idx_out, tab);
+    return check_launch("ball_query_kernel<table>");
+}
+
+extern "C" int ptt_sa_compact_reset(void* ws0, void* ws1, void* ws2, void* ws3, ptt_stream_t stream) {
+    void* const ws[4] = {ws0, ws1, ws2, ws3};
+    bool any = false;
+    for (void* p : ws) {
+        if (reinterpret_cast<uintptr_t>(p) & 15) return fail(PTT_EWORKSPACE, "ptt_sa_compact_reset: a workspace is not 16-byte aligned");
+        any = any || p;
+    }
+    if (!any) return PTT_OK;
+    hipLaunchKernelGGL(sa_compact_reset_kernel, dim3(1), dim3(64), 0, as_stream(stream), static_cast<int32_t*>(ws0),
+                       static_cast<int32_t*>(ws1), static_cast<int32_t*>(ws2), static_cast<int32_t*>(ws3));
+    return check_launch("sa_compact_reset_kernel");
 }
 
 extern "C" int ptt_gather_f32(const float* feat, const int32_t* idx, int B, int C, int N, int M, float* out,
@@ -1166,14 +1298,37 @@
     const int cpw = ball_cpw(BM, M);
     if (cpw == 8)
         hipLaunchKernelGGL((centres_ball_query_kernel<8>), dim3((BM / 8 + 3) / 4), dim3(256), 0, as_stream(stream), xyz, sel, BM,
-                           M, N, radius * radius, nsample, new_xyz, reinterpret_cast<long long*>(idx64_out), idx_out);
+                           M, N, radius * radius, nsample, new_xyz, reinterpret_cast<long long*>(idx64_out), idx_out, NoBallTable{});
     else if (cpw == 4)
         hipLaunchKernelGGL((centres_ball_query_kernel<4>), dim3((BM / 4 + 3) / 4), dim3(256), 0, as_stream(stream), xyz, sel, BM,
-                           M, N, radius * radius, nsample, new_xyz, reinterpret_cast<long long*>(idx64_out), idx_out);
+                           M, N, radius * radius, nsample, new_xyz, reinterpret_cast<long long*>(idx64_out), idx_out, NoBallTable{});
     else
         hipLaunchKernelGGL((centres_ball_query_kernel<1>), dim3((BM + 3) / 4), dim3(256), 0, as_stream(stream), xyz, sel, BM, M,
-                           N, radius * radius, nsample, new_xyz, reinterpret_cast<long long*>(idx64_out), idx_out);
+                           N, radius * radius, nsample, new_xyz, reinterpret_cast<long long*>(idx64_out), idx_out, NoBallTable{});
     return check_launch("centres_ball_query_kernel");
+}
+
+extern "C" int ptt_centres_ball_query_table_f32(const float* xyz, const int32_t* sel, int B, int N, int M, float radius, int nsample,
+                                                float* new_xyz, int64_t* idx64_out, int32_t* idx_out, void* compact_ws,
+                                                size_t compact_ws_bytes, ptt_stream_t stream) {
+    if (B < 0 || M < 0 || N <= 0 || nsample <= 0 || (!sel && M > N))
+        return fail(PTT_EINVAL, "ptt_centres_ball_query_table_f32: B=%d M=%d N=%d nsample=%d", B, M, N, nsample);
+    if (B == 0 || M == 0) return PTT_OK;
+    if (!xyz || !new_xyz || !idx_out) return fail(PTT_EINVAL, "ptt_centres_ball_query_table_f32: null pointer");
+    if (int rc = ball_table_check("ptt_centres_ball_query_table_f32", B, M, nsample, compact_ws, compact_ws_bytes)) return rc;
+    const int BM = B * M;
+    const int cpw = ball_cpw_table(BM, M);
+    const SacTable tab{static_cast<int32_t*>(compact_ws), BM};
+    if (cpw == 8)
+        hipLaunchKernelGGL((centres_ball_query_kernel<8, true>), dim3((BM / 8 + 3) / 4), dim3(256), 0, as_stream(stream), xyz, sel, BM,
+                           M, N, radius * radius, nsample, new_xyz, reinterpret_cast<long long*>(idx64_out), idx_out, tab);
+    else if (cpw == 4)
+        hipLaunchKernelGGL((centres_ball_query_kernel<4, true>), dim3((BM / 4 + 3) / 4), dim3(256), 0, as_stream(stream), xyz, sel, BM,
+                           M, N, radius * radius, nsample, new_xyz, reinterpret_cast<long long*>(idx64_out), idx_out, tab);
+    else
+        hipLaunchKernelGGL((centres_ball_query_kernel<1, true>), dim3((BM + 3) / 4), dim3(256), 0, as_stream(stream), xyz, sel, BM, M,
+                           N, radius * radius, nsample, new_xyz, reinterpret_cast<long long*>(idx64_out), idx_out, tab);
+    return check_launch("centres_ball_query_kernel<table>");
 }
 
 
diff --git a/ptt_amd/models/backbones_3d/pointnet2/pointnet2_modules.py b/ptt_amd/models/backbones_3d/pointnet2/pointnet2_modules.py
--- a/ptt_amd/models/backbones_3d/pointnet2/pointnet2_modules.py
+++ b/ptt_amd/models/backbones_3d/pointnet2/pointnet2_modules.py
@@ -5,7 +5,7 @@
 import torch.nn as nn
 import torch.nn.functional as F
 
-from .... import ops, train_ops
+from .... import _lib, ops, train_ops
 from ....param_cache import (DropsCachesOnModeChange, FoldedLayer, ParamCache, conv_bn_tensors, fold_conv_bn,
                              index_table)
 from . import pointnet2_utils
@@ -13,6 +13,7 @@
 
 STREAM_COMPACT_MIN_BALLS = 2048
 STREAM_COMPACT_MAX_POINTS = 1024
+TABLE_FROM_QUERY_MIN_BALLS = 2048
 
 
 class PointnetSAModuleVotes(DropsCachesOnModeChange, nn.Module):
@@ -93,13 +94,13 @@
         return layers, hoist
 
     def forward(self, xyz: torch.Tensor, features: torch.Tensor, npoint: int, inds: torch.Tensor = None, pre=None,
-                compact: bool = False):
+                compact: bool = False, table: torch.Tensor = None):
         self.centres_knn = None
         if self._fusable(xyz, features):
-            return self._forward_fused(xyz, features, npoint, inds, pre, compact)
+            return self._forward_fused(xyz, features, npoint, inds, pre, compact, table)
         return self._forward_train(xyz, features, npoint, inds)
 
-    def _forward_fused(self, xyz, features, npoint, inds, pre, compact):
+    def _forward_fused(self, xyz, features, npoint, inds, pre, compact, table=None):
         if (pre is None and inds is None and self.sample_method == 'fps' and xyz.shape[1] <= 256 and npoint <= 128
                 and xyz.shape[0] * npoint * self.nsample <= ops.ONE_FRAME_MAX_SA_ROWS and self.centres_knn_k <= npoint):
             xyz = xyz.contiguous()
@@ -117,13 +118,16 @@
             inds = inds.to(torch.int32)
 
         xyz = xyz.contiguous()
+        layers, hoist = self._fused_params(xyz.device)
+        compact = (bool(compact) and hoist is not None and features is not None and xyz.shape[0] * npoint >= STREAM_COMPACT_MIN_BALLS
+                   and xyz.shape[1] <= STREAM_COMPACT_MAX_POINTS)
+        filed = table if (compact and pre is None and self.nsample == 32 and xyz.shape[0] * npoint >= TABLE_FROM_QUERY_MIN_BALLS) else None
         if pre is not None:
             new_xyz, idx, inds64 = pre
         elif prefix:
-            new_xyz, _, idx = ops.centres_ball_query(xyz, None, npoint, self.radius, self.nsample)
+            new_xyz, _, idx = ops.centres_ball_query(xyz, None, npoint, self.radius, self.nsample, table=filed)
         else:
-            new_xyz, inds64, idx = ops.centres_ball_query(xyz, inds.contiguous(), npoint, self.radius, self.nsample)
-        layers, hoist = self._fused_params(xyz.device)
+            new_xyz, inds64, idx = ops.centres_ball_query(xyz, inds.contiguous(), npoint, self.radius, self.nsample, table=filed)
         if hoist is not None and features is not None:
             wf_packed, wx, c0, relu0 = hoist
             rows = features.transpose(1, 2)
@@ -141,12 +145,14 @@
                 return new_xyz, pooled.transpose(1, 2), inds64
             new_features = ops.sa_fused_forward(xyz, new_xyz, idx, None, layers[1:], self.radius, True,
                                                 self.normalize_xyz, point_major_out=True, l0=(term, wx, relu0),
-                                                compact=(bool(compact) and B * M >= STREAM_COMPACT_MIN_BALLS
-                                                         and xyz.shape[1] <= STREAM_COMPACT_MAX_POINTS))
+                                                compact=compact,
+                                                table=((filed, _lib.SA_COMPACT_FILED) if filed is not None else
+                                                       (table, _lib.SA_COMPACT_RESET) if compact and table is not None else None))
         else:
             new_features = ops.sa_fused_forward(xyz, new_xyz, idx, features, layers, self.radius,
                                                 self.use_xyz, self.normalize_xyz, point_major_out=True,
-                                                compact=features is None)
+                                                compact=features is None,
+                                                table=(table, _lib.SA_COMPACT_RESET) if table is not None else None)
         return new_xyz, new_features, inds64
 
     def _forward_train(self, xyz, features, npoint, inds):
diff --git a/ptt_amd/models/backbones_3d/pointnet2_backbone.py b/ptt_amd/models/backbones_3d/pointnet2_backbone.py
--- a/ptt_amd/models/backbones_3d/pointnet2_backbone.py
+++ b/ptt_amd/models/backbones_3d/pointnet2_backbone.py
@@ -30,6 +30,7 @@
         self.seed_knn = 16
         self.overlap_branches = True
         self._side_stream = None
+        self.compact_levels = {'search': (len(sa.RADIUS) - 1,), 'template': ()}
 
     @staticmethod
     def _break_up_pc(pc):
@@ -52,6 +53,13 @@
         rows = features.transpose(1, 2)
         out = ops.linear(rows, wpacked, w.shape[0], None, bias)
         return out.transpose(1, 2)
+
+    def _branch_tables(self, xyz, features, npoints, compact_levels):
+        if (self.training or not xyz.is_cuda or len(self.SA_modules) != 3 or not compact_levels
+                or xyz.shape[0] * max(npoints[k] for k in compact_levels) < pointnet2_modules.STREAM_COMPACT_MIN_BALLS):
+            return {}
+        levels = ([0] if features is None else []) + sorted(compact_levels)
+        return dict(zip(levels, ops.sa_compact_tables(xyz.device, [(xyz.shape[0], int(npoints[k])) for k in levels])))
 
     def branch_forward(self, pts, npoints: List, inds0=None, want_knn=0, compact_levels=()):
         xyz, features = self._break_up_pc(pts)
@@ -79,9 +87,12 @@
             xyz, features, inds2 = self.SA_modules[2](xyz=xyz, features=features, npoint=npoints[2],
                                                       pre=(levels[2][0], levels[2][1], seq[2]))
         else:
-            xyz, features, inds0 = self.SA_modules[0](xyz=xyz, features=features, npoint=npoints[0], inds=inds0)
-            xyz, features, inds1 = self.SA_modules[1](xyz=xyz, features=features, npoint=npoints[1], compact=1 in compact_levels)
-            xyz, features, inds2 = self.SA_modules[2](xyz=xyz, features=features, npoint=npoints[2], compact=2 in compact_levels)
+            tables = self._branch_tables(xyz, features, npoints, compact_levels)
+            xyz, features, inds0 = self.SA_modules[0](xyz=xyz, features=features, npoint=npoints[0], inds=inds0, table=tables.get(0))
+            xyz, features, inds1 = self.SA_modules[1](xyz=xyz, features=features, npoint=npoints[1], compact=1 in compact_levels,
+                                                      table=tables.get(1))
+            xyz, features, inds2 = self.SA_modules[2](xyz=xyz, features=features, npoint=npoints[2], compact=2 in compact_levels,
+                                                      table=tables.get(2))
         point_features = self._cov_final(features)
         assert inds1.dtype == inds2.dtype == torch.int64, 'index type must be int64, not {}'.format(inds2.dtype)
         if all(m.sample_method in ('rs', 'sequence') for m in self.SA_modules[1:]) and inds0.shape[1] >= npoints[2]:
@@ -102,18 +113,19 @@
     def forward_branches(self, search_points, template_points, inds=None):
         sa = self.model_cfg.SA_CONFIG
         i_s, i_t = inds if inds is not None else (None, None)
-        last = (len(self.SA_modules) - 1,) if (search_points.is_cuda and not self.training) else ()
+        on = search_points.is_cuda and not self.training
+        c_s, c_t = (tuple(self.compact_levels[k]) if on else () for k in ('search', 'template'))
         if not (self.overlap_branches and search_points.is_cuda and not self.training):
-            r = self.branch_forward(search_points, sa.NPOINTS_SEARCH, i_s, want_knn=self.seed_knn, compact_levels=last)
-            t_seeds, t_feats, t_inds = self.branch_forward(template_points, sa.NPOINTS_TEMPLATE, i_t)
+            r = self.branch_forward(search_points, sa.NPOINTS_SEARCH, i_s, want_knn=self.seed_knn, compact_levels=c_s)
+            t_seeds, t_feats, t_inds = self.branch_forward(template_points, sa.NPOINTS_TEMPLATE, i_t, compact_levels=c_t)
         else:
             if self._side_stream is None or self._side_stream.device != search_points.device:
                 self._side_stream = torch.cuda.Stream(device=search_points.device)
             main = torch.cuda.current_stream(search_points.device)
             side = graph_policy.branch(main, self._side_stream)
             with torch.cuda.stream(side):
-                t_seeds, t_feats, t_inds = self.branch_forward(template_points, sa.NPOINTS_TEMPLATE, i_t)
-            r = self.branch_forward(search_points, sa.NPOINTS_SEARCH, i_s, want_knn=self.seed_knn, compact_levels=last)
+                t_seeds, t_feats, t_inds = self.branch_forward(template_points, sa.NPOINTS_TEMPLATE, i_t, compact_levels=c_t)
+            r = self.branch_forward(search_points, sa.NPOINTS_SEARCH, i_s, want_knn=self.seed_knn, compact_levels=c_s)
             graph_policy.join(main, side)
             if side is not main:
                 for t in (t_seeds, t_feats, t_inds, template_points):
diff --git a/ptt_amd/models/trackers/tracker3d_template.py b/ptt_amd/models/trackers/tracker3d_template.py
--- a/ptt_amd/models/trackers/tracker3d_template.py
+++ b/ptt_amd/models/trackers/tracker3d_template.py
@@ -49,6 +49,8 @@
             model_cfg=cfg, input_channels=model_info_dict['num_point_features'],
             grid_size=model_info_dict['grid_size'], voxel_size=model_info_dict['voxel_size'],
             point_cloud_range=model_info_dict['point_cloud_range'])
+        if hasattr(module, 'compact_levels'):
+            module.compact_levels = {'search': (1, 2), 'template': (1, 2)}
         model_info_dict['module_list'].append(module)
         model_info_dict['num_point_features'] = module.num_point_features
         return module, model_info_dict
diff --git a/ptt_amd/ops.py b/ptt_amd/ops.py
--- a/ptt_amd/ops.py
+++ b/ptt_amd/ops.py
@@ -220,12 +220,42 @@
 GRID_BALL_QUERY_MIN_POINTS = 4096
 
 
-def ball_query(new_xyz, xyz, radius, nsample):
+def sa_compact_workspace(B, M, device):
+    return torch.empty(((_host("ptt_sa_compact_workspace", int(B), int(M)) + 3) // 4,), dtype=torch.int32, device=device)
+
+
+def sa_compact_tables(device, shapes):
+    words = [(_host("ptt_sa_compact_workspace", int(B), int(M)) // 4 + 3) & ~3 for B, M in shapes]
+    tables = list(torch.empty((sum(words),), dtype=torch.int32, device=device).split(words))
+    sa_compact_reset(*tables)
+    return tables
+
+
+def sa_compact_reset(*tables):
+    if not 1 <= len(tables) <= 4:
+        raise RuntimeError("sa_compact_reset takes one to four workspaces")
+    a, b, c, d = [_ptr(t) for t in tables] + [None] * (4 - len(tables))
+    _launch("ptt_sa_compact_reset", tables[0].device, a, b, c, d)
+
+
+def _table_arg(table, xyz, N):
+    if not isinstance(table, torch.Tensor) or table.device != xyz.device or not table.is_contiguous():
+        raise RuntimeError("table must be a contiguous workspace tensor on %s" % xyz.device)
+    if N >= GRID_BALL_QUERY_MIN_POINTS:
+        raise RuntimeError("the grid ball query (clouds of %d points or more) files no ball table" % GRID_BALL_QUERY_MIN_POINTS)
+    return _ptr(table), table.numel() * table.element_size()
+
+
+def ball_query(new_xyz, xyz, radius, nsample, table=None):
     _chk(new_xyz, "new_xyz", torch.float32, 3)
     _chk(xyz, "xyz", torch.float32, 3)
     B, M, _ = new_xyz.shape
     N = xyz.shape[1]
     out = torch.empty((B, M, int(nsample)), dtype=torch.int32, device=xyz.device)
+    if table is not None:
+        _launch("ptt_ball_query_table_f32", xyz.device, _ptr(new_xyz), _ptr(xyz), B, M, N, float(radius), int(nsample), _ptr(out),
+                *_table_arg(table, xyz, N), timed='ptt_ball_query_f32')
+        return out
     if GRID_BALL_QUERY_MIN_POINTS <= N <= 131072:
         ws, ws_arg = _workspace("ptt_ball_query_grid_workspace", xyz.device, B, N)
         _launch("ptt_ball_query_grid_f32", xyz.device, _ptr(new_xyz), _ptr(xyz), B, M, N, float(radius), int(nsample), _ptr(out), *ws_arg,
@@ -236,7 +266,7 @@
     return out
 
 
-def centres_ball_query(xyz, sel, npoint, radius, nsample, want_idx64=True):
+def centres_ball_query(xyz, sel, npoint, radius, nsample, want_idx64=True, table=None):
     _chk(xyz, "xyz", torch.float32, 3)
     B, N, _ = xyz.shape
     if sel is not None:
@@ -245,7 +275,10 @@
     new_xyz = torch.empty((B, M, 3), dtype=torch.float32, device=xyz.device)
     idx64 = torch.empty((B, M), dtype=torch.int64, device=xyz.device) if (want_idx64 and sel is not None) else None
     idx = torch.empty((B, M, int(nsample)), dtype=torch.int32, device=xyz.device)
-    if GRID_BALL_QUERY_MIN_POINTS <= N <= 131072:
+    if table is not None:
+        _launch("ptt_centres_ball_query_table_f32", xyz.device, _ptr(xyz), _ptr(sel), B, N, M, float(radius), int(nsample), _ptr(new_xyz),
+                _ptr(idx64), _ptr(idx), *_table_arg(table, xyz, N), timed='ptt_ball_query_f32')
+    elif GRID_BALL_QUERY_MIN_POINTS <= N <= 131072:
         ws, ws_arg = _workspace("ptt_ball_query_grid_workspace", xyz.device, B, N)
         _launch("ptt_centres_ball_query_grid_f32", xyz.device, _ptr(xyz), _ptr(sel), B, N, M, float(radius), int(nsample), _ptr(new_xyz), _ptr(idx64),
                 _ptr(idx), *ws_arg, timed='ptt_ball_query_f32')
@@ -345,7 +378,7 @@
 
 
 def sa_fused_forward(xyz, new_xyz, idx, features, layers, radius, use_xyz=True, normalize_xyz=False,
-                     point_major_out=True, l0=None, compact=False):
+                     point_major_out=True, l0=None, compact=False, table=None):
     _chk(xyz, "xyz", torch.float32, 3)
     _chk(new_xyz, "new_xyz", torch.float32, 3)
     _chk(idx, "idx", torch.int32, 3)
@@ -388,7 +421,13 @@
             raise RuntimeError("l0 point term must be (B,N,C0) and the xyz weight (3,C0)")
         d.l0_point_term, d.l0_xyz_weight = term.data_ptr(), wx.data_ptr()
         d.l0_channels, d.l0_relu = term.shape[2], int(bool(l0_relu))
-    if isinstance(compact, torch.Tensor):
+    if table is not None and not isinstance(compact, torch.Tensor):
+        if compact:
+            ws, d.compact_state = table
+            if not isinstance(ws, torch.Tensor) or ws.device != xyz.device or not ws.is_contiguous():
+                raise RuntimeError("compact workspace must be a contiguous tensor on %s" % xyz.device)
+            d.compact_ws, d.compact_ws_bytes = ws.data_ptr(), ws.numel() * ws.element_size()
+    elif isinstance(compact, torch.Tensor):
         if not compact.is_cuda or compact.device != xyz.device or not compact.is_contiguous():
             raise RuntimeError("compact workspace must be a contiguous tensor on %s" % xyz.device)
         d.compact_ws, d.compact_ws_bytes = compact.data_ptr(), compact.numel() * compact.element_size()
```

Result: no change. 17430 (-0.1%).
